# populationgenomics/cuKING

Hardware: AMD Instinct MI355X
Metric: sample-pairs/s (all-pairs KING) (higher is better)
Workload: dtype fp4 products, f32 accumulate (exact integers)

## Files before the change

### cuking_amd/build.py

```python
from __future__ import annotations

import argparse
import os
import shutil
import subprocess
import sys
from pathlib import Path

PKG = Path(__file__).resolve().parent
ROOT = PKG.parent
CSRC = PKG / "csrc"
HOST = PKG / "host"
INCLUDE = ROOT / "include"

LIB_PATH = PKG / "libcuking_amd.so"
CLI_PATH = PKG / "bin" / "cuking"
LIB_FLAGS_PATH = PKG / "libcuking_amd.flags"

HIP_SOURCES = ["king_abi.hip", "king_kernels.hip", "king_mfma.hip", "king_filter.hip",
               "king_sort.hip", "synth.hip"]
HOST_ABI_SOURCES = ["king_host.cc"]
HIP_FLAGS = [
    "--offload-arch=gfx950", "-O3", "-std=c++17", "-fPIC", "-Wall",
    "-fno-fast-math", "-ffp-contract=off",
    "-fhip-fp32-correctly-rounded-divide-sqrt",
]


ROCM = Path(os.environ.get("ROCM_PATH", "/opt/rocm"))
ROCM_HOST_FLAGS = ["-D__HIP_PLATFORM_AMD__=1", f"-isystem{ROCM / 'include'}"]
ROCM_HOST_LIBS = [f"-L{ROCM / 'lib'}", "-lrccl", "-lamdhip64"]


def _hipcc() -> str:
    exe = shutil.which("hipcc") or "/opt/rocm/bin/hipcc"
    if not os.path.exists(exe):
        raise RuntimeError("hipcc not found: the HIP library cannot be built")
    return exe


def _newer(target: Path, deps) -> bool:
    if not target.exists():
        return False
    t = target.stat().st_mtime
    return all(Path(d).stat().st_mtime <= t for d in deps)


def build_library(force: bool = False, save_temps: bool = False) -> Path:
    srcs = [CSRC / s for s in HIP_SOURCES + HOST_ABI_SOURCES]
    deps = srcs + [CSRC / "king_common.h", CSRC / "king_device.h", CSRC / "king_host.h",
                   CSRC / "king_submatrix.h", INCLUDE / "cuking_amd.h",
                   Path(__file__)]
    extra = os.environ.get("CUKING_EXTRA_HIPFLAGS", "").split()
    wanted = " ".join(extra)
    stamped = LIB_FLAGS_PATH.read_text().strip() if LIB_FLAGS_PATH.exists() else wanted
    if not force and _newer(LIB_PATH, deps) and stamped == wanted:
        return LIB_PATH
    cmd = [_hipcc(), *HIP_FLAGS, "-shared", f"-I{INCLUDE}", f"-I{CSRC}",
           *map(str, srcs), "-o", str(LIB_PATH)]
    for flag in extra:
        cmd.insert(1, flag)
    cwd = PKG / "build_tmp"
    cwd.mkdir(exist_ok=True)
    cmd += ["-save-temps"]
    if save_temps:
        cmd += ["-Rpass-analysis=kernel-resource-usage"]
        subprocess.run(cmd, check=True, cwd=str(cwd))
    else:
        with open(cwd / "build.log", "w") as log:
            r = subprocess.run(cmd, cwd=str(cwd), stdout=log, stderr=subprocess.STDOUT)
        if r.returncode != 0:
            sys.stderr.write((cwd / "build.log").read_text()[-8000:])
            raise subprocess.CalledProcessError(r.returncode, cmd)
    problems = check_mfma_loops(cwd / "king_mfma-hip-amdgcn-amd-amdhsa-gfx950.s")
    problems += check_filter_loop(cwd / "king_filter-hip-amdgcn-amd-amdhsa-gfx950.s")
    if problems and not extra:
        LIB_PATH.unlink(missing_ok=True)
        raise RuntimeError("matrix-core kernel: the compiler put vector-memory waits or scratch "
                           "accesses inside an LDS-DMA loop:\n  " + "\n  ".join(problems))
    for line in problems:
        print("warning (experiment build):", line, file=sys.stderr)
    LIB_FLAGS_PATH.write_text(wanted + "\n")
    return LIB_PATH


def check_filter_loop(asm_path: Path, verbose: bool = False):
    import re
    text = Path(asm_path).read_text()
    bodies = [m.group(1) for m in re.finditer(
        r"\n_ZN6cuking12_GLOBAL__N_1\d+king_filter(?:_persistent)?_kernelE\w+:(.*?)\.Lfunc_end", text, re.S)]
    if len(bodies) < 2:
        return [f"king_filter_kernel / king_filter_persistent_kernel not both in {asm_path}"]
    problems, seen = [], 0
    for block in (b for body in bodies for b in re.split(r"\n(?=\.LBB\d+_\d+:)", body)):
        lines = block.split("\n")
        head = lines[0].split(":")[0]
        end = next((i for i, l in enumerate(lines)
                    if re.search(r"s_cbranch_\w+ " + re.escape(head) + r"\b", l)), None)
        if end is None:
            continue
        loop = lines[:end + 1]
        mfma = sum("v_mfma" in l for l in loop)
        if mfma < 16 or not any("global_load_lds" in l for l in loop):
            continue
        seen += 1
        scratch = [l.strip() for l in loop if "scratch_" in l]
        waits = [l.strip() for l in loop if re.search(r"s_waitcnt.*vmcnt\(\d+\)", l)]
        foreign = [w for w in waits if "vmcnt(22)" not in w]
        if verbose:
            print(f"king_filter_kernel: loop {head} ({mfma} MFMAs): scratch {len(scratch)}, "
                  f"vmcnt waits {waits}")
        if scratch or foreign:
            problems.append(f"king_filter_kernel, loop {head}: scratch {scratch[:2]}, waits {foreign}")
    if seen < 2:
        problems.append("king_filter kernels: an LDS-DMA loop is missing (listing format changed?)")
    return problems


def check_mfma_loops(asm_path: Path, verbose: bool = False):
    import re
    text = Path(asm_path).read_text()
    funcs = re.split(r"\n(?=_ZN6cuking12_GLOBAL__N_116king_mfma_kernel\w+:)", text)[1:]
    if not funcs:
        return [f"no king_mfma_kernel in {asm_path}"]
    problems = []
    for f in funcs:
        m = re.match(r"_ZN6cuking12_GLOBAL__N_116king_mfma_kernelILb(\d)ELb(\d)ELb(\d)", f)
        label = f"king_mfma_kernel<FULL={m.group(1)}, SPLIT={m.group(2)}, N4={m.group(3)}>"
        body = f.split(".Lfunc_end")[0]
        seen = 0
        for block in re.split(r"\n(?=\.LBB\d+_\d+:)", body):
            lines = block.split("\n")
            head = lines[0].split(":")[0]
            end = next((i for i, l in enumerate(lines)
                        if re.search(r"s_cbranch_\w+ " + re.escape(head) + r"\b", l)), None)
            if end is None:
                continue
            loop = lines[:end + 1]
            mfma = sum("v_mfma" in l for l in loop)
            if mfma < 16 or not any("global_load_lds" in l for l in loop):
                continue
            seen += 1
            scratch = [l.strip() for l in loop if "scratch_" in l]
            waits = [l.strip() for l in loop if re.search(r"s_waitcnt.*vmcnt\(\d+\)", l)]
            foreign = [w for w in waits
                       if not any(f"vmcnt({n})" in w for n in (16, 20, 24))]
            if verbose:
                print(f"{label}: loop {head} ({mfma} MFMAs): scratch {len(scratch)}, "
                      f"vmcnt waits {waits}")
            if scratch or foreign:
                problems.append(f"{label}, loop {head}: scratch {scratch[:2]}, waits {foreign}")
        if seen == 0:
            problems.append(f"{label}: no LDS-DMA loop found (listing format changed?)")
    return problems


def arrow_flags():
    import pyarrow
    inc = pyarrow.get_include()
    libdir = pyarrow.get_library_dirs()[0]
    libs = []
    for stem in ("parquet", "arrow"):
        cands = sorted(Path(libdir).glob(f"lib{stem}.so.*"))
        if not cands:
            raise RuntimeError(f"lib{stem}.so not found in {libdir}")
        libs.append(f"-l:{cands[0].name}")
    return inc, libdir, libs


def build_cli(force: bool = False) -> Path:
    srcs = sorted(HOST.glob("*.cc"))
    if not srcs:
        raise RuntimeError("no host sources")
    deps = srcs + sorted(HOST.glob("*.h")) + [INCLUDE / "cuking_amd.h",
                                              LIB_PATH, Path(__file__)]
    if not force and _newer(CLI_PATH, deps):
        return CLI_PATH
    inc, libdir, libs = arrow_flags()
    CLI_PATH.parent.mkdir(exist_ok=True)
    cmd = ["g++", "-O2", "-std=c++20", "-Wall", "-pthread",
           f"-I{INCLUDE}", f"-I{HOST}", f"-isystem{inc}", *ROCM_HOST_FLAGS,
           *map(str, srcs), "-o", str(CLI_PATH),
           f"-L{PKG}", "-l:libcuking_amd.so", f"-L{libdir}", *libs, *ROCM_HOST_LIBS,
           f"-Wl,-rpath,{libdir}", "-Wl,-rpath,$ORIGIN/..",
           "-Wl,-rpath,/opt/rocm/lib"]
    subprocess.run(cmd, check=True)
    return CLI_PATH


def main(argv=None) -> int:
    ap = argparse.ArgumentParser()
    ap.add_argument("--lib", action="store_true", help="library only")
    ap.add_argument("--force", action="store_true")
    ap.add_argument("--save-temps", action="store_true")
    args = ap.parse_args(argv)
    print(build_library(force=args.force, save_temps=args.save_temps))
    if not args.lib:
        print(build_cli(force=args.force))
    return 0


if __name__ == "__main__":
    sys.exit(main())
```

### cuking_amd/csrc/king_abi.hip

```cpp
#include <hip/hip_runtime.h>

#include <algorithm>
#include <atomic>
#include <cstdarg>
#include <cstdio>
#include <cstdlib>
#include <cstring>
#include <string>
#include <tuple>
#include <vector>

#include "king_common.h"
#include "king_host.h"

using namespace cuking;

namespace {

#define HIP_TRY(expr)                                                      \
  do {                                                                     \
    const hipError_t _e = (expr);                                          \
    if (_e != hipSuccess) {                                                \
      (void)hipGetLastError();  \
      return cuking_fail(_e == hipErrorOutOfMemory ? CUKING_ERR_OUT_OF_MEMORY     \
                                            : CUKING_ERR_DEVICE,           \
                  "%s failed: %s", #expr, hipGetErrorString(_e));          \
    }                                                                      \
  } while (0)

uint32_t ceil_div(uint32_t a, uint32_t b) {
  return (uint32_t)(((uint64_t)a + b - 1) / b);
}
uint32_t round_up(uint32_t a, uint32_t b) { return ceil_div(a, b) * b; }

struct EventPair {
  hipEvent_t start = nullptr, stop = nullptr;
};

struct Timer {
  std::vector<EventPair> pool;
  size_t used = 0;

  hipError_t begin(hipStream_t s, EventPair **out) {
    if (used == pool.size()) {
      EventPair p;
      hipError_t e = hipEventCreate(&p.start);
      if (e != hipSuccess) return e;
      e = hipEventCreate(&p.stop);
      if (e != hipSuccess) return e;
      pool.push_back(p);
    }
    *out = &pool[used++];
    return hipEventRecord((*out)->start, s);
  }
  hipError_t collect(double *ms, uint64_t *n) {
    *ms = 0;
    *n = used;
    for (size_t k = 0; k < used; ++k) {
      hipError_t e = hipEventSynchronize(pool[k].stop);
      if (e != hipSuccess) return e;
      float t = 0;
      e = hipEventElapsedTime(&t, pool[k].start, pool[k].stop);
      if (e != hipSuccess) return e;
      *ms += t;
    }
    return hipSuccess;
  }
  void destroy() {
    for (auto &p : pool) {
      if (p.start) (void)hipEventDestroy(p.start);
      if (p.stop) (void)hipEventDestroy(p.stop);
    }
    pool.clear();
    used = 0;
  }
};

}

struct cuking_ctx {
  int device = 0;
  cuking_kernel kernel = CUKING_KERNEL_TILED;
  int variant = 0;
  uint32_t band_rows = 0;
  int counts_mode = -1;
  int xcd_swizzle = 2;
  uint32_t dyn_tail_tiles = 16384;

  uint4 *planes = nullptr;
  size_t planes_bytes = 0;
  uint64_t *band_prefix = nullptr;
  size_t band_prefix_entries = 0;
  TileSpace prefix_for = {0, 0, 0, 0};

  uint32_t split_wgs = 0;
  std::vector<std::pair<hipStream_t, uint32_t *>> split_scratch;
  struct FilterScratch {
    hipStream_t stream;
    uint8_t *base;
    uint64_t tiles;
  };
  std::vector<FilterScratch> filter_scratch;
  unsigned long long filter_totals_retired[kNumTotals] = {};
  uint32_t filter_quadrant_cap = kFilterQuadrantCap;
  uint32_t filter_cand_cap = kFilterCandCap;
  uint32_t filter_split_min_steps = 8;
  int filter_check0 = 1, filter_check1 = 1, filter_check_emit = (int)kCheckEmitCap;
  int filter_rotate = 1;
  uint32_t filter_rotate_min_steps = 128;
  uint32_t filter_rotate_min_tiles = 2048;
  bool filter_persistent = false;
  uint32_t filter_persistent_min_tiles = 2048;
  int filter_sort = 1;
  bool filter_lazy_codes = true;
  void *sort_temp = nullptr;
  size_t sort_temp_bytes = 0;

  struct Prepared {
    bool valid = false;
    cuking_submatrix sm = {0, 0, 0, 0};
    uint32_t words_per_sample = 0;
    int variant = -1;
    uint32_t tile = 0;
    const uint64_t *bits = nullptr;
    bool codes = true;
    std::vector<uint8_t> tiles;
    hipStream_t ordered_on = nullptr;
    bool ordered_valid = false;
  } prepared;
  std::vector<std::pair<hipStream_t, hipEvent_t>> readers;

  bool reuse_prepared = false;
  uint64_t workspace_allocations = 0, host_syncs = 0, conversions_skipped = 0;

  bool timing = false;
  Timer king_timer, prepare_timer;
};

namespace {

int default_variant() {
  if (const char *v = getenv("CUKING_AMD_VARIANT")) {
    const int k = atoi(v);
    if (k >= 0 && k < kNumTiledVariants) return k;
  }
  return kMfmaFilterVariant;
}

int effective_variant(const cuking_ctx *ctx, uint32_t words_per_sample) {
  const uint64_t sites = (uint64_t)round_up(words_per_sample, 8) * 32;
  int v = ctx->variant;
  if ((v == kMfmaN4Variant || v == kMfmaFilterVariant) && sites > kMfmaN4MaxSites) v = kMfmaVariant;
  if (v == kMfmaVariant && sites > kMfmaMaxSites) v = 2;
  return v;
}

TiledVariant plan_variant(const cuking_ctx *ctx, uint32_t words_per_sample) {
  TiledVariant v = tiled_variant(effective_variant(ctx, words_per_sample));
  v.tile = tiled_variant(ctx->variant).tile;
  return v;
}

bool use_full_counts(const cuking_ctx *ctx, float kin_threshold, bool dense,
                     uint32_t words_per_sample) {
  if (dense || ctx->counts_mode == 1) return true;
  if (ctx->counts_mode == 0) return false;
  if (!(kin_threshold > 0.0f)) return true;
  const double sites = 32.0 * words_per_sample;
  const double c = is_mfma_variant(effective_variant(ctx, words_per_sample)) ? 2.05 : 1.6;
  return (double)kin_threshold * kin_threshold * sites < c * c;
}

cuking_status bind(cuking_ctx *ctx) {
  if (ctx == nullptr) return cuking_fail(CUKING_ERR_INVALID_ARGUMENT, "null context");
  HIP_TRY(hipSetDevice(ctx->device));
  return CUKING_OK;
}

PlaneGeometry make_geometry(const cuking_submatrix &sm,
                            uint32_t words_per_sample,
                            const TiledVariant &v) {
  PlaneGeometry g;
  g.num_rows = sm_num_rows(sm);
  g.num_cols = sm_num_cols(sm);
  g.diag = sm_is_diag(sm) ? 1u : 0u;
  g.rows_padded = round_up(g.num_rows, v.tile);
  g.cols_padded = round_up(g.num_cols, v.tile);
  g.col_base = g.diag ? 0u : g.rows_padded;
  g.s_stride = g.diag ? g.rows_padded : g.rows_padded + g.cols_padded;
  g.k_words = round_up(words_per_sample, v.k_chunk);
  return g;
}

uint32_t band_rows_for(uint32_t pinned, const PlaneGeometry &g, const TiledVariant &v) {
  if (pinned != 0) return pinned;
  if (v.layout == kLayoutWord) return 17;
  if (v.tile == kFilterTile) return 8;
  return g.rows_padded / v.tile >= 128 ? 5 : 17;
}

TileSpace make_tiles(const PlaneGeometry &g, const TiledVariant &v,
                     uint32_t band_rows) {
  band_rows = band_rows_for(band_rows, g, v);
  TileSpace t;
  t.tiles_r = g.rows_padded / v.tile;
  t.tiles_c = g.cols_padded / v.tile;
  t.band_rows = band_rows;
  t.diag = g.diag;
  return t;
}

uint64_t total_tiles(const TileSpace &t) {
  uint64_t n = 0;
  for (uint32_t b = 0; b < t.num_bands(); ++b) n += t.band_tiles(b);
  return n;
}

cuking_status split_scratch_for(cuking_ctx *ctx, hipStream_t stream,
                                uint32_t **scratch, uint32_t **counters) {
  *scratch = *counters = nullptr;
  if (ctx->split_wgs == 0 || !is_mfma_variant(ctx->variant)) return CUKING_OK;
  const size_t bytes = mfma_split_scratch_bytes(ctx->split_wgs);
  uint32_t *base = nullptr;
  for (auto &e : ctx->split_scratch)
    if (e.first == stream) base = e.second;
  if (base == nullptr) {
    if (ctx->split_scratch.size() >= 8) {
      ++ctx->host_syncs;
      HIP_TRY(hipDeviceSynchronize());
      for (auto &e : ctx->split_scratch) (void)hipFree(e.second);
      ctx->split_scratch.clear();
    }
    HIP_TRY(hipMalloc(reinterpret_cast<void **>(&base), bytes));
    ++ctx->workspace_allocations;
    hipError_t e = hipMemsetAsync(base, 0, mfma_split_counter_bytes(ctx->split_wgs), stream);
    if (e != hipSuccess) {
      (void)hipFree(base);
      HIP_TRY(e);
    }
    ctx->split_scratch.emplace_back(stream, base);
  }
  *counters = base;
  *scratch = base + mfma_split_counter_bytes(ctx->split_wgs) / sizeof(uint32_t);
  return CUKING_OK;
}

static void retire_filter_totals(cuking_ctx *ctx, const cuking_ctx::FilterScratch &e) {
  if (e.base == nullptr) return;
  unsigned long long v[kNumTotals] = {};
  if (hipMemcpy(v, e.base + filter_scratch_layout(e.tiles).totals, sizeof v,
                hipMemcpyDeviceToHost) != hipSuccess) {
    (void)hipGetLastError();
    return;
  }
  for (uint32_t k = 0; k < kNumTotals; ++k) ctx->filter_totals_retired[k] += v[k];
}

cuking_status filter_scratch_for(cuking_ctx *ctx, hipStream_t stream, const PlaneGeometry &geo,
                                 uint64_t tiles, TiledArgs *a) {
  a->sample_stats = nullptr;
  a->t2 = nullptr;
  a->filter_ctrl = nullptr;
  a->cand_list = nullptr;
  a->dense_list = nullptr;
  a->cand_cap = a->dense_cap = a->quadrant_cap = 0;
  a->fsplit_parts = a->fsplit_first = a->fsplit_tile0 = 0;
  a->fsplit_slabs = nullptr;
  a->fsplit_tickets = nullptr;
  a->filter_totals = nullptr;
  a->tile_done = nullptr;
  a->prefix_u = nullptr;
  a->cohort_sums = nullptr;
  a->check_steps = nullptr;
  a->check0 = a->check1 = 0;
  a->rotate = a->rotate_min_steps = a->rotate_min_tiles = 0;
  a->persist_wgs = a->persist_min_tiles = 0;
  if (ctx->variant != kMfmaFilterVariant) return CUKING_OK;
  const FilterScratchLayout want = filter_scratch_layout(tiles);
  cuking_ctx::FilterScratch *entry = nullptr;
  for (auto &e : ctx->filter_scratch)
    if (e.stream == stream) entry = &e;
  if (entry != nullptr && filter_scratch_layout(entry->tiles).bytes < want.bytes) {
    ++ctx->host_syncs;
    HIP_TRY(hipStreamSynchronize(stream));
    retire_filter_totals(ctx, *entry);
    (void)hipFree(entry->base);
    entry->base = nullptr;
  }
  if (entry == nullptr || entry->base == nullptr) {
    if (entry == nullptr && ctx->filter_scratch.size() >= 8) {
      ++ctx->host_syncs;
      HIP_TRY(hipStreamSynchronize(ctx->filter_scratch.front().stream));
      (void)hipGetLastError();
      retire_filter_totals(ctx, ctx->filter_scratch.front());
      (void)hipFree(ctx->filter_scratch.front().base);
      ctx->filter_scratch.erase(ctx->filter_scratch.begin());
    }
    uint8_t *base = nullptr;
    HIP_TRY(hipMalloc(reinterpret_cast<void **>(&base), want.bytes));
    ++ctx->workspace_allocations;
    hipError_t e = hipMemsetAsync(base + want.totals, 0, kFilterCtrlBytes + kFilterTicketBytes, stream);
    if (e != hipSuccess) {
      (void)hipFree(base);
      HIP_TRY(e);
    }
    if (entry == nullptr) {
      ctx->filter_scratch.push_back({stream, base, tiles});
      entry = &ctx->filter_scratch.back();
    } else {
      entry->base = base;
      entry->tiles = tiles;
    }
  }
  uint8_t *base = entry->base;
  const FilterScratchLayout l = filter_scratch_layout(entry->tiles);
  a->sample_stats = plane_stats(ctx->planes, geo);
  a->t2 = plane_t2(ctx->planes, geo);
  a->prefix_u = plane_prefix_u(ctx->planes, geo);
  a->cohort_sums = plane_cohort_sums(ctx->planes, geo);
  a->filter_ctrl = reinterpret_cast<uint32_t *>(base);
  a->filter_totals = reinterpret_cast<unsigned long long *>(base + l.totals);
  a->fsplit_tickets = reinterpret_cast<uint32_t *>(base + l.tickets);
  a->tile_done = base + l.tile_done;
  a->cand_list = reinterpret_cast<uint2 *>(base + l.cand);
  a->cand_cap = ctx->filter_cand_cap < l.cand_entries ? ctx->filter_cand_cap : l.cand_entries;
  a->quadrant_cap = ctx->filter_quadrant_cap;
  a->dense_list = reinterpret_cast<uint2 *>(base + l.dense);
  a->dense_cap = l.chunk_tiles * 4;
  a->fsplit_first = ctx->filter_split_min_steps;
  a->fsplit_slabs = ctx->split_wgs != 0 ? reinterpret_cast<float4 *>(base + l.slabs) : nullptr;
  a->check0 = (uint32_t)ctx->filter_check0;
  a->check1 = (uint32_t)ctx->filter_check1 | ((uint32_t)ctx->filter_check_emit << 8) |
              (ctx->filter_check0 != 0 ? 1u << 16 : 0u);
  a->rotate = (uint32_t)ctx->filter_rotate;
  a->rotate_min_steps = ctx->filter_rotate_min_steps;
  a->rotate_min_tiles = ctx->filter_rotate_min_tiles;
  a->persist_wgs = ctx->filter_persistent ? 1u : 0u;
  a->persist_min_tiles = ctx->filter_persistent_min_tiles;
  a->check_steps = plane_check_steps(ctx->planes, geo);
  return CUKING_OK;
}

void layout_order_for(const cuking_ctx *ctx, uint32_t words_per_sample, const PlaneGeometry &geo,
                      TiledArgs *a) {
  a->perm = nullptr;
  a->codes_ready = nullptr;
  if (plan_variant(ctx, words_per_sample).layout != kLayoutNibbleStats) return;
  a->perm = plane_perm(ctx->planes, geo);
  if (!ctx->prepared.codes) a->codes_ready = plane_flags(ctx->planes, geo);
}

hipError_t launch_planned(const cuking_ctx *ctx, uint32_t words_per_sample, bool full,
                          TiledArgs a, uint64_t num_tiles, hipStream_t stream) {
  const int kv = effective_variant(ctx, words_per_sample);
  a.quad = 0;
  a.tile_list = nullptr;
  a.tile_list_count = nullptr;
  a.tile_list_cap = 0;
  if (tiled_variant(kv).tile != tiled_variant(ctx->variant).tile) {
    if (tiled_variant(kv).tile * 2 != tiled_variant(ctx->variant).tile) return hipErrorInvalidValue;
    a.quad = 1;
    a.tile_begin *= 4;
    num_tiles *= 4;
  }
  return launch_tiled(kv, full, a, num_tiles, stream);
}

void note_reader(cuking_ctx *ctx, hipStream_t stream) {
  for (auto &r : ctx->readers)
    if (r.first == stream) return;
  ctx->readers.emplace_back(stream, nullptr);
}

cuking_status wait_for_readers(cuking_ctx *ctx, hipStream_t stream) {
  bool failed = false;
  for (auto &r : ctx->readers) {
    if (r.first == stream) continue;
    if (r.second == nullptr &&
        hipEventCreateWithFlags(&r.second, hipEventDisableTiming) != hipSuccess) {
      failed = true;
      break;
    }
    if (hipEventRecord(r.second, r.first) != hipSuccess ||
        hipStreamWaitEvent(stream, r.second, 0) != hipSuccess) {
      failed = true;
      break;
    }
  }
  if (failed) {
    (void)hipGetLastError();
    ++ctx->host_syncs;
    HIP_TRY(hipDeviceSynchronize());
  }
  for (auto &r : ctx->readers)
    if (r.second) (void)hipEventDestroy(r.second);
  ctx->readers.clear();
  ctx->readers.emplace_back(stream, nullptr);
  ctx->prepared.ordered_on = stream;
  ctx->prepared.ordered_valid = true;
  for (auto &t : ctx->prepared.tiles)
    if (t == 2) t = 1;
  return CUKING_OK;
}

void mark_read(cuking_ctx *ctx, uint32_t begin, uint32_t end) {
  std::vector<uint8_t> &t = ctx->prepared.tiles;
  if (end > t.size()) end = (uint32_t)t.size();
  for (uint32_t k = begin; k < end; ++k) t[k] = 2;
}

bool same_block(const cuking_ctx::Prepared &p, const cuking_submatrix &sm,
                uint32_t words_per_sample, int variant, uint32_t tile, const uint64_t *bits) {
  return p.valid && p.sm.i_begin == sm.i_begin && p.sm.i_end == sm.i_end &&
         p.sm.j_begin == sm.j_begin && p.sm.j_end == sm.j_end &&
         p.words_per_sample == words_per_sample && p.variant == variant &&
         p.tile == tile && p.bits == bits;
}

cuking_status ensure_workspace(cuking_ctx *ctx, size_t need, size_t entries) {
  if (need > ctx->planes_bytes) {
    ++ctx->host_syncs;
    HIP_TRY(hipDeviceSynchronize());
    if (ctx->planes) HIP_TRY(hipFree(ctx->planes));
    ctx->planes = nullptr;
    ctx->planes_bytes = 0;
    ctx->prepared.valid = false;
    HIP_TRY(hipMalloc(reinterpret_cast<void **>(&ctx->planes), need));
    ++ctx->workspace_allocations;
    ctx->planes_bytes = need;
  }
  if (entries > ctx->band_prefix_entries) {
    ++ctx->host_syncs;
    HIP_TRY(hipDeviceSynchronize());
    if (ctx->band_prefix) HIP_TRY(hipFree(ctx->band_prefix));
    ctx->band_prefix = nullptr;
    ctx->band_prefix_entries = 0;
    ctx->prefix_for = TileSpace{0, 0, 0, 0};
    HIP_TRY(hipMalloc(reinterpret_cast<void **>(&ctx->band_prefix), entries * sizeof(uint64_t)));
    ++ctx->workspace_allocations;
    ctx->band_prefix_entries = entries;
  }
  return CUKING_OK;
}

cuking_status ensure_sort_temp(cuking_ctx *ctx, uint32_t n) {
  const size_t need = sort_temp_bytes_for(n);
  if (need <= ctx->sort_temp_bytes) return CUKING_OK;
  ++ctx->host_syncs;
  HIP_TRY(hipDeviceSynchronize());
  if (ctx->sort_temp) HIP_TRY(hipFree(ctx->sort_temp));
  ctx->sort_temp = nullptr;
  ctx->sort_temp_bytes = 0;
  HIP_TRY(hipMalloc(&ctx->sort_temp, need));
  ++ctx->workspace_allocations;
  ctx->sort_temp_bytes = need;
  return CUKING_OK;
}

bool same_tile_space(const TileSpace &a, const TileSpace &b) {
  return a.tiles_r == b.tiles_r && a.tiles_c == b.tiles_c && a.band_rows == b.band_rows &&
         a.diag == b.diag;
}

cuking_status upload_prefix(cuking_ctx *ctx, const TileSpace &tiles, hipStream_t stream) {
  const uint32_t nb = tiles.num_bands();
  std::vector<uint64_t> prefix((size_t)nb + 1, 0);
  for (uint32_t b = 0; b < nb; ++b) prefix[b + 1] = prefix[b] + tiles.band_tiles(b);
  HIP_TRY(hipMemcpyAsync(ctx->band_prefix, prefix.data(), prefix.size() * sizeof(uint64_t),
                         hipMemcpyHostToDevice, stream));
  ++ctx->host_syncs;
  HIP_TRY(hipStreamSynchronize(stream));
  ctx->prefix_for = tiles;
  return CUKING_OK;
}

cuking_status convert_codes_now(cuking_ctx *ctx, const PlaneGeometry &geo,
                                uint32_t words_per_sample, const uint64_t *d_bit_sets,
                                hipStream_t stream) {
  cuking_ctx::Prepared &pr = ctx->prepared;
  const uint32_t all = (uint32_t)pr.tiles.size();
  for (uint32_t t = 0; t < all;) {
    if (pr.tiles[t] == 0) {
      ++t;
      continue;
    }
    uint32_t e = t;
    while (e < all && pr.tiles[e] != 0) ++e;
    HIP_TRY(launch_prepare_nibbles(true, false, d_bit_sets, words_per_sample, geo, ctx->planes,
                                   plane_perm(ctx->planes, geo), t, e, nullptr, nullptr, stream));
    t = e;
  }
  HIP_TRY(hipMemsetAsync(plane_flags(ctx->planes, geo), 1, sizeof(uint32_t), stream));
  pr.codes = true;
  return CUKING_OK;
}

cuking_status prepare(cuking_ctx *ctx, const cuking_submatrix &sm,
                      uint32_t words_per_sample, const uint64_t *d_bit_sets,
                      hipStream_t stream, PlaneGeometry *geo_out,
                      TileSpace *tiles_out, bool need_codes, uint32_t s_tile_begin = 0,
                      uint32_t s_tile_end = 0xFFFFFFFFu) {
  const int variant = effective_variant(ctx, words_per_sample);
  const TiledVariant v = plan_variant(ctx, words_per_sample);
  const PlaneGeometry geo = make_geometry(sm, words_per_sample, v);
  const TileSpace tiles = make_tiles(geo, v, ctx->band_rows);
  *geo_out = geo;
  *tiles_out = tiles;

  const size_t need = plane_bytes(geo, v.layout);
  const uint32_t nb = tiles.num_bands();
  cuking_status st = ensure_workspace(ctx, need, (size_t)nb + 1);
  if (st != CUKING_OK) return st;
  if (v.layout == kLayoutNibbleStats && ctx->filter_sort != 0) {
    st = ensure_sort_temp(ctx, geo.s_stride);
    if (st != CUKING_OK) return st;
  }
  const uint32_t all_tiles = (geo.s_stride + 63) / 64;
  const uint32_t t_end = s_tile_end < all_tiles ? s_tile_end : all_tiles;
  cuking_ctx::Prepared &pr = ctx->prepared;
  const bool new_prefix = !same_tile_space(ctx->prefix_for, tiles);
  const bool same = same_block(pr, sm, words_per_sample, variant, v.tile, d_bit_sets);
  if (ctx->reuse_prepared && same && !new_prefix) {
    bool all_there = true;
    for (uint32_t t = s_tile_begin; t < t_end && all_there; ++t) all_there = pr.tiles[t] != 0;
    if (all_there) {
      ++ctx->conversions_skipped;
      if (v.layout == kLayoutNibbleStats && need_codes && !pr.codes)
        return convert_codes_now(ctx, geo, words_per_sample, d_bit_sets, stream);
      return CUKING_OK;
    }
  }
  const bool other_stream = pr.ordered_valid && pr.ordered_on != stream;
  bool must_wait = new_prefix && !ctx->readers.empty();
  if (!same) {
    must_wait = must_wait || !ctx->readers.empty();
    pr.valid = true;
    pr.sm = sm;
    pr.words_per_sample = words_per_sample;
    pr.variant = variant;
    pr.tile = v.tile;
    pr.bits = d_bit_sets;
    pr.tiles.assign(all_tiles, 0);
    pr.codes = true;
  }
  for (uint32_t t = s_tile_begin; t < t_end; ++t)
    must_wait = must_wait || pr.tiles[t] == 2 || (pr.tiles[t] == 1 && other_stream);
  if (must_wait) {
    st = wait_for_readers(ctx, stream);
    if (st != CUKING_OK) return st;
  }
  for (uint32_t t = s_tile_begin; t < t_end; ++t) pr.tiles[t] = 1;
  if (new_prefix) {
    st = upload_prefix(ctx, tiles, stream);
    if (st != CUKING_OK) return st;
  }

  if (need == 0) return CUKING_OK;
  EventPair *ev = nullptr;
  if (ctx->timing) HIP_TRY(ctx->prepare_timer.begin(stream, &ev));
  if (v.layout == kLayoutNibbleStats) {
    const bool whole = s_tile_begin == 0 && t_end == all_tiles;
    const bool codes = need_codes || !ctx->filter_lazy_codes || !whole;
    const uint32_t sb = s_tile_begin * 64, se = t_end * 64;
    if (s_tile_begin == 0)
      HIP_TRY(hipMemsetAsync(const_cast<unsigned long long *>(plane_cohort_sums(ctx->planes, geo)),
                             0, 64, stream));
    HIP_TRY(hipMemsetAsync(plane_flags(ctx->planes, geo), 0, sizeof(uint32_t), stream));
    HIP_TRY(launch_sample_stats(d_bit_sets, words_per_sample, geo, ctx->planes, sb, se, stream));
    HIP_TRY(launch_sample_order(geo, words_per_sample, ctx->planes, sb, se,
                                ctx->filter_sort == 2 || (ctx->filter_sort == 1 && whole),
                                ctx->sort_temp, ctx->sort_temp_bytes, stream));
    HIP_TRY(launch_prepare_nibbles(codes, true, d_bit_sets, words_per_sample, geo, ctx->planes,
                                   plane_perm(ctx->planes, geo), s_tile_begin, t_end, nullptr,
                                   nullptr, stream));
    if (!codes) {
      pr.codes = false;
    } else if (!pr.codes) {
      st = convert_codes_now(ctx, geo, words_per_sample, d_bit_sets, stream);
      if (st != CUKING_OK) return st;
    } else {
      HIP_TRY(hipMemsetAsync(plane_flags(ctx->planes, geo), 1, sizeof(uint32_t), stream));
    }
  } else {
    HIP_TRY(launch_prepare_planes(v.layout, d_bit_sets, words_per_sample, geo, ctx->planes,
                                  s_tile_begin, s_tile_end, stream));
  }
  if (ev) HIP_TRY(hipEventRecord(ev->stop, stream));
  return CUKING_OK;
}

cuking_status run_tiled(cuking_ctx *ctx, const cuking_submatrix &sm,
                        uint32_t words_per_sample, const uint64_t *d_bit_sets,
                        uint64_t tile_begin, uint64_t tile_end, bool whole,
                        float kin_threshold, uint32_t max_results,
                        cuking_result *d_results, uint32_t *d_result_index,
                        uint32_t *d_result_overflow, cuking_counts *d_counts,
                        hipStream_t stream) {
  PlaneGeometry geo;
  TileSpace tiles;
  const bool full = use_full_counts(ctx, kin_threshold, d_counts != nullptr, words_per_sample);
  const bool filter_runs = effective_variant(ctx, words_per_sample) == kMfmaFilterVariant &&
                           !full && kin_threshold > 0.f && kin_threshold < 0.5f;
  cuking_status st =
      prepare(ctx, sm, words_per_sample, d_bit_sets, stream, &geo, &tiles, !filter_runs);
  if (st != CUKING_OK) return st;
  const uint64_t n_tiles = total_tiles(tiles);
  if (whole) {
    tile_begin = 0;
    tile_end = n_tiles;
  }
  if (tile_begin > tile_end || tile_end > n_tiles)
    return cuking_fail(CUKING_ERR_INVALID_ARGUMENT,
                "tile range [%llu, %llu) outside [0, %llu)",
                (unsigned long long)tile_begin, (unsigned long long)tile_end,
                (unsigned long long)n_tiles);
  if (tile_begin == tile_end) return CUKING_OK;

  TiledArgs a = {};
  a.planes = ctx->planes;
  a.geo = geo;
  a.tiles = tiles;
  a.band_prefix = ctx->band_prefix;
  a.tile_begin = tile_begin;
  a.i_begin = sm.i_begin;
  a.j_begin = sm.j_begin;
  a.kin_threshold = kin_threshold;
  a.max_results = max_results;
  a.results = d_results;
  a.result_index = d_result_index;
  a.result_overflow = d_result_overflow;
  a.dense_counts = d_counts;
  a.rect_rows = a.rect_cols = a.rect_row0 = a.rect_col0 = 0;
  a.rect_row_stride = 1;
  a.bits = d_bit_sets;
  a.words_per_sample = words_per_sample;
  a.split_tiles = 0;
  a.split_whole = 0;
  a.split_wgs = ctx->split_wgs;
  a.xcd_chunk = (uint32_t)ctx->xcd_swizzle;
  a.launch_tiles = 0;
  a.dyn_tiles = ctx->dyn_tail_tiles;
  a.dyn_wgs = 0;
  st = split_scratch_for(ctx, stream, &a.split_scratch, &a.split_counters);
  if (st != CUKING_OK) return st;
  st = filter_scratch_for(ctx, stream, geo, n_tiles, &a);
  if (st != CUKING_OK) return st;
  layout_order_for(ctx, words_per_sample, geo, &a);

  EventPair *ev = nullptr;
  if (ctx->timing) HIP_TRY(ctx->king_timer.begin(stream, &ev));
  HIP_TRY(launch_planned(ctx, words_per_sample, full, a, tile_end - tile_begin, stream));
  note_reader(ctx, stream);
  mark_read(ctx, 0, 0xFFFFFFFFu);
  if (ev) HIP_TRY(hipEventRecord(ev->stop, stream));
  return CUKING_OK;
}

cuking_status run_stream(cuking_ctx *ctx, const cuking_submatrix &sm,
                         uint32_t words_per_sample, const uint64_t *d_bit_sets,
                         float kin_threshold, uint32_t max_results,
                         cuking_result *d_results, uint32_t *d_result_index,
                         uint32_t *d_result_overflow, cuking_counts *d_counts,
                         hipStream_t stream) {
  EventPair *ev = nullptr;
  if (ctx->timing) HIP_TRY(ctx->king_timer.begin(stream, &ev));
  HIP_TRY(launch_stream(sm, words_per_sample, d_bit_sets, kin_threshold,
                        max_results, d_results, d_result_index,
                        d_result_overflow, d_counts, stream));
  if (ev) HIP_TRY(hipEventRecord(ev->stop, stream));
  return CUKING_OK;
}

}

extern "C" {


int cuking_device_count(void) {
  int n = 0;
  if (hipGetDeviceCount(&n) != hipSuccess) return 0;
  return n;
}

cuking_status cuking_ctx_create(int device, cuking_ctx **out) {
  if (out == nullptr) return cuking_fail(CUKING_ERR_INVALID_ARGUMENT, "null out pointer");
  *out = nullptr;
  int n = 0;
  hipError_t e = hipGetDeviceCount(&n);
  if (e != hipSuccess || n == 0)
    return cuking_fail(CUKING_ERR_DEVICE,
                "no HIP device available (%s); this library has no CPU path",
                e == hipSuccess ? "0 devices" : hipGetErrorString(e));
  if (device < 0 || device >= n)
    return cuking_fail(CUKING_ERR_INVALID_ARGUMENT, "device %d outside [0, %d)", device, n);
  hipDeviceProp_t prop;
  HIP_TRY(hipGetDeviceProperties(&prop, device));
  if (strncmp(prop.gcnArchName, "gfx950", 6) != 0)
    return cuking_fail(CUKING_ERR_DEVICE,
                "device %d is %s; this library only carries gfx950 code",
                device, prop.gcnArchName);
  HIP_TRY(hipSetDevice(device));
  cuking_ctx *ctx = new cuking_ctx();
  ctx->device = device;
  ctx->variant = default_variant();
  ctx->split_wgs = (uint32_t)prop.multiProcessorCount;
  if (const char *v = getenv("CUKING_AMD_SPLIT_WGS")) {
    const int k = atoi(v);
    if (k >= 0 && k <= 4096) ctx->split_wgs = (uint32_t)k;
  }
  if (const char *v = getenv("CUKING_AMD_XCD_SWIZZLE")) {
    const int k = atoi(v);
    if (k >= 0 && k <= 2) ctx->xcd_swizzle = k;
  }
  if (const char *v = getenv("CUKING_AMD_DYN_TAIL_TILES")) {
    const long long k = atoll(v);
    if (k >= 0 && k <= 0x7FFFFFFF) ctx->dyn_tail_tiles = (uint32_t)k;
  }
  if (const char *v = getenv("CUKING_AMD_BAND_ROWS")) {
    const int k = atoi(v);
    if (k >= 1 && k <= 64) ctx->band_rows = (uint32_t)k;
  }
  *out = ctx;
  return CUKING_OK;
}

void cuking_ctx_destroy(cuking_ctx *ctx) {
  if (ctx == nullptr) return;
  (void)hipSetDevice(ctx->device);
  if (ctx->planes) (void)hipFree(ctx->planes);
  if (ctx->band_prefix) (void)hipFree(ctx->band_prefix);
  if (ctx->sort_temp) (void)hipFree(ctx->sort_temp);
  for (auto &e : ctx->split_scratch) (void)hipFree(e.second);
  for (auto &e : ctx->filter_scratch) (void)hipFree(e.base);
  for (auto &r : ctx->readers)
    if (r.second) (void)hipEventDestroy(r.second);
  ctx->king_timer.destroy();
  ctx->prepare_timer.destroy();
  delete ctx;
}

cuking_status cuking_ctx_set_kernel(cuking_ctx *ctx, cuking_kernel kernel) {
  if (ctx == nullptr) return cuking_fail(CUKING_ERR_INVALID_ARGUMENT, "null context");
  if (kernel != CUKING_KERNEL_TILED && kernel != CUKING_KERNEL_STREAM)
    return cuking_fail(CUKING_ERR_INVALID_ARGUMENT, "unknown kernel %d", (int)kernel);
  ctx->kernel = kernel;
  return CUKING_OK;
}

cuking_status cuking_ctx_set_option(cuking_ctx *ctx, const char *key,
                                    int64_t value) {
  if (ctx == nullptr || key == nullptr)
    return cuking_fail(CUKING_ERR_INVALID_ARGUMENT, "null argument");
  if (strcmp(key, "variant") == 0) {
    if (value < 0 || value >= kNumTiledVariants)
      return cuking_fail(CUKING_ERR_INVALID_ARGUMENT, "variant outside [0, %d)",
                  kNumTiledVariants);
    ctx->variant = (int)value;
    return CUKING_OK;
  }
  if (strcmp(key, "band_rows") == 0) {
    if (value < 0 || value > 64)
      return cuking_fail(CUKING_ERR_INVALID_ARGUMENT, "band_rows outside [0, 64]");
    ctx->band_rows = (uint32_t)value;
    return CUKING_OK;
  }
  if (strcmp(key, "split_wgs") == 0) {
    if (value < 0 || value > 4096)
      return cuking_fail(CUKING_ERR_INVALID_ARGUMENT, "split_wgs outside [0, 4096]");
    if ((uint32_t)value != ctx->split_wgs) {
      HIP_TRY(hipDeviceSynchronize());
      for (auto &e : ctx->split_scratch) (void)hipFree(e.second);
      ctx->split_scratch.clear();
    }
    ctx->split_wgs = (uint32_t)value;
    return CUKING_OK;
  }
  if (strcmp(key, "max_launch_blocks") == 0) {
    if (value < 0) return cuking_fail(CUKING_ERR_INVALID_ARGUMENT, "negative block cap");
    set_max_blocks_per_launch((uint64_t)value);
    return CUKING_OK;
  }
  if (strcmp(key, "dyn_tail_tiles") == 0) {
    if (value < 0 || value > 0x7FFFFFFF)
      return cuking_fail(CUKING_ERR_INVALID_ARGUMENT, "dyn_tail_tiles outside [0, 2^31)");
    ctx->dyn_tail_tiles = (uint32_t)value;
    return CUKING_OK;
  }
  if (strcmp(key, "xcd_swizzle") == 0) {
    if (value < 0 || value > 2)
      return cuking_fail(CUKING_ERR_INVALID_ARGUMENT, "xcd_swizzle outside [0, 2]");
    ctx->xcd_swizzle = (int)value;
    return CUKING_OK;
  }
  if (strcmp(key, "counts_mode") == 0) {
    if (value < -1 || value > 1)
      return cuking_fail(CUKING_ERR_INVALID_ARGUMENT, "counts_mode outside [-1, 1]");
    ctx->counts_mode = (int)value;
    return CUKING_OK;
  }
  if (strcmp(key, "filter_quadrant_cap") == 0) {
    if (value < 0 || value > 16384)
      return cuking_fail(CUKING_ERR_INVALID_ARGUMENT, "filter_quadrant_cap outside [0, 16384]");
    ctx->filter_quadrant_cap = (uint32_t)value;
    return CUKING_OK;
  }
  if (strcmp(key, "filter_split_min_steps") == 0) {
    if (value < 1 || value > 4096)
      return cuking_fail(CUKING_ERR_INVALID_ARGUMENT, "filter_split_min_steps outside [1, 4096]");
    ctx->filter_split_min_steps = (uint32_t)value;
    return CUKING_OK;
  }
  if (strcmp(key, "filter_check_min_steps") == 0) {
    if (value < 4 || value > 1 << 20)
      return cuking_fail(CUKING_ERR_INVALID_ARGUMENT, "filter_check_min_steps outside [4, 2^20]");
    set_filter_check_min_steps((uint32_t)value);
    ctx->prepared.valid = false;
    return CUKING_OK;
  }
  if (strcmp(key, "filter_sort") == 0) {
    if (value < 0 || value > 2)
      return cuking_fail(CUKING_ERR_INVALID_ARGUMENT, "filter_sort outside [0, 2]");
    ctx->filter_sort = (int)value;
    ctx->prepared.valid = false;
    return CUKING_OK;
  }
  if (strcmp(key, "filter_lazy_codes") == 0) {
    if (value < 0 || value > 1)
      return cuking_fail(CUKING_ERR_INVALID_ARGUMENT, "filter_lazy_codes outside [0, 1]");
    ctx->filter_lazy_codes = value != 0;
    ctx->prepared.valid = false;
    return CUKING_OK;
  }
  if (strcmp(key, "filter_check0") == 0) {
    if (value < 0 || value > 2)
      return cuking_fail(CUKING_ERR_INVALID_ARGUMENT, "filter_check0 outside [0, 2]");
    ctx->filter_check0 = (int)value;
    return CUKING_OK;
  }
  if (strcmp(key, "filter_rotate") == 0) {
    if (value < 0 || value > 2 + (int64_t)kNumPhases)
      return cuking_fail(CUKING_ERR_INVALID_ARGUMENT, "filter_rotate outside [0, %u]", 2 + kNumPhases);
    ctx->filter_rotate = (int)value;
    return CUKING_OK;
  }
  if (strcmp(key, "filter_persistent_min_tiles") == 0) {
    if (value < 0 || value > (1 << 30))
      return cuking_fail(CUKING_ERR_INVALID_ARGUMENT, "filter_persistent_min_tiles outside [0, 2^30]");
    ctx->filter_persistent_min_tiles = (uint32_t)value;
    return CUKING_OK;
  }
  if (strcmp(key, "filter_persistent") == 0) {
    ctx->filter_persistent = value != 0;
    return CUKING_OK;
  }
  if (strcmp(key, "filter_rotate_min_tiles") == 0) {
    if (value < 0 || value > (1 << 30))
      return cuking_fail(CUKING_ERR_INVALID_ARGUMENT, "filter_rotate_min_tiles outside [0, 2^30]");
    ctx->filter_rotate_min_tiles = (uint32_t)value;
    return CUKING_OK;
  }
  if (strcmp(key, "filter_rotate_min_steps") == 0) {
    if (value < 1 || value > (1 << 20))
      return cuking_fail(CUKING_ERR_INVALID_ARGUMENT, "filter_rotate_min_steps outside [1, 2^20]");
    ctx->filter_rotate_min_steps = (uint32_t)value;
    return CUKING_OK;
  }
  if (strcmp(key, "filter_check_emit") == 0) {
    if (value < 0 || value > 255)
      return cuking_fail(CUKING_ERR_INVALID_ARGUMENT, "filter_check_emit outside [0, 255]");
    ctx->filter_check_emit = (int)value;
    return CUKING_OK;
  }
  if (strcmp(key, "filter_check1") == 0) {
    if (value < 0 || value > 1 + (int64_t)kNumCheckShares || value == 2)
      return cuking_fail(CUKING_ERR_INVALID_ARGUMENT, "filter_check1 outside {0, 1, 3 .. %u}",
                  1 + kNumCheckShares);
    ctx->filter_check1 = (int)value;
    return CUKING_OK;
  }
  if (strcmp(key, "filter_cand_cap") == 0) {
    if (value < 0 || value > (int64_t)kFilterCandCap)
      return cuking_fail(CUKING_ERR_INVALID_ARGUMENT, "filter_cand_cap outside [0, %u]", kFilterCandCap);
    ctx->filter_cand_cap = (uint32_t)value;
    return CUKING_OK;
  }
  if (strcmp(key, "reuse_prepared") == 0) {
    if (value < 0 || value > 1)
      return cuking_fail(CUKING_ERR_INVALID_ARGUMENT, "reuse_prepared outside [0, 1]");
    ctx->reuse_prepared = value != 0;
    return CUKING_OK;
  }
  return cuking_fail(CUKING_ERR_INVALID_ARGUMENT, "unknown option %s", key);
}

cuking_status cuking_device_alloc(cuking_ctx *ctx, size_t bytes, void **d_ptr) {
  cuking_status st = bind(ctx);
  if (st != CUKING_OK) return st;
  if (d_ptr == nullptr) return cuking_fail(CUKING_ERR_INVALID_ARGUMENT, "null out pointer");
  *d_ptr = nullptr;
  if (bytes == 0) return CUKING_OK;
  HIP_TRY(hipMalloc(d_ptr, bytes));
  return CUKING_OK;
}

cuking_status cuking_device_free(cuking_ctx *ctx, void *d_ptr) {
  cuking_status st = bind(ctx);
  if (st != CUKING_OK) return st;
  if (d_ptr) HIP_TRY(hipFree(d_ptr));
  return CUKING_OK;
}

cuking_status cuking_memset_async(cuking_ctx *ctx, void *d_ptr, int byte_value,
                                  size_t bytes, void *stream) {
  cuking_status st = bind(ctx);
  if (st != CUKING_OK) return st;
  if (bytes) HIP_TRY(hipMemsetAsync(d_ptr, byte_value, bytes, (hipStream_t)stream));
  return CUKING_OK;
}

cuking_status cuking_copy_to_device(cuking_ctx *ctx, void *d_dst,
                                    const void *src, size_t bytes,
                                    void *stream) {
  cuking_status st = bind(ctx);
  if (st != CUKING_OK) return st;
  if (bytes)
    HIP_TRY(hipMemcpyAsync(d_dst, src, bytes, hipMemcpyHostToDevice,
                           (hipStream_t)stream));
  return CUKING_OK;
}

cuking_status cuking_copy_to_host(cuking_ctx *ctx, void *dst, const void *d_src,
                                  size_t bytes, void *stream) {
  cuking_status st = bind(ctx);
  if (st != CUKING_OK) return st;
  if (bytes)
    HIP_TRY(hipMemcpyAsync(dst, d_src, bytes, hipMemcpyDeviceToHost,
                           (hipStream_t)stream));
  return CUKING_OK;
}

cuking_status cuking_stream_synchronize(cuking_ctx *ctx, void *stream) {
  cuking_status st = bind(ctx);
  if (st != CUKING_OK) return st;
  HIP_TRY(hipStreamSynchronize((hipStream_t)stream));
  return CUKING_OK;
}

cuking_status cuking_stream_create(cuking_ctx *ctx, void **stream) {
  cuking_status st = bind(ctx);
  if (st != CUKING_OK) return st;
  if (stream == nullptr) return cuking_fail(CUKING_ERR_INVALID_ARGUMENT, "null out pointer");
  hipStream_t s = nullptr;
  HIP_TRY(hipStreamCreateWithFlags(&s, hipStreamNonBlocking));
  *stream = s;
  return CUKING_OK;
}

cuking_status cuking_stream_destroy(cuking_ctx *ctx, void *stream) {
  cuking_status st = bind(ctx);
  if (st != CUKING_OK) return st;
  if (stream) {
    auto &rs = ctx->readers;
    for (size_t k = 0; k < rs.size(); ++k)
      if (rs[k].first == (hipStream_t)stream) {
        HIP_TRY(hipStreamSynchronize((hipStream_t)stream));
        if (rs[k].second) (void)hipEventDestroy(rs[k].second);
        rs.erase(rs.begin() + k);
        break;
      }
    HIP_TRY(hipStreamDestroy((hipStream_t)stream));
  }
  return CUKING_OK;
}

cuking_status cuking_host_alloc(cuking_ctx *ctx, size_t bytes, void **ptr) {
  cuking_status st = bind(ctx);
  if (st != CUKING_OK) return st;
  if (ptr == nullptr) return cuking_fail(CUKING_ERR_INVALID_ARGUMENT, "null out pointer");
  *ptr = nullptr;
  if (bytes == 0) return CUKING_OK;
  HIP_TRY(hipHostMalloc(ptr, bytes, hipHostMallocDefault));
  return CUKING_OK;
}

cuking_status cuking_host_free(cuking_ctx *ctx, void *ptr) {
  cuking_status st = bind(ctx);
  if (st != CUKING_OK) return st;
  if (ptr) HIP_TRY(hipHostFree(ptr));
  return CUKING_OK;
}


cuking_status cuking_pack_device(cuking_ctx *ctx, const cuking_submatrix *sm,
                                 uint32_t words_per_sample, uint64_t *d_bit_set,
                                 const int64_t *d_row_idx,
                                 const int64_t *d_col_idx,
                                 const int32_t *d_n_alt_alleles,
                                 size_t num_triples, uint32_t *d_status,
                                 void *stream) {
  cuking_status st = bind(ctx);
  if (st != CUKING_OK) return st;
  st = cuking_check_block(sm, words_per_sample);
  if (st != CUKING_OK) return st;
  if (num_triples &&
      (!d_bit_set || !d_row_idx || !d_col_idx || !d_n_alt_alleles || !d_status))
    return cuking_fail(CUKING_ERR_INVALID_ARGUMENT, "null device pointer");
  HIP_TRY(launch_pack(*sm, words_per_sample, d_bit_set, d_row_idx, d_col_idx,
                      d_n_alt_alleles, num_triples, d_status,
                      (hipStream_t)stream));
  return CUKING_OK;
}

cuking_status cuking_pack_device_compact(cuking_ctx *ctx, const cuking_submatrix *sm,
                                         uint32_t words_per_sample, uint64_t *d_bit_set,
                                         const uint32_t *d_site,
                                         const uint32_t *d_sample_alt, size_t num_triples,
                                         uint32_t *d_status, void *stream) {
  cuking_status st = bind(ctx);
  if (st != CUKING_OK) return st;
  st = cuking_check_block(sm, words_per_sample);
  if (st != CUKING_OK) return st;
  if (num_triples && (!d_bit_set || !d_site || !d_sample_alt || !d_status))
    return cuking_fail(CUKING_ERR_INVALID_ARGUMENT, "null device pointer");
  HIP_TRY(launch_pack_compact(words_per_sample, sm_num_samples(*sm), d_bit_set, d_site,
                              d_sample_alt, num_triples, d_status, (hipStream_t)stream));
  return CUKING_OK;
}

cuking_status cuking_event_create(cuking_ctx *ctx, void **event) {
  cuking_status st = bind(ctx);
  if (st != CUKING_OK) return st;
  if (event == nullptr) return cuking_fail(CUKING_ERR_INVALID_ARGUMENT, "null out pointer");
  hipEvent_t e = nullptr;
  HIP_TRY(hipEventCreateWithFlags(&e, hipEventDisableTiming));
  *event = e;
  return CUKING_OK;
}

cuking_status cuking_event_record(cuking_ctx *ctx, void *event, void *stream) {
  cuking_status st = bind(ctx);
  if (st != CUKING_OK) return st;
  HIP_TRY(hipEventRecord((hipEvent_t)event, (hipStream_t)stream));
  return CUKING_OK;
}

cuking_status cuking_event_synchronize(cuking_ctx *ctx, void *event) {
  cuking_status st = bind(ctx);
  if (st != CUKING_OK) return st;
  HIP_TRY(hipEventSynchronize((hipEvent_t)event));
  return CUKING_OK;
}

cuking_status cuking_event_destroy(cuking_ctx *ctx, void *event) {
  cuking_status st = bind(ctx);
  if (st != CUKING_OK) return st;
  if (event) HIP_TRY(hipEventDestroy((hipEvent_t)event));
  return CUKING_OK;
}

uint32_t cuking_tile_samples(const cuking_ctx *ctx) {
  return tiled_variant(ctx ? ctx->variant : default_variant()).tile;
}

uint64_t cuking_num_tiles(const cuking_ctx *ctx, const cuking_submatrix *sm) {
  if (sm == nullptr) return 0;
  const TiledVariant &v = tiled_variant(ctx ? ctx->variant : default_variant());
  const PlaneGeometry g = make_geometry(*sm, 2, v);
  if (g.num_rows == 0 || g.num_cols == 0) return 0;
  return total_tiles(make_tiles(g, v, ctx ? ctx->band_rows : 0));
}

cuking_status cuking_tile_bounds(const cuking_ctx *ctx,
                                 const cuking_submatrix *sm, uint64_t tile,
                                 uint32_t *row_begin, uint32_t *row_end,
                                 uint32_t *col_begin, uint32_t *col_end) {
  cuking_status st = cuking_check_block(sm, 2);
  if (st != CUKING_OK) return st;
  const TiledVariant &v = tiled_variant(ctx ? ctx->variant : default_variant());
  const PlaneGeometry g = make_geometry(*sm, 2, v);
  const TileSpace ts = make_tiles(g, v, ctx ? ctx->band_rows : 0);
  if (g.num_rows == 0 || g.num_cols == 0 || tile >= total_tiles(ts))
    return cuking_fail(CUKING_ERR_INVALID_ARGUMENT, "tile index out of range");
  uint32_t b = 0;
  uint64_t first = 0;
  while (first + ts.band_tiles(b) <= tile) first += ts.band_tiles(b++);
  uint32_t tr, tc;
  ts.decode(b, tile - first, &tr, &tc);
  auto clampr = [&](uint64_t x) { return (uint32_t)std::min<uint64_t>(x, g.num_rows); };
  auto clampc = [&](uint64_t x) { return (uint32_t)std::min<uint64_t>(x, g.num_cols); };
  if (row_begin) *row_begin = sm->i_begin + clampr((uint64_t)tr * v.tile);
  if (row_end) *row_end = sm->i_begin + clampr((uint64_t)(tr + 1) * v.tile);
  if (col_begin) *col_begin = sm->j_begin + clampc((uint64_t)tc * v.tile);
  if (col_end) *col_end = sm->j_begin + clampc((uint64_t)(tc + 1) * v.tile);
  return CUKING_OK;
}

cuking_status cuking_ctx_get_option(const cuking_ctx *ctx, const char *key,
                                    int64_t *value) {
  if (ctx == nullptr || key == nullptr || value == nullptr)
    return cuking_fail(CUKING_ERR_INVALID_ARGUMENT, "null argument");
  if (strcmp(key, "variant") == 0) *value = ctx->variant;
  else if (strcmp(key, "split_wgs") == 0) *value = ctx->split_wgs;
  else if (strcmp(key, "band_rows") == 0) *value = ctx->band_rows;
  else if (strcmp(key, "counts_mode") == 0) *value = ctx->counts_mode;
  else if (strcmp(key, "xcd_swizzle") == 0) *value = ctx->xcd_swizzle;
  else if (strcmp(key, "dyn_tail_tiles") == 0) *value = ctx->dyn_tail_tiles;
  else if (strcmp(key, "reuse_prepared") == 0) *value = ctx->reuse_prepared ? 1 : 0;
  else if (strcmp(key, "filter_quadrant_cap") == 0) *value = ctx->filter_quadrant_cap;
  else if (strcmp(key, "filter_cand_cap") == 0) *value = ctx->filter_cand_cap;
  else if (strcmp(key, "filter_split_min_steps") == 0) *value = ctx->filter_split_min_steps;
  else if (strcmp(key, "filter_sort") == 0) *value = ctx->filter_sort;
  else if (strcmp(key, "filter_lazy_codes") == 0) *value = ctx->filter_lazy_codes ? 1 : 0;
  else if (strcmp(key, "filter_check0") == 0) *value = ctx->filter_check0;
  else if (strcmp(key, "filter_check1") == 0) *value = ctx->filter_check1;
  else if (strcmp(key, "filter_check_emit") == 0) *value = ctx->filter_check_emit;
  else if (strcmp(key, "filter_rotate") == 0) *value = ctx->filter_rotate;
  else if (strcmp(key, "filter_rotate_min_steps") == 0) *value = ctx->filter_rotate_min_steps;
  else if (strcmp(key, "filter_rotate_min_tiles") == 0) *value = ctx->filter_rotate_min_tiles;
  else if (strcmp(key, "filter_persistent") == 0) *value = ctx->filter_persistent ? 1 : 0;
  else if (strcmp(key, "filter_persistent_min_tiles") == 0) *value = ctx->filter_persistent_min_tiles;
  else if (strcmp(key, "filter_candidates") == 0 || strcmp(key, "filter_dense_quadrants") == 0 ||
           strcmp(key, "filter_early_exits") == 0 || strcmp(key, "filter_rotated_tiles") == 0) {
    const size_t word = strcmp(key, "filter_candidates") == 0        ? kTotalCand
                        : strcmp(key, "filter_dense_quadrants") == 0 ? kTotalDense
                        : strcmp(key, "filter_early_exits") == 0     ? kTotalEarly
                                                                     : kTotalRotated;
    unsigned long long total = 0;
    if (hipSetDevice(ctx->device) != hipSuccess || hipDeviceSynchronize() != hipSuccess)
      return cuking_fail(CUKING_ERR_DEVICE, "device wait failed");
    for (auto &e : ctx->filter_scratch) {
      unsigned long long v = 0;
      if (hipMemcpy(&v, e.base + filter_scratch_layout(e.tiles).totals + word * 8, 8,
                    hipMemcpyDeviceToHost) != hipSuccess)
        return cuking_fail(CUKING_ERR_DEVICE, "reading the filter counters failed");
      total += v;
    }
    *value = (int64_t)(total + ctx->filter_totals_retired[word]);
  }
  else if (strcmp(key, "filter_step_ticks16") == 0) {
    if (hipSetDevice(ctx->device) != hipSuccess || hipDeviceSynchronize() != hipSuccess)
      return cuking_fail(CUKING_ERR_DEVICE, "device wait failed");
    uint64_t sum = 0, count = 0;
    for (auto &e : ctx->filter_scratch) {
      uint32_t w[8];
      if (hipMemcpy(w, e.base + kCtrlStepTicks * 4, sizeof w, hipMemcpyDeviceToHost) != hipSuccess)
        return cuking_fail(CUKING_ERR_DEVICE, "reading the filter counters failed");
      for (uint32_t v : w)
        if (v != 0) {
          sum += v;
          ++count;
        }
    }
    *value = count != 0 ? (int64_t)(sum / count) : 0;
  }
  else if (strcmp(key, "workspace_allocations") == 0) *value = (int64_t)ctx->workspace_allocations;
  else if (strcmp(key, "host_syncs") == 0) *value = (int64_t)ctx->host_syncs;
  else if (strcmp(key, "conversions_skipped") == 0) *value = (int64_t)ctx->conversions_skipped;
  else return cuking_fail(CUKING_ERR_INVALID_ARGUMENT, "unknown option %s", key);
  return CUKING_OK;
}

int cuking_num_variants(void) { return kNumTiledVariants; }
const char *cuking_variant_name(int variant) {
  if (variant < 0 || variant >= kNumTiledVariants) return "";
  return tiled_variant(variant).name;
}

static cuking_status check_compute_args(const cuking_submatrix *sm,
                                        uint32_t words_per_sample,
                                        const uint64_t *d_bit_sets) {
  cuking_status st = cuking_check_block(sm, words_per_sample);
  if (st != CUKING_OK) return st;
  if (sm_num_samples(*sm) != 0 && d_bit_sets == nullptr)
    return cuking_fail(CUKING_ERR_INVALID_ARGUMENT, "null bitset pointer");
  return CUKING_OK;
}

cuking_status cuking_compute_king(cuking_ctx *ctx, const cuking_submatrix *sm,
                                  uint32_t words_per_sample,
                                  const uint64_t *d_bit_sets,
                                  float kin_threshold, uint32_t max_results,
                                  cuking_result *d_results,
                                  uint32_t *d_result_index,
                                  uint32_t *d_result_overflow, void *stream) {
  cuking_status st = bind(ctx);
  if (st != CUKING_OK) return st;
  st = check_compute_args(sm, words_per_sample, d_bit_sets);
  if (st != CUKING_OK) return st;
  if (!d_result_index || !d_result_overflow || (max_results && !d_results))
    return cuking_fail(CUKING_ERR_INVALID_ARGUMENT, "null result pointer");
  if (sm_num_rows(*sm) == 0 || sm_num_cols(*sm) == 0) return CUKING_OK;
  if (ctx->kernel == CUKING_KERNEL_STREAM)
    return run_stream(ctx, *sm, words_per_sample, d_bit_sets, kin_threshold,
                      max_results, d_results, d_result_index, d_result_overflow,
                      nullptr, (hipStream_t)stream);
  return run_tiled(ctx, *sm, words_per_sample, d_bit_sets, 0, 0, true,
                   kin_threshold, max_results, d_results, d_result_index,
                   d_result_overflow, nullptr, (hipStream_t)stream);
}

cuking_status cuking_compute_king_tiles(
    cuking_ctx *ctx, const cuking_submatrix *sm, uint32_t words_per_sample,
    const uint64_t *d_bit_sets, uint64_t tile_begin, uint64_t tile_end,
    float kin_threshold, uint32_t max_results, cuking_result *d_results,
    uint32_t *d_result_index, uint32_t *d_result_overflow, void *stream) {
  cuking_status st = bind(ctx);
  if (st != CUKING_OK) return st;
  st = check_compute_args(sm, words_per_sample, d_bit_sets);
  if (st != CUKING_OK) return st;
  if (!d_result_index || !d_result_overflow || (max_results && !d_results))
    return cuking_fail(CUKING_ERR_INVALID_ARGUMENT, "null result pointer");
  if (sm_num_rows(*sm) == 0 || sm_num_cols(*sm) == 0) {
    if (tile_begin != 0 || tile_end != 0)
      return cuking_fail(CUKING_ERR_INVALID_ARGUMENT, "empty block has no tiles");
    return CUKING_OK;
  }
  return run_tiled(ctx, *sm, words_per_sample, d_bit_sets, tile_begin, tile_end,
                   false, kin_threshold, max_results, d_results, d_result_index,
                   d_result_overflow, nullptr, (hipStream_t)stream);
}

static cuking_status tile_span(const cuking_submatrix &sm, uint32_t tile,
                               uint32_t begin, uint32_t end, const char *what,
                               uint32_t *t0, uint32_t *t1) {
  if (begin < sm.i_begin || end > sm.i_end || begin > end)
    return cuking_fail(CUKING_ERR_INVALID_ARGUMENT, "%s range [%u, %u) outside the block",
                what, begin, end);
  const uint32_t b = begin - sm.i_begin, e = end - sm.i_begin;
  if (b % tile != 0 || (e % tile != 0 && end != sm.i_end))
    return cuking_fail(CUKING_ERR_INVALID_ARGUMENT,
                "%s range [%u, %u) is not aligned to the %u-sample tile edge", what,
                begin, end, tile);
  *t0 = b / tile;
  *t1 = (e + tile - 1) / tile;
  return CUKING_OK;
}

cuking_status cuking_prepare_samples(cuking_ctx *ctx, const cuking_submatrix *sm,
                                     uint32_t words_per_sample,
                                     const uint64_t *d_bit_sets,
                                     uint32_t sample_begin, uint32_t sample_end,
                                     void *stream) {
  cuking_status st = bind(ctx);
  if (st != CUKING_OK) return st;
  st = check_compute_args(sm, words_per_sample, d_bit_sets);
  if (st != CUKING_OK) return st;
  if (!sm_is_diag(*sm))
    return cuking_fail(CUKING_ERR_INVALID_ARGUMENT,
                "staged preparation needs a diagonal block (rows == columns)");
  const uint32_t tile = plan_variant(ctx, words_per_sample).tile;
  uint32_t t0, t1;
  st = tile_span(*sm, tile, sample_begin, sample_end, "sample", &t0, &t1);
  if (st != CUKING_OK) return st;
  if (t0 == t1) return CUKING_OK;
  PlaneGeometry geo;
  TileSpace tiles;
  return prepare(ctx, *sm, words_per_sample, d_bit_sets, (hipStream_t)stream, &geo,
                 &tiles, true, t0 * (tile / 64), t1 * (tile / 64));
}

cuking_status cuking_compute_king_rect(
    cuking_ctx *ctx, const cuking_submatrix *sm, uint32_t words_per_sample,
    const uint64_t *d_bit_sets, uint32_t row_begin, uint32_t row_end,
    uint32_t row_step, uint32_t col_begin, uint32_t col_end, float kin_threshold,
    uint32_t max_results, cuking_result *d_results, uint32_t *d_result_index,
    uint32_t *d_result_overflow, void *stream) {
  cuking_status st = bind(ctx);
  if (st != CUKING_OK) return st;
  st = check_compute_args(sm, words_per_sample, d_bit_sets);
  if (st != CUKING_OK) return st;
  if (!sm_is_diag(*sm))
    return cuking_fail(CUKING_ERR_INVALID_ARGUMENT,
                "rectangle launches need a diagonal block (rows == columns)");
  if (!d_result_index || !d_result_overflow || (max_results && !d_results))
    return cuking_fail(CUKING_ERR_INVALID_ARGUMENT, "null result pointer");
  const TiledVariant v = plan_variant(ctx, words_per_sample);
  const PlaneGeometry geo = make_geometry(*sm, words_per_sample, v);
  const TileSpace tiles = make_tiles(geo, v, ctx->band_rows ? ctx->band_rows : 17);
  const size_t need = plane_bytes(geo, v.layout);
  const int variant = effective_variant(ctx, words_per_sample);
  if (ctx->planes == nullptr || ctx->planes_bytes < need ||
      !same_block(ctx->prepared, *sm, words_per_sample, variant, v.tile, d_bit_sets))
    return cuking_fail(CUKING_ERR_FAILED_PRECONDITION,
                "cuking_prepare_samples() has not been called for this block "
                "(or the workspace has been converted for another one since)");
  uint32_t r0, r1, c0, c1;
  st = tile_span(*sm, v.tile, row_begin, row_end, "row", &r0, &r1);
  if (st != CUKING_OK) return st;
  st = tile_span(*sm, v.tile, col_begin, col_end, "column", &c0, &c1);
  if (st != CUKING_OK) return st;
  if (r0 == r1 || c0 == c1) return CUKING_OK;
  if (row_step == 0) row_step = v.tile;
  if (row_step % v.tile != 0)
    return cuking_fail(CUKING_ERR_INVALID_ARGUMENT,
                "row_step %u is not a multiple of the %u-sample tile edge", row_step,
                v.tile);
  const uint32_t stride = row_step / v.tile;
  const uint32_t n_rows = (r1 - r0 + stride - 1) / stride;
  {
    const uint32_t per = v.tile / 64;
    const std::vector<uint8_t> &done = ctx->prepared.tiles;
    auto converted = [&](uint32_t tile) {
      for (uint32_t t = tile * per; t < (tile + 1) * per; ++t)
        if (t >= done.size() || !done[t]) return false;
      return true;
    };
    for (uint32_t r = r0; r < r1; r += stride)
      if (!converted(r))
        return cuking_fail(CUKING_ERR_FAILED_PRECONDITION,
                    "row samples from %u on have not been prepared",
                    sm->i_begin + r * v.tile);
    for (uint32_t c = c0; c < c1; ++c)
      if (!converted(c))
        return cuking_fail(CUKING_ERR_FAILED_PRECONDITION,
                    "column samples from %u on have not been prepared",
                    sm->i_begin + c * v.tile);
  }

  TiledArgs a = {};
  a.planes = ctx->planes;
  a.geo = geo;
  a.tiles = tiles;
  a.band_prefix = ctx->band_prefix;
  a.tile_begin = 0;
  a.rect_rows = n_rows;
  a.rect_cols = c1 - c0;
  a.rect_row0 = r0;
  a.rect_col0 = c0;
  a.rect_row_stride = stride;
  a.i_begin = sm->i_begin;
  a.j_begin = sm->j_begin;
  a.kin_threshold = kin_threshold;
  a.max_results = max_results;
  a.results = d_results;
  a.result_index = d_result_index;
  a.result_overflow = d_result_overflow;
  a.dense_counts = nullptr;
  a.bits = d_bit_sets;
  a.words_per_sample = words_per_sample;
  a.split_tiles = 0;
  a.split_whole = 0;
  a.split_wgs = ctx->split_wgs;
  a.xcd_chunk = ctx->xcd_swizzle == 2 ? 2u : 0u;
  a.launch_tiles = 0;
  a.dyn_tiles = ctx->dyn_tail_tiles;
  a.dyn_wgs = 0;
  st = split_scratch_for(ctx, (hipStream_t)stream, &a.split_scratch, &a.split_counters);
  if (st != CUKING_OK) return st;
  st = filter_scratch_for(ctx, (hipStream_t)stream, geo, total_tiles(make_tiles(geo, v, ctx->band_rows)), &a);
  if (st != CUKING_OK) return st;
  layout_order_for(ctx, words_per_sample, geo, &a);
  const bool full = use_full_counts(ctx, kin_threshold, false, words_per_sample);
  if (v.layout == kLayoutNibbleStats && !ctx->prepared.codes &&
      !(variant == kMfmaFilterVariant && !full && kin_threshold > 0.f && kin_threshold < 0.5f)) {
    st = convert_codes_now(ctx, geo, words_per_sample, d_bit_sets, (hipStream_t)stream);
    if (st != CUKING_OK) return st;
    a.codes_ready = nullptr;
  }
  EventPair *ev = nullptr;
  if (ctx->timing) HIP_TRY(ctx->king_timer.begin((hipStream_t)stream, &ev));
  HIP_TRY(launch_planned(ctx, words_per_sample, full, a, (uint64_t)n_rows * (c1 - c0),
                         (hipStream_t)stream));
  note_reader(ctx, (hipStream_t)stream);
  {
    const uint32_t per = v.tile / 64;
    for (uint32_t r = r0; r < r1; r += stride) mark_read(ctx, r * per, (r + 1) * per);
    mark_read(ctx, c0 * per, c1 * per);
  }
  if (ev) HIP_TRY(hipEventRecord(ev->stop, (hipStream_t)stream));
  return CUKING_OK;
}

cuking_status cuking_ctx_reserve(cuking_ctx *ctx, const cuking_submatrix *sm,
                                 uint32_t words_per_sample, void *const *streams,
                                 size_t num_streams) {
  cuking_status st = bind(ctx);
  if (st != CUKING_OK) return st;
  st = cuking_check_block(sm, words_per_sample);
  if (st != CUKING_OK) return st;
  if (num_streams != 0 && streams == nullptr)
    return cuking_fail(CUKING_ERR_INVALID_ARGUMENT, "null stream list");
  if (sm_num_rows(*sm) == 0 || sm_num_cols(*sm) == 0) return CUKING_OK;
  const TiledVariant v = plan_variant(ctx, words_per_sample);
  const PlaneGeometry geo = make_geometry(*sm, words_per_sample, v);
  const TileSpace tiles = make_tiles(geo, v, ctx->band_rows);
  st = ensure_workspace(ctx, plane_bytes(geo, v.layout), (size_t)tiles.num_bands() + 1);
  if (st != CUKING_OK) return st;
  if (v.layout == kLayoutNibbleStats && ctx->filter_sort != 0) {
    st = ensure_sort_temp(ctx, geo.s_stride);
    if (st != CUKING_OK) return st;
  }
  if (!same_tile_space(ctx->prefix_for, tiles)) {
    if (!ctx->readers.empty()) {
      ++ctx->host_syncs;
      HIP_TRY(hipDeviceSynchronize());
    }
    st = upload_prefix(ctx, tiles, nullptr);
    if (st != CUKING_OK) return st;
  }
  if (num_streams > 8)
    return cuking_fail(CUKING_ERR_INVALID_ARGUMENT, "at most 8 streams per context can be reserved");
  if (ctx->split_wgs != 0 && is_mfma_variant(ctx->variant)) {
    size_t missing = 0;
    for (size_t k = 0; k < num_streams; ++k) {
      bool have = false;
      for (auto &e : ctx->split_scratch) have = have || e.first == (hipStream_t)streams[k];
      missing += have ? 0 : 1;
    }
    if (missing != 0 && ctx->split_scratch.size() + missing > 8) {
      ++ctx->host_syncs;
      HIP_TRY(hipDeviceSynchronize());
      for (auto &e : ctx->split_scratch) (void)hipFree(e.second);
      ctx->split_scratch.clear();
    }
  }
  if (ctx->variant == kMfmaFilterVariant) {
    size_t missing = 0;
    for (size_t k = 0; k < num_streams; ++k) {
      bool have = false;
      for (auto &e : ctx->filter_scratch) have = have || e.stream == (hipStream_t)streams[k];
      missing += have ? 0 : 1;
    }
    if (missing != 0 && ctx->filter_scratch.size() + missing > 8) {
      ++ctx->host_syncs;
      HIP_TRY(hipDeviceSynchronize());
      std::vector<cuking_ctx::FilterScratch> keep;
      for (auto &e : ctx->filter_scratch) {
        bool named = false;
        for (size_t k = 0; k < num_streams; ++k) named = named || e.stream == (hipStream_t)streams[k];
        if (named) {
          keep.push_back(e);
        } else {
          retire_filter_totals(ctx, e);
          (void)hipFree(e.base);
        }
      }
      ctx->filter_scratch.swap(keep);
    }
  }
  for (size_t k = 0; k < num_streams; ++k) {
    uint32_t *scratch, *counters;
    st = split_scratch_for(ctx, (hipStream_t)streams[k], &scratch, &counters);
    if (st != CUKING_OK) return st;
    TiledArgs unused = {};
    st = filter_scratch_for(ctx, (hipStream_t)streams[k], geo, total_tiles(tiles), &unused);
    if (st != CUKING_OK) return st;
  }
  return CUKING_OK;
}

cuking_status cuking_invalidate(cuking_ctx *ctx) {
  if (ctx == nullptr) return cuking_fail(CUKING_ERR_INVALID_ARGUMENT, "null context");
  ctx->prepared.valid = false;
  return CUKING_OK;
}

cuking_status cuking_compute_counts(cuking_ctx *ctx, const cuking_submatrix *sm,
                                    uint32_t words_per_sample,
                                    const uint64_t *d_bit_sets,
                                    cuking_counts *d_counts, void *stream) {
  cuking_status st = bind(ctx);
  if (st != CUKING_OK) return st;
  st = check_compute_args(sm, words_per_sample, d_bit_sets);
  if (st != CUKING_OK) return st;
  if (sm_num_rows(*sm) == 0 || sm_num_cols(*sm) == 0) return CUKING_OK;
  if (d_counts == nullptr)
    return cuking_fail(CUKING_ERR_INVALID_ARGUMENT, "null counts pointer");
  if (ctx->kernel == CUKING_KERNEL_STREAM)
    return run_stream(ctx, *sm, words_per_sample, d_bit_sets, 0.f, 0, nullptr,
                      nullptr, nullptr, d_counts, (hipStream_t)stream);
  return run_tiled(ctx, *sm, words_per_sample, d_bit_sets, 0, 0, true, 0.f, 0,
                   nullptr, nullptr, nullptr, d_counts, (hipStream_t)stream);
}


cuking_status cuking_timing_enable(cuking_ctx *ctx, int enabled) {
  if (ctx == nullptr) return cuking_fail(CUKING_ERR_INVALID_ARGUMENT, "null context");
  ctx->timing = enabled != 0;
  return CUKING_OK;
}

cuking_status cuking_timing_reset(cuking_ctx *ctx) {
  if (ctx == nullptr) return cuking_fail(CUKING_ERR_INVALID_ARGUMENT, "null context");
  ctx->king_timer.used = 0;
  ctx->prepare_timer.used = 0;
  return CUKING_OK;
}

cuking_status cuking_timing_collect(cuking_ctx *ctx, double *king_ms,
                                    uint64_t *king_launches, double *prepare_ms,
                                    uint64_t *prepare_launches) {
  cuking_status st = bind(ctx);
  if (st != CUKING_OK) return st;
  double a = 0, b = 0;
  uint64_t na = 0, nb = 0;
  HIP_TRY(ctx->king_timer.collect(&a, &na));
  HIP_TRY(ctx->prepare_timer.collect(&b, &nb));
  if (king_ms) *king_ms = a;
  if (king_launches) *king_launches = na;
  if (prepare_ms) *prepare_ms = b;
  if (prepare_launches) *prepare_launches = nb;
  return CUKING_OK;
}

cuking_status cuking_clock_probe(cuking_ctx *ctx, uint64_t microseconds,
                                 uint64_t *d_ticks, void *stream) {
  cuking_status st = bind(ctx);
  if (st != CUKING_OK) return st;
  if (d_ticks == nullptr) return cuking_fail(CUKING_ERR_INVALID_ARGUMENT, "null out pointer");
  if (microseconds == 0 || microseconds > 60ull * 1000 * 1000)
    return cuking_fail(CUKING_ERR_INVALID_ARGUMENT, "probe time outside (0, 60 s]");
  HIP_TRY(launch_clock_probe(microseconds, d_ticks, (hipStream_t)stream));
  return CUKING_OK;
}


cuking_status cuking_synth_bitset(cuking_ctx *ctx, uint64_t seed,
                                  const uint32_t *d_kind, const uint32_t *d_pa,
                                  const uint32_t *d_pb, uint32_t sample_begin,
                                  uint32_t sample_end, uint32_t num_sites,
                                  uint32_t words_per_sample,
                                  uint64_t *d_bit_set, void *stream) {
  cuking_status st = bind(ctx);
  if (st != CUKING_OK) return st;
  if (sample_end < sample_begin)
    return cuking_fail(CUKING_ERR_INVALID_ARGUMENT, "sample range reversed");
  if (words_per_sample != cuking_words_per_sample(num_sites))
    return cuking_fail(CUKING_ERR_INVALID_ARGUMENT,
                "words_per_sample %u does not match %u sites", words_per_sample,
                num_sites);
  if (sample_end > sample_begin && (!d_kind || !d_pa || !d_pb || !d_bit_set))
    return cuking_fail(CUKING_ERR_INVALID_ARGUMENT, "null device pointer");
  HIP_TRY(launch_synth(seed, d_kind, d_pa, d_pb, sample_begin, sample_end,
                       num_sites, words_per_sample, d_bit_set,
                       (hipStream_t)stream));
  return CUKING_OK;
}

}
```

### cuking_amd/csrc/king_common.h

```cpp
#ifndef CUKING_AMD_KING_COMMON_H_
#define CUKING_AMD_KING_COMMON_H_

#include <hip/hip_runtime.h>
#include <stdint.h>

#include "cuking_amd.h"
#include "king_submatrix.h"

namespace cuking {

constexpr uint32_t kLayoutWord = 0;
constexpr uint32_t kLayoutQuad = 1;
constexpr uint32_t kLayoutNibble = 2;
constexpr uint32_t kLayoutNibbleStats = 3;

struct PlaneGeometry {
  uint32_t num_rows, num_cols;
  uint32_t rows_padded, cols_padded;
  uint32_t col_base;
  uint32_t s_stride;
  uint32_t k_words;
  uint32_t diag;
};

struct TileSpace {
  uint32_t tiles_r, tiles_c;
  uint32_t band_rows;
  uint32_t diag;

  __host__ __device__ uint32_t num_bands() const {
    return (tiles_r + band_rows - 1) / band_rows;
  }
  __host__ __device__ uint64_t band_tiles(uint32_t b) const {
    const uint32_t r0 = b * band_rows;
    const uint32_t h = (tiles_r - r0 < band_rows) ? tiles_r - r0 : band_rows;
    if (!diag) return (uint64_t)h * tiles_c;
    const uint32_t ncols = tiles_c - r0;
    return (uint64_t)h * (h + 1) / 2 + (uint64_t)(ncols - h) * h;
  }
  __host__ __device__ void decode(uint32_t b, uint64_t u, uint32_t *tr,
                                  uint32_t *tc) const {
    const uint32_t r0 = b * band_rows;
    const uint32_t h = (tiles_r - r0 < band_rows) ? tiles_r - r0 : band_rows;
    if (!diag) {
      *tc = (uint32_t)(u / h);
      *tr = r0 + (uint32_t)(u % h);
      return;
    }
    const uint64_t tri = (uint64_t)h * (h + 1) / 2;
    if (u < tri) {
      uint32_t c = 0;
      uint64_t before = 0;
      while (before + c + 1 <= u) {
        before += c + 1;
        ++c;
      }
      *tc = r0 + c;
      *tr = r0 + (uint32_t)(u - before);
    } else {
      const uint64_t v = u - tri;
      *tc = r0 + h + (uint32_t)(v / h);
      *tr = r0 + (uint32_t)(v % h);
    }
  }
};

struct TiledArgs {
  const uint4 *planes;
  PlaneGeometry geo;
  TileSpace tiles;
  const uint64_t *band_prefix;
  uint64_t tile_begin;
  uint32_t rect_rows, rect_cols, rect_row0, rect_col0, rect_row_stride;
  uint32_t i_begin, j_begin;
  float kin_threshold;
  uint32_t max_results;
  cuking_result *results;
  uint32_t *result_index;
  uint32_t *result_overflow;
  cuking_counts *dense_counts;
  const uint64_t *bits;
  uint32_t words_per_sample;
  uint32_t split_tiles, split_wgs;
  uint32_t split_whole;
  uint32_t *split_scratch, *split_counters;
  uint32_t xcd_chunk, launch_tiles;
  uint32_t dyn_tiles, dyn_wgs;
  uint32_t quad;
  const uint2 *tile_list;
  const uint32_t *tile_list_count;
  uint32_t tile_list_cap;
  const float2 *sample_stats;
  const uint4 *t2;
  uint32_t *filter_ctrl;
  unsigned long long *filter_totals;
  uint2 *cand_list;
  uint32_t cand_cap;
  uint32_t quadrant_cap;
  uint2 *dense_list;
  uint32_t dense_cap;
  uint32_t fsplit_parts, fsplit_first, fsplit_tile0;
  float4 *fsplit_slabs;
  uint32_t *fsplit_tickets;
  const uint32_t *check_steps;
  const float *prefix_u;
  const unsigned long long *cohort_sums;
  uint32_t check0, check1;
  uint32_t rotate, rotate_min_steps;
  uint32_t rotate_min_tiles;
  uint32_t persist_wgs;
  uint32_t persist_min_tiles;
  uint8_t *tile_done;
  const uint32_t *gate;
  uint32_t gate_count;
  const uint8_t *skip_tiles;
  uint64_t skip_base;
  const uint32_t *perm;
  uint32_t *codes_ready;
};

constexpr uint32_t kCheckEmitCap = 64;
constexpr uint32_t kNumCheckShares = 8;
constexpr uint32_t kCheckShares64[kNumCheckShares] = {8, 50, 53, 56, 58, 60, 61, 62};
constexpr uint32_t kNumPhases = 128;
constexpr uint32_t kPhasesPerShare = kNumPhases / 64;
constexpr uint32_t kNumCum = kNumPhases - 1;
__host__ __device__ inline uint32_t phase_step(uint32_t all_steps, uint32_t x) {
  return (uint32_t)((uint64_t)all_steps * x / kNumPhases);
}
__host__ __device__ inline uint32_t check_step_of(uint32_t all_steps, uint32_t k,
                                                  uint32_t min_steps = 64) {
  if (all_steps < min_steps) return 0;
  return phase_step(all_steps, kCheckShares64[k] * kPhasesPerShare);
}
constexpr uint32_t kFilterSplitSlabs = 256;
constexpr size_t kFilterSlabBytes = 256 * 256 * sizeof(float);
constexpr size_t kFilterTicketBytes = kFilterSplitSlabs * sizeof(uint32_t);
__host__ __device__ inline size_t plane_bytes(const PlaneGeometry &g,
                                              uint32_t layout) {
  const size_t base = (size_t)g.k_words * g.s_stride * (layout == kLayoutQuad ? 8 : 16);
  if (layout == kLayoutNibble) return base + base / 4;
  if (layout == kLayoutNibbleStats)
    return base + base / 4 + base / 2 + (size_t)g.s_stride * sizeof(float2) +
           (size_t)g.s_stride * kNumCum * sizeof(float) + 64 + 64 +
           64 + (size_t)g.s_stride * (4 + 8 + 4 * kNumCum + 16);
  return base;
}
__host__ __device__ inline const uint4 *plane_t2(const uint4 *planes, const PlaneGeometry &g) {
  return planes + (size_t)g.k_words * g.s_stride * 5 / 4;
}
__host__ __device__ inline const float2 *plane_stats(const uint4 *planes, const PlaneGeometry &g) {
  return reinterpret_cast<const float2 *>(planes + (size_t)g.k_words * g.s_stride * 7 / 4);
}
__host__ __device__ inline const float *plane_prefix_u(const uint4 *planes, const PlaneGeometry &g) {
  return reinterpret_cast<const float *>(plane_stats(planes, g) + g.s_stride);
}
__host__ __device__ inline const unsigned long long *plane_cohort_sums(const uint4 *planes,
                                                                       const PlaneGeometry &g) {
  return reinterpret_cast<const unsigned long long *>(plane_prefix_u(planes, g) +
                                                      (size_t)g.s_stride * kNumCum);
}

struct TiledVariant {
  const char *name;
  uint32_t tile;
  uint32_t k_chunk;
  uint32_t threads;
  uint32_t lds_bytes;
  uint32_t layout;
};

constexpr uint32_t kMfmaMaxSites = 1u << 24;

constexpr int kNumTiledVariants = 8;
constexpr int kMfmaVariant = 5;
constexpr int kMfmaN4Variant = 6;
constexpr uint32_t kMfmaN4MaxSites = 1u << 22;
constexpr int kMfmaN4Stages = 5;
constexpr uint32_t kMfmaN4LdsBytes = kMfmaN4Stages * 2 * 2 * 4 * 128 * 16;
static_assert(kMfmaN4LdsBytes <= 160 * 1024, "LDS of one CU");
constexpr int kMfmaFilterVariant = 7;
constexpr uint32_t kFilterTile = 256;
constexpr uint32_t kFilterLdsBytes = 5 * 2 * 2 * 2 * 256 * 16;
static_assert(kFilterLdsBytes <= 160 * 1024, "LDS of one CU");
constexpr uint32_t kFilterChunkTiles = 1u << 17;
constexpr uint32_t kFilterCandCap = 1u << 25;
constexpr uint32_t kFilterQuadrantCap = 384;
constexpr size_t kFilterCtrlBytes = 256;
constexpr uint32_t kCtrlCand = 0, kCtrlDense = 1, kCtrlDyn = 2, kCtrlFinished = 3,
                   kCtrlLeft = 4, kCtrlAllLeave = 5, kCtrlGate = 6;
constexpr uint32_t kCtrlStepTicks = 8, kCtrlPos = 16, kPosSlots = 16;
constexpr uint32_t kCtrlTickets = kCtrlPos + 8 * kPosSlots * 2;
constexpr size_t kCtrlChunkBytes = (kCtrlTickets + 16) * 4;
constexpr uint32_t kTotalCand = 0, kTotalDense = 1, kTotalEarly = 2, kTotalRotated = 3;
constexpr uint32_t kNumTotals = 4;
__host__ __device__ inline const uint32_t *plane_check_steps(const uint4 *planes,
                                                             const PlaneGeometry &g) {
  return reinterpret_cast<const uint32_t *>(plane_cohort_sums(planes, g) + 8);
}
__host__ __device__ inline uint32_t *plane_flags(const uint4 *planes, const PlaneGeometry &g) {
  return const_cast<uint32_t *>(plane_check_steps(planes, g)) + 16;
}
__host__ __device__ inline uint32_t *plane_perm(const uint4 *planes, const PlaneGeometry &g) {
  return plane_flags(planes, g) + 16;
}
__host__ __device__ inline float2 *plane_tmp_stats(const uint4 *planes, const PlaneGeometry &g) {
  return reinterpret_cast<float2 *>(plane_perm(planes, g) + g.s_stride);
}
__host__ __device__ inline float *plane_tmp_prefix(const uint4 *planes, const PlaneGeometry &g) {
  return reinterpret_cast<float *>(plane_tmp_stats(planes, g) + g.s_stride);
}
__host__ __device__ inline uint32_t *plane_sort_words(const uint4 *planes, const PlaneGeometry &g) {
  return reinterpret_cast<uint32_t *>(plane_tmp_prefix(planes, g) +
                                      (size_t)g.s_stride * kNumCum);
}
constexpr uint32_t kNoSample = 0xFFFFFFFFu;

struct FilterScratchLayout {
  size_t tile_done, totals, tickets, cand, dense, slabs, bytes;
  uint32_t chunk_tiles, cand_entries;
};
inline FilterScratchLayout filter_scratch_layout(uint64_t tiles) {
  FilterScratchLayout l;
  l.chunk_tiles = (uint32_t)(tiles < kFilterChunkTiles ? (tiles ? tiles : 1) : kFilterChunkTiles);
  const uint64_t cand = (uint64_t)l.chunk_tiles * 4 * 64;
  l.cand_entries = (uint32_t)(cand < kFilterCandCap ? cand : kFilterCandCap);
  auto up = [](size_t x) { return (x + 255) / 256 * 256; };
  l.tile_done = kCtrlChunkBytes;
  l.totals = up(l.tile_done + l.chunk_tiles);
  l.tickets = l.totals + kFilterCtrlBytes;
  l.cand = l.tickets + kFilterTicketBytes;
  l.dense = l.cand + up((size_t)l.cand_entries * sizeof(uint2));
  l.slabs = l.dense + up((size_t)l.chunk_tiles * 4 * sizeof(uint2));
  l.bytes = l.slabs + kFilterSplitSlabs * kFilterSlabBytes;
  return l;
}
inline bool is_mfma_variant(int v) {
  return v == kMfmaVariant || v == kMfmaN4Variant || v == kMfmaFilterVariant;
}
constexpr int kMfmaStages = 6;
constexpr uint32_t kMfmaLdsBytes = kMfmaStages * 2 * 2 * 2 * 128 * 16;
constexpr uint32_t kMfmaParkBytes = 4 * 64 * 64 * 4;
static_assert(kMfmaLdsBytes + kMfmaParkBytes <= 160 * 1024, "LDS of one CU");
const TiledVariant &tiled_variant(int v);
hipError_t launch_tiled(int variant, bool full, const TiledArgs &args,
                        uint64_t num_tiles, hipStream_t stream);
hipError_t launch_mfma(bool full, bool nibble, const TiledArgs &args, uint64_t num_tiles,
                       uint32_t lds_bytes, hipStream_t stream);
hipError_t launch_mfma_list(const TiledArgs &args, uint32_t grid, hipStream_t stream);
hipError_t launch_mfma_gated(const TiledArgs &args, uint64_t num_units, uint32_t grid,
                             hipStream_t stream);
hipError_t launch_filter(const TiledArgs &args, uint64_t num_tiles, hipStream_t stream);
hipError_t launch_sample_stats(const uint64_t *d_bit_sets, uint32_t words_per_sample,
                               const PlaneGeometry &geo, uint4 *d_planes, uint32_t s_begin,
                               uint32_t s_end, hipStream_t stream);
void set_filter_check_min_steps(uint32_t steps);
size_t sort_temp_bytes_for(uint32_t n);
hipError_t launch_sample_order(const PlaneGeometry &geo, uint32_t words_per_sample,
                               uint4 *d_planes, uint32_t s_begin, uint32_t s_end, bool sort,
                               void *sort_temp, size_t sort_temp_bytes, hipStream_t stream);
hipError_t launch_prepare_nibbles(bool codes, bool t2, const uint64_t *d_bit_sets,
                                  uint32_t words_per_sample, const PlaneGeometry &geo,
                                  uint4 *d_planes, const uint32_t *perm, uint32_t s_tile_begin,
                                  uint32_t s_tile_end, const uint32_t *gate,
                                  const uint32_t *ready, hipStream_t stream);
hipError_t launch_mark_codes_ready(const uint32_t *gate, uint32_t *ready, hipStream_t stream);
size_t mfma_split_scratch_bytes(uint32_t wgs);
size_t mfma_split_counter_bytes(uint32_t wgs);

void set_max_blocks_per_launch(uint64_t blocks);

hipError_t launch_prepare_planes(uint32_t layout, const uint64_t *d_bit_sets,
                                 uint32_t words_per_sample,
                                 const PlaneGeometry &geo, uint4 *d_planes,
                                 uint32_t s_tile_begin, uint32_t s_tile_end,
                                 hipStream_t stream);

hipError_t launch_stream(const cuking_submatrix &sm, uint32_t words_per_sample,
                         const uint64_t *d_bit_sets, float kin_threshold,
                         uint32_t max_results, cuking_result *d_results,
                         uint32_t *d_result_index, uint32_t *d_result_overflow,
                         cuking_counts *d_dense_counts, hipStream_t stream);

hipError_t launch_pack(const cuking_submatrix &sm, uint32_t words_per_sample,
                       uint64_t *d_bit_set, const int64_t *d_row_idx,
                       const int64_t *d_col_idx, const int32_t *d_n_alt,
                       size_t num_triples, uint32_t *d_status,
                       hipStream_t stream);

hipError_t launch_pack_compact(uint32_t words_per_sample, uint32_t num_samples,
                               uint64_t *d_bit_set, const uint32_t *d_site,
                               const uint32_t *d_sample_alt, size_t num_triples,
                               uint32_t *d_status, hipStream_t stream);

hipError_t launch_synth(uint64_t seed, const uint32_t *d_kind,
                        const uint32_t *d_pa, const uint32_t *d_pb,
                        uint32_t sample_begin, uint32_t sample_end,
                        uint32_t num_sites, uint32_t words_per_sample,
                        uint64_t *d_bit_set, hipStream_t stream);

hipError_t launch_clock_probe(uint64_t microseconds, uint64_t *d_out,
                              hipStream_t stream);

}

#endif
```

### cuking_amd/csrc/king_filter.hip

```cpp
#include <hip/hip_runtime.h>
#include <stdio.h>

#include <atomic>
#include <stdlib.h>

#include "king_common.h"
#include "king_device.h"

#pragma clang diagnostic ignored "-Winline-asm"

namespace cuking {

namespace {

typedef int v8i __attribute__((ext_vector_type(8)));
typedef float v16f __attribute__((ext_vector_type(16)));

constexpr int kT = (int)kFilterTile;
constexpr int kUnits = 2;
constexpr int kStages = 5;
constexpr int kSliceU4 = kT;
constexpr int kStageU4 = 2 * 2 * kUnits * kSliceU4;
constexpr int kStageReqs = 4 * kUnits;
constexpr int kSyncVm = (kStages - 3) * kStageReqs + (kStageReqs - 2);
static_assert(kSyncVm < 64, "vmcnt is a 6-bit counter");
static_assert(kStages * kStageU4 * 16 == (int)kFilterLdsBytes, "LDS size");
constexpr int vmcnt_imm(int n) { return 0x0F70 | (n & 15) | ((n >> 4) << 14); }
constexpr uint32_t kNoPair = 0xFFFFFFFFu;

__device__ __forceinline__ uint32_t source_sample(const PlaneGeometry &geo, uint32_t ps) {
  if (geo.diag || ps < geo.rows_padded) return ps < geo.num_rows ? ps : kNoPair;
  const uint32_t c = ps - geo.col_base;
  return c < geo.num_cols ? geo.num_rows + c : kNoPair;
}

struct CheckWords {
  uint32_t w[kNumCheckShares];
};
constexpr uint32_t kStatsMaxSteps = kMfmaN4MaxSites / 256;
__global__ __launch_bounds__(256) void sample_stats_kernel(
    const uint64_t *__restrict__ bits, uint32_t words_per_sample, PlaneGeometry geo,
    float2 *__restrict__ stats, float *__restrict__ cum, unsigned long long *__restrict__ sums,
    uint32_t *__restrict__ steps_out, CheckWords cw, uint32_t s_begin, uint32_t s_end) {
  __shared__ uint8_t phase_of[kStatsMaxSteps];
  __shared__ int32_t phase_sum[4][kNumPhases];
  const uint32_t lane = threadIdx.x & 63, wave = threadIdx.x >> 6;
  if (blockIdx.x == 0 && threadIdx.x < kNumCheckShares) steps_out[threadIdx.x] = cw.w[threadIdx.x];
  const uint32_t all_steps = geo.k_words / 8;
  for (uint32_t st = threadIdx.x; st < all_steps; st += 256) {
    const uint32_t x = (kNumPhases * (st + 1) - 1) / all_steps;
    phase_of[st] = (uint8_t)(x < kNumPhases ? x : kNumPhases - 1);
  }
#pragma unroll
  for (uint32_t k = 0; k < kNumPhases / 64; ++k) phase_sum[wave][lane + 64 * k] = 0;
  __syncthreads();
  const uint32_t ps = s_begin + blockIdx.x * 4 + wave;
  if (ps >= s_end) return;
  const uint32_t src = source_sample(geo, ps);
  int32_t yc = 0, mc = 0, hc = 0;
  if (src != kNoPair) {
    const uint32_t n = words_per_sample / 2;
    const uint64_t *het = bits + (uint64_t)src * words_per_sample;
    const uint64_t *hom = het + n;
    constexpr uint32_t kAhead = 4;
    for (uint32_t w0 = 0; w0 < n; w0 += 64 * kAhead) {
      uint64_t h[kAhead], v[kAhead];
#pragma unroll
      for (uint32_t k = 0; k < kAhead; ++k) {
        const uint32_t w = w0 + 64 * k + lane;
        const bool in = w < n;
        h[k] = in ? het[w] : 0ull;
        v[k] = in ? hom[w] : 0ull;
      }
#pragma unroll
      for (uint32_t k = 0; k < kAhead; ++k) {
        const uint32_t w = w0 + 64 * k + lane;
        const bool in = w < n;
        const int32_t y = in ? __popcll(~h[k]) : 0;
        const int32_t m = __popcll(h[k] & v[k]);
        yc += y;
        mc += m;
        hc += __popcll(h[k] & ~v[k]);
        int32_t d = y - m;
        d += __shfl_xor(d, 1);
        d += __shfl_xor(d, 2);
        if ((lane & 3) == 0 && in) atomicAdd(&phase_sum[wave][phase_of[w >> 2]], d);
      }
    }
#pragma unroll
    for (int off = 32; off > 0; off >>= 1) {
      yc += __shfl_xor(yc, off);
      mc += __shfl_xor(mc, off);
      hc += __shfl_xor(hc, off);
    }
  }
  static_assert(kNumPhases == 128, "two phases per lane");
  const int32_t p0 = phase_sum[wave][2 * lane], p1 = phase_sum[wave][2 * lane + 1];
  int32_t run = p0 + p1;
#pragma unroll
  for (int off = 1; off < 64; off <<= 1) {
    const int32_t up = __shfl_up(run, off);
    if ((int)lane >= off) run += up;
  }
  cum[(size_t)(2 * lane) * geo.s_stride + ps] = (float)(run - p1);
  if (2 * lane + 1 < kNumCum) cum[(size_t)(2 * lane + 1) * geo.s_stride + ps] = (float)run;
  if (lane == 0) {
    stats[ps] = make_float2((float)(yc - mc), (float)hc);
    if (src != kNoPair && ((blockIdx.x & 15) == 0 || gridDim.x < 64)) {
      __hip_atomic_fetch_add(sums, 1ull, __ATOMIC_RELAXED, __HIP_MEMORY_SCOPE_AGENT);
      __hip_atomic_fetch_add(sums + 1, (unsigned long long)mc, __ATOMIC_RELAXED,
                             __HIP_MEMORY_SCOPE_AGENT);
      __hip_atomic_fetch_add(sums + 2, (unsigned long long)hc, __ATOMIC_RELAXED,
                             __HIP_MEMORY_SCOPE_AGENT);
    }
  }
}

__device__ __forceinline__ v16f mma(const v8i a, const v8i b, const v16f c) {
  return __builtin_amdgcn_mfma_scale_f32_32x32x64_f8f6f4(a, b, c, 4 , 4, 0, 0, 0, 0);
}

__device__ __forceinline__ v8i tfrag(const uint4 w, uint32_t mask) {
  v8i r = {0, 0, 0, 0, 0, 0, 0, 0};
  r[0] = (int)(w.x & mask);
  r[1] = (int)(w.y & mask);
  r[2] = (int)(w.z & mask);
  r[3] = (int)(w.w & mask);
  return r;
}

__device__ __forceinline__ uint4 shl2(const uint4 w) {
  return make_uint4(w.x << 2, w.y << 2, w.z << 2, w.w << 2);
}

#define F_ISSUE(SRC, DST, OFF)                                                 \
  asm volatile("s_mov_b32 m0, %0\n\t"                                          \
               "s_nop 0\n\t"                                                   \
               "global_load_lds_dwordx4 %1, %2 offset:" #OFF                   \
               :                                                               \
               : "s"(DST), "v"(lane16), "s"(SRC)                               \
               : "memory", "m0")

__device__ __forceinline__ int filter_tile(const TiledArgs &a, const uint32_t wg, uint4 *const lds) {
  uint32_t bid = wg;
  const bool split = a.fsplit_parts != 0 && wg >= a.fsplit_first;
  uint32_t part = 0, piece = 0;
  if (split) {
    piece = wg - a.fsplit_first;
    part = __builtin_amdgcn_readfirstlane(piece % a.fsplit_parts);
    bid = a.fsplit_tile0 + piece / a.fsplit_parts;
  } else
  if (a.dyn_tiles != 0 && wg >= a.launch_tiles) {
    uint32_t *slot = reinterpret_cast<uint32_t *>(lds);
    if (threadIdx.x == 0)
      *slot = __hip_atomic_fetch_add(a.filter_ctrl + kCtrlDyn, 1u, __ATOMIC_RELAXED,
                                     __HIP_MEMORY_SCOPE_AGENT);
    __syncthreads();
    const uint32_t t = __builtin_amdgcn_readfirstlane(*slot);
    __syncthreads();
    if (t >= a.dyn_tiles) return 1;
    bid = a.launch_tiles + t;
  } else if (a.xcd_chunk == 1) {
    const uint32_t x = bid & 7, j = bid >> 3;
    bid = (((j >> 5) * 8 + x) << 5) + (j & 31);
    if (bid >= a.launch_tiles) return 0;
  }
  bid = __builtin_amdgcn_readfirstlane(bid);
  uint32_t tr, tc;
  if (!decode_tile_space(a, a.tile_begin + bid, &tr, &tc)) return 0;
  tr = __builtin_amdgcn_readfirstlane(tr);
  tc = __builtin_amdgcn_readfirstlane(tc);

  const uint32_t lane = threadIdx.x & 63;
  const uint32_t wave = __builtin_amdgcn_readfirstlane(threadIdx.x >> 6);
  const uint32_t wy = wave >> 1, wx = wave & 1;
  uint32_t xcd_pos = 0;
  if (!split && a.tile_done != nullptr) {
    uint32_t *verdict = reinterpret_cast<uint32_t *>(lds);
    if (threadIdx.x == 0) {
      uint32_t leave = __hip_atomic_load(a.filter_ctrl + kCtrlAllLeave, __ATOMIC_RELAXED,
                                         __HIP_MEMORY_SCOPE_AGENT);
      if (leave == 0 && a.cohort_sums != nullptr && a.check_steps != nullptr) {
        const float ns = (float)a.cohort_sums[0], nm = (float)a.cohort_sums[1],
                    nh = (float)a.cohort_sums[2];
        if (ns > 0.f && nh > 0.f) {
          const float sites = 32.f * (float)a.geo.k_words;
          const float m = nm / (ns * sites), h = nh / (ns * sites);
          if (m * (1.f + m / (2.f * h * (1.f - m))) - 4.f * rsqrtf(sites) > a.kin_threshold &&
              (a.check1 >> 16) != 0) {
            leave = 1;
            __hip_atomic_store(a.filter_ctrl + kCtrlAllLeave, 1u, __ATOMIC_RELAXED,
                               __HIP_MEMORY_SCOPE_AGENT);
            __hip_atomic_store(a.filter_ctrl + kCtrlGate, 1u, __ATOMIC_RELAXED,
                               __HIP_MEMORY_SCOPE_AGENT);
          }
        }
      }
      if (leave == 0) {
        const uint32_t dense_so_far =
            __hip_atomic_load(a.filter_ctrl + kCtrlDense, __ATOMIC_RELAXED, __HIP_MEMORY_SCOPE_AGENT) +
            __hip_atomic_load(a.filter_ctrl + kCtrlLeft, __ATOMIC_RELAXED, __HIP_MEMORY_SCOPE_AGENT);
        const uint32_t finished = __hip_atomic_load(a.filter_ctrl + kCtrlFinished, __ATOMIC_RELAXED,
                                                    __HIP_MEMORY_SCOPE_AGENT);
        if (finished >= 512 && 2 * dense_so_far > finished) {
          leave = 1;
          __hip_atomic_store(a.filter_ctrl + kCtrlAllLeave, 1u, __ATOMIC_RELAXED,
                             __HIP_MEMORY_SCOPE_AGENT);
          __hip_atomic_store(a.filter_ctrl + kCtrlGate, 1u, __ATOMIC_RELAXED,
                             __HIP_MEMORY_SCOPE_AGENT);
        }
      }
      verdict[0] = leave;
    }
    if (a.rotate == 1 && threadIdx.x < kPosSlots) {
      const uint32_t x = wg & 7;
      const unsigned long long said = __hip_atomic_load(
          reinterpret_cast<const unsigned long long *>(a.filter_ctrl + kCtrlPos) + x * kPosSlots +
              threadIdx.x,
          __ATOMIC_RELAXED, __HIP_MEMORY_SCOPE_AGENT);
      const uint32_t ticks16 = __hip_atomic_load(a.filter_ctrl + kCtrlStepTicks + x,
                                                 __ATOMIC_RELAXED, __HIP_MEMORY_SCOPE_AGENT);
      uint32_t pos = (uint32_t)(said >> 32);
      const uint32_t ago = (uint32_t)__builtin_amdgcn_s_memrealtime() - (uint32_t)said;
      if (said != 0 && ticks16 != 0 && ago < 16384u)
        pos += ago * 16u / ticks16;
      verdict[1 + threadIdx.x] = pos;
    }
    __syncthreads();
    const bool give_up = verdict[0] != 0;
    if (a.rotate == 1) {
#pragma unroll
      for (uint32_t k = 0; k < kPosSlots; ++k) xcd_pos = max(xcd_pos, verdict[1 + k]);
    }
    __syncthreads();
    if (give_up) {
      if (threadIdx.x == 0)
        __hip_atomic_fetch_add(a.filter_totals + kTotalDense, 4ull, __ATOMIC_RELAXED,
                               __HIP_MEMORY_SCOPE_AGENT);
      return 0;
    }
  }
  xcd_pos = __builtin_amdgcn_readfirstlane(xcd_pos);
  const uint32_t g = lane >> 5;
  const uint32_t lr = lane & 31;
  uint32_t lane16 = lane * 16;
  const uint32_t s_stride = a.geo.s_stride;
  const uint32_t all_steps = a.geo.k_words / (4 * kUnits);
  const uint32_t k_first = __builtin_amdgcn_readfirstlane(
      split ? part * all_steps / a.fsplit_parts : 0u);
  const uint32_t num_steps = __builtin_amdgcn_readfirstlane(
      split ? (part + 1) * all_steps / a.fsplit_parts - k_first : all_steps);
  const uint4 *g_rows = a.t2 + (uint64_t)tr * kT;
  const uint4 *g_cols = a.t2 + a.geo.col_base + (uint64_t)tc * kT;

  uint32_t mT;
  asm volatile("s_mov_b32 %0, 0xcccccccc" : "=s"(mT));

  const uint32_t dma_side = wave >> 1, dma_h = wave & 1;
  const uint32_t row_bytes = s_stride * 16;
  const char *const g_wave = reinterpret_cast<const char *>(
      (dma_side ? g_cols : g_rows) + ((uint64_t)2 * kUnits * k_first + kUnits * dma_h) * s_stride);
  const uint32_t l_wave = (uint32_t)(uintptr_t)(lds_void_ptr)(
      lds + ((dma_side * 2 + dma_h) * kUnits) * kSliceU4);
  struct Addr { const char *src; uint32_t dst; };
  const uint32_t kstep_bytes = 2 * kUnits * row_bytes;
  const char *seg_src = g_wave;
  uint32_t seg_steps = num_steps;
  uint32_t seg_wrap = 0xFFFFFFFFu;
  auto addr_of = [&](uint32_t step, uint32_t buf) {
    Addr pa;
    if (step >= seg_steps) step = seg_steps - 1;
    const int32_t rel = (int32_t)step - (int32_t)(step >= seg_wrap ? all_steps : 0u);
    pa.src = seg_src + (int64_t)rel * (int64_t)kstep_bytes;
    pa.dst = l_wave + buf * (kStageU4 * 16);
    asm volatile("" : "+s"(pa.src), "+s"(pa.dst));
    return pa;
  };
  auto addr_next = [&](const Addr &cur, uint32_t step, uint32_t buf) {
    Addr pa;
    const int32_t adv = (int32_t)(step < seg_steps ? 1u : 0u) -
                        (int32_t)(step == seg_wrap ? all_steps : 0u);
    pa.src = cur.src + (int64_t)adv * (int64_t)kstep_bytes;
    pa.dst = l_wave + buf * (kStageU4 * 16);
    asm volatile("" : "+s"(pa.src), "+s"(pa.dst));
    return pa;
  };
#define F_ISSUE4(PA, C)                                                        \
  {                                                                            \
    const char *src_ = (PA).src + (C) * row_bytes;                             \
    const uint32_t dst_ = (PA).dst + (C) * (kSliceU4 * 16);                    \
    F_ISSUE(src_, dst_, 0);                                                    \
    F_ISSUE(src_, dst_, 1024);                                                 \
    F_ISSUE(src_, dst_, 2048);                                                 \
    F_ISSUE(src_, dst_, 3072);                                                 \
  }

  v16f acc[4][4];
#pragma unroll
  for (int bi = 0; bi < 4; ++bi)
#pragma unroll
    for (int bj = 0; bj < 4; ++bj)
#pragma unroll
      for (int r = 0; r < 16; ++r) acc[bi][bj][r] = 0.f;

  uint32_t row_off = ((0 * 2 + g) * kUnits) * kSliceU4 + wy * 128 + lr;
  uint32_t col_off = ((1 * 2 + g) * kUnits) * kSliceU4 + wx * 128 + lr;
  asm volatile("" : "+v"(row_off), "+v"(col_off), "+v"(lane16));
  v8i FA[2][4], FB[2][4];
  uint4 RAW[8];
#define F_READ(K, BUF, C)                                                      \
  RAW[K] = lds[(BUF) * kStageU4 + ((K) < 4 ? row_off : col_off) + (C) * kSliceU4 + ((K) & 3) * 32];
#define F_PIN4(W) asm volatile("" : "+v"((W).x), "+v"((W).y), "+v"((W).z), "+v"((W).w));
#define F_PINF(F) asm volatile("" : "+v"((F)[0]), "+v"((F)[1]), "+v"((F)[2]), "+v"((F)[3]));
#define F_BUILD_B(NXT, K)                                                      \
  F_PIN4(RAW[K])                                                               \
  if ((K) < 4) {                                                               \
    FA[NXT][(K) & 3] = tfrag(RAW[K], mT);                                      \
    F_PINF(FA[NXT][(K) & 3])                                                   \
  } else {                                                                     \
    FB[NXT][(K) & 3] = tfrag(RAW[K], mT);                                      \
    F_PINF(FB[NXT][(K) & 3])                                                   \
  }
#define F_BUILD_A(NXT, K)                                                      \
  F_PIN4(RAW[K])                                                               \
  if ((K) < 4) {                                                               \
    FA[NXT][(K) & 3] = tfrag(shl2(RAW[K]), mT);                                \
    F_PINF(FA[NXT][(K) & 3])                                                   \
  } else {                                                                     \
    FB[NXT][(K) & 3] = tfrag(shl2(RAW[K]), mT);                                \
    F_PINF(FB[NXT][(K) & 3])                                                   \
  }
#define F_MMA(CUR, BI, BJ) acc[BI][BJ] = mma(FA[CUR][BI], FB[CUR][BJ], acc[BI][BJ]);
#define F_BAR __builtin_amdgcn_sched_barrier(0);
#define F_SLICE_B(CUR, NXT, PA, DC, OFF0, OFF1)                                \
  {                                                                            \
    const char *src_ = (PA).src + (DC) * row_bytes;                            \
    const uint32_t dst_ = (PA).dst + (DC) * (kSliceU4 * 16);                   \
    F_ISSUE(src_, dst_, OFF0);                                                 \
    F_MMA(CUR, 0, 0) F_BAR                                                     \
    F_BUILD_A(NXT, 0) F_MMA(CUR, 0, 1) F_BAR                                   \
    F_MMA(CUR, 0, 2) F_BAR                                                     \
    F_BUILD_A(NXT, 1) F_MMA(CUR, 0, 3) F_BAR                                   \
    F_MMA(CUR, 1, 0) F_BAR                                                     \
    F_BUILD_A(NXT, 2) F_MMA(CUR, 1, 1) F_BAR                                   \
    F_MMA(CUR, 1, 2) F_BAR                                                     \
    F_BUILD_A(NXT, 3) F_MMA(CUR, 1, 3) F_BAR                                   \
    F_ISSUE(src_, dst_, OFF1);                                                 \
    F_MMA(CUR, 2, 0) F_BAR                                                     \
    F_BUILD_A(NXT, 4) F_MMA(CUR, 2, 1) F_BAR                                   \
    F_MMA(CUR, 2, 2) F_BAR                                                     \
    F_BUILD_A(NXT, 5) F_MMA(CUR, 2, 3) F_BAR                                   \
    F_MMA(CUR, 3, 0) F_BAR                                                     \
    F_BUILD_A(NXT, 6) F_MMA(CUR, 3, 1) F_BAR                                   \
    F_MMA(CUR, 3, 2) F_BAR                                                     \
    F_BUILD_A(NXT, 7) F_MMA(CUR, 3, 3) F_BAR                                   \
  }
#define F_SLICE_A(CUR, NXT, RBUF, RC, SYNC, PA, DC, OFF0, OFF1)                \
  {                                                                            \
    if (SYNC) {                                                                \
      __builtin_amdgcn_s_waitcnt(vmcnt_imm(kSyncVm));                          \
      __syncthreads();                                                         \
    }                                                                          \
    const char *src_ = (PA).src + (DC) * row_bytes;                            \
    const uint32_t dst_ = (PA).dst + (DC) * (kSliceU4 * 16);                   \
    F_READ(0, RBUF, RC) F_READ(1, RBUF, RC)                                    \
    F_ISSUE(src_, dst_, OFF0);                                                 \
    F_MMA(CUR, 0, 0) F_MMA(CUR, 0, 1) F_BAR                                    \
    F_READ(2, RBUF, RC) F_READ(3, RBUF, RC)                                    \
    F_MMA(CUR, 0, 2) F_MMA(CUR, 0, 3) F_BAR                                    \
    F_READ(4, RBUF, RC) F_READ(5, RBUF, RC)                                    \
    F_ISSUE(src_, dst_, OFF1);                                                 \
    F_MMA(CUR, 1, 0) F_MMA(CUR, 1, 1) F_BAR                                    \
    F_READ(6, RBUF, RC) F_READ(7, RBUF, RC)                                    \
    F_MMA(CUR, 1, 2) F_MMA(CUR, 1, 3) F_BAR                                    \
    F_BUILD_B(NXT, 0) F_MMA(CUR, 2, 0) F_BAR                                   \
    F_BUILD_B(NXT, 1) F_MMA(CUR, 2, 1) F_BAR                                   \
    F_BUILD_B(NXT, 2) F_MMA(CUR, 2, 2) F_BAR                                   \
    F_BUILD_B(NXT, 3) F_MMA(CUR, 2, 3) F_BAR                                   \
    F_BUILD_B(NXT, 4) F_MMA(CUR, 3, 0) F_BAR                                   \
    F_BUILD_B(NXT, 5) F_MMA(CUR, 3, 1) F_BAR                                   \
    F_BUILD_B(NXT, 6) F_MMA(CUR, 3, 2) F_BAR                                   \
    F_BUILD_B(NXT, 7) F_MMA(CUR, 3, 3) F_BAR                                   \
  }
#define F_KSTEP                                                                \
  {                                                                            \
    const uint32_t nbuf = buf == kStages - 1 ? 0 : buf + 1;                    \
    F_SLICE_B(0, 1, pa, 0, 0, 1024)                                            \
    F_SLICE_A(1, 0, buf, 1, false, pa, 0, 2048, 3072)                          \
    F_SLICE_B(0, 1, pa, 1, 0, 1024)                                            \
    F_SLICE_A(1, 0, nbuf, 0, true, pa, 1, 2048, 3072)                          \
    pa = addr_next(pa, step + kStages, buf);                                   \
    buf = nbuf;                                                                \
    ++step;                                                                    \
  }

  uint32_t chk0 = 0, chk1 = 0, entry1 = 0, share1 = 0;
  uint32_t phase = 0, k0 = 0, wrap = 0, start_abs = 0;
  if (!split && a.check_steps != nullptr && a.tile_done != nullptr) {
    if (a.rotate != 0 && all_steps >= a.rotate_min_steps) {
      uint32_t base = 0;
      if (a.rotate == 1) {
        const uint32_t r = xcd_pos % all_steps;
        base = xcd_pos - r;
        phase = (r * kNumPhases + all_steps / 2) / all_steps;
        if (phase >= kNumPhases) {
          phase = 0;
          base += all_steps;
        }
      } else if (a.rotate == 2) {
        phase = (bid * 37u + 11u) & (kNumPhases - 1);
      } else {
        phase = (a.rotate - 3u) & (kNumPhases - 1);
      }
      k0 = phase_step(all_steps, phase);
      start_abs = base + k0;
      wrap = k0 != 0 ? all_steps - k0 : 0u;
    }
    float kappa = -1.f;
    {
      const float ns = (float)a.cohort_sums[0], nm = (float)a.cohort_sums[1],
                  nh = (float)a.cohort_sums[2];
      if (ns > 0.f && nh > 0.f) {
        const float sites = 256.f * (float)all_steps;
        const float m = nm / (ns * sites), h = nh / (ns * sites);
        kappa = m * (1.f + m / (2.f * h * (1.f - m))) + 4.6f * rsqrtf(sites) + 0.003f;
      }
    }
    auto steps_of = [&](uint32_t share) {
      const uint32_t hi = phase + share * kPhasesPerShare;
      return hi <= kNumPhases ? phase_step(all_steps, hi) - k0
                              : (all_steps - k0) + phase_step(all_steps, hi - kNumPhases);
    };
    if ((a.check0 == 2 || (a.check0 == 1 && kappa > 0.7f * a.kin_threshold)) &&
        a.check_steps[0] != 0)
      chk0 = steps_of(kCheckShares64[0]);
    const uint32_t sw1 = a.check1 & 0xFFu;
    if (sw1 >= 2) {
      entry1 = sw1 - 2;
    } else if (sw1 == 1 && kappa >= 0.f) {
      const float f64 = 64.f * (1.f - 2.f * a.kin_threshold) / (1.f - 2.f * kappa);
      if (f64 <= 62.f) {
        share1 = (uint32_t)ceilf(f64);
        if (share1 < 32) share1 = 32;
        entry1 = 1;
      }
    }
#pragma unroll
    for (uint32_t k = 1; k < kNumCheckShares; ++k)
      if (sw1 >= 2 && k == entry1) share1 = kCheckShares64[k];
    if (share1 != 0 && a.check_steps[entry1] != 0) chk1 = steps_of(share1);
    if (chk0 >= num_steps) chk0 = 0;
    if (chk1 >= num_steps || chk1 <= chk0) chk1 = 0;
  }
  chk0 = __builtin_amdgcn_readfirstlane(chk0);
  chk1 = __builtin_amdgcn_readfirstlane(chk1);
  share1 = __builtin_amdgcn_readfirstlane(share1);
  phase = __builtin_amdgcn_readfirstlane(phase);
  k0 = __builtin_amdgcn_readfirstlane(k0);
  wrap = __builtin_amdgcn_readfirstlane(wrap);
  start_abs = __builtin_amdgcn_readfirstlane(start_abs);
  auto prefix_u_of = [&](uint32_t share, size_t idx, float total) {
    const uint32_t hi = phase + share * kPhasesPerShare;
    const uint32_t xb = hi > kNumPhases ? hi - kNumPhases : hi;
    float u = hi > kNumPhases ? total : 0.f;
    if (xb == kNumPhases)
      u += total;
    else if (xb != 0)
      u += a.prefix_u[(size_t)(xb - 1) * s_stride + idx];
    if (phase != 0) u -= a.prefix_u[(size_t)(phase - 1) * s_stride + idx];
    return u;
  };
  unsigned long long *const pos_word =
      reinterpret_cast<unsigned long long *>(a.filter_ctrl + kCtrlPos) +
      (wg & 7) * kPosSlots + ((wg >> 3) & (kPosSlots - 1));
  uint32_t *const ticks_word = a.filter_ctrl + kCtrlStepTicks + (wg & 7);
  const uint32_t t_start = a.rotate == 1 ? (uint32_t)__builtin_amdgcn_s_memrealtime() : 0u;
#define F_PUBLISH(STEPS)                                                       \
  if (a.rotate == 1 && wave == 0) {                                            \
    const uint32_t now_ = (uint32_t)__builtin_amdgcn_s_memrealtime();          \
    const unsigned long long val_ =                                            \
        ((unsigned long long)(start_abs + (STEPS)) << 32) | now_;              \
     \
    const uint32_t t16_ = (STEPS) >= 32 ? (now_ - t_start) * 16u / (STEPS) : 0u; \
    const uint32_t zero_ = 0;                                                  \
    unsigned long long save_;                                                  \
    asm volatile("s_mov_b64 %0, exec\n\t"                                      \
                 "s_mov_b64 exec, 1\n\t"                                       \
                 "global_store_dwordx2 %1, %2, %3\n\t"                         \
                 "s_mov_b64 exec, %0"                                          \
                 : "=&s"(save_)                                                \
                 : "v"(zero_), "v"(val_), "s"(pos_word)                        \
                 : "memory");                                                  \
    if (t16_ != 0)                                                             \
      asm volatile("s_mov_b64 %0, exec\n\t"                                    \
                   "s_mov_b64 exec, 1\n\t"                                     \
                   "global_store_dword %1, %2, %3\n\t"                         \
                   "s_mov_b64 exec, %0"                                        \
                   : "=&s"(save_)                                              \
                   : "v"(zero_), "v"(t16_), "s"(ticks_word)                    \
                   : "memory");                                                \
  }

  uint32_t seg_first = 0;
  bool left = false, left_forecast = false, left_emit = false;
#pragma nounroll
  while (true) {
    uint32_t seg_end = num_steps;
    if (chk1 > seg_first) seg_end = chk1;
    if (chk0 > seg_first) seg_end = chk0;
    seg_end = __builtin_amdgcn_readfirstlane(seg_end);
    seg_steps = seg_end - seg_first;
    const uint32_t seg_k = seg_first >= wrap && wrap != 0 ? seg_first - wrap : k0 + seg_first;
    seg_src = g_wave + (uint64_t)seg_k * kstep_bytes;
    seg_wrap = __builtin_amdgcn_readfirstlane(
        wrap > seg_first && wrap < seg_end ? wrap - seg_first : 0xFFFFFFFFu);
    asm volatile("" : "+s"(seg_src), "+s"(seg_steps), "+s"(seg_wrap));

#pragma unroll
    for (int st = 0; st < kStages - 1; ++st) {
      const Addr p0 = addr_of(st, st);
      F_ISSUE4(p0, 0)
      F_ISSUE4(p0, 1)
    }
    __builtin_amdgcn_s_waitcnt(vmcnt_imm((kStages - 2) * kStageReqs));
    __syncthreads();
#pragma unroll
    for (int k = 0; k < 8; ++k) {
      F_READ(k, 0, 0)
    }
#pragma unroll
    for (int k = 0; k < 8; ++k) {
      F_BUILD_B(0, k)
    }
    uint32_t buf = 0;
    Addr pa = addr_of(kStages - 1, kStages - 1);
    uint32_t step = 0;
    while (step + 1 < seg_steps) {
      F_KSTEP
      F_KSTEP
    }
    if (step < seg_steps) F_KSTEP
    __builtin_amdgcn_s_waitcnt(0x0F70);
    __syncthreads();
    F_PUBLISH(seg_end)
    if (seg_end == num_steps) break;

    const bool forecast = seg_end == chk0;
    const float scale = forecast ? (float)kCheckShares64[0] * (1.f / 64.f) : 1.f;
    float2 *const ck_rows = reinterpret_cast<float2 *>(lds);
    float2 *const ck_cols = ck_rows + kT;
    uint32_t *const ck_words = reinterpret_cast<uint32_t *>(ck_cols + kT);
    {
      const uint32_t share = forecast ? kCheckShares64[0] : share1;
      const float thr_f = forecast ? a.kin_threshold + 3.66f * rsqrtf(256.f * (float)all_steps)
                                   : a.kin_threshold;
      const float t = 2.f - 4.f * thr_f;
      const size_t ir = (size_t)tr * kT + threadIdx.x;
      const size_t ic = (size_t)a.geo.col_base + (size_t)tc * kT + threadIdx.x;
      const float2 sr = a.sample_stats[ir], sc = a.sample_stats[ic];
      ck_rows[threadIdx.x] = make_float2(prefix_u_of(share, ir, sr.x), scale * fmaf(t, sr.y, 8.f));
      ck_cols[threadIdx.x] = make_float2(prefix_u_of(share, ic, sc.x), scale * fmaf(t, sc.y, 8.f));
    }
    __syncthreads();
    const uint32_t emit_cap = (a.check1 >> 8) & 0xFFu;
    uint32_t cnt = 0;
    {
      float2 cc[4];
#pragma unroll
      for (int bj = 0; bj < 4; ++bj) cc[bj] = ck_cols[wx * 128 + bj * 32 + lr];
#pragma unroll
      for (int bi = 0; bi < 4; ++bi)
#pragma unroll
        for (int r = 0; r < 16; ++r) {
          const float2 cr = ck_rows[wy * 128 + bi * 32 + (r & 3) + 8 * (r >> 2) + 4 * g];
#pragma unroll
          for (int bj = 0; bj < 4; ++bj)
            cnt += fmaf(-0.5f, acc[bi][bj][r], cr.x + cc[bj].x) < fminf(cr.y, cc[bj].y) ? 1u : 0u;
        }
    }
#pragma unroll
    for (int off = 32; off > 0; off >>= 1) cnt += __shfl_xor(cnt, off);
    if (lane == 0)
      ck_words[wave] = forecast ? (cnt > 2 * a.quadrant_cap ? 1u : 0u)
                                : (cnt > emit_cap ? emit_cap + 1 : cnt);
    __syncthreads();
    uint32_t found = forecast ? ck_words[0] + ck_words[1] + ck_words[2] + ck_words[3]
                              : max(max(ck_words[0], ck_words[1]), max(ck_words[2], ck_words[3]));
    found = __builtin_amdgcn_readfirstlane(found);
    __syncthreads();
    if (forecast ? found >= 3 : found <= emit_cap) {
      left = true;
      left_forecast = forecast;
      left_emit = !forecast && found != 0;
      break;
    }
    seg_first = seg_end;
  }
#undef F_KSTEP
#undef F_SLICE_A
#undef F_SLICE_B
#undef F_BAR
#undef F_MMA
#undef F_BUILD_A
#undef F_BUILD_B
#undef F_PIN4
#undef F_PINF
#undef F_READ
#undef F_ISSUE4
#undef F_PUBLISH
  if (left && left_emit && threadIdx.x == 0)
    __hip_atomic_fetch_add(a.filter_totals + kTotalEarly, 1ull, __ATOMIC_RELAXED,
                           __HIP_MEMORY_SCOPE_AGENT);
  if (phase != 0 && threadIdx.x == 0)
    __hip_atomic_fetch_add(a.filter_totals + kTotalRotated, 1ull, __ATOMIC_RELAXED,
                           __HIP_MEMORY_SCOPE_AGENT);
  if (left && !left_emit) {
    if (threadIdx.x == 0) {
      __hip_atomic_fetch_add(a.filter_ctrl + kCtrlFinished, 4u, __ATOMIC_RELAXED,
                             __HIP_MEMORY_SCOPE_AGENT);
      if (left_forecast) {
        __hip_atomic_fetch_add(a.filter_ctrl + kCtrlLeft, 4u, __ATOMIC_RELAXED,
                               __HIP_MEMORY_SCOPE_AGENT);
        __hip_atomic_store(a.filter_ctrl + kCtrlGate, 1u, __ATOMIC_RELAXED,
                           __HIP_MEMORY_SCOPE_AGENT);
        __hip_atomic_fetch_add(
            a.filter_totals + kTotalDense, 4ull,
            __ATOMIC_RELAXED, __HIP_MEMORY_SCOPE_AGENT);
      } else {
        a.tile_done[bid] = 1;
        __hip_atomic_fetch_add(
            a.filter_totals + kTotalEarly, 1ull,
            __ATOMIC_RELAXED, __HIP_MEMORY_SCOPE_AGENT);
      }
    }
    return 0;
  }

  if (!split && a.tile_done != nullptr && threadIdx.x == 0) a.tile_done[bid] = 1;

  if (split) {
    typedef uint32_t v4u __attribute__((ext_vector_type(4)));
    constexpr uint32_t kSlabU4 = 64 * 256;
    {
      const __amdgpu_buffer_rsrc_t rsrc = __builtin_amdgcn_make_buffer_rsrc(
          a.fsplit_slabs + (size_t)piece * kSlabU4, 0, (int)(kSlabU4 * 16), 0x00020000);
#pragma unroll
      for (int bi = 0; bi < 4; ++bi)
#pragma unroll
        for (int bj = 0; bj < 4; ++bj)
#pragma unroll
          for (int r4 = 0; r4 < 4; ++r4) {
            v4u v;
            v[0] = __float_as_uint(acc[bi][bj][4 * r4]);
            v[1] = __float_as_uint(acc[bi][bj][4 * r4 + 1]);
            v[2] = __float_as_uint(acc[bi][bj][4 * r4 + 2]);
            v[3] = __float_as_uint(acc[bi][bj][4 * r4 + 3]);
            __builtin_amdgcn_raw_buffer_store_b128(
                v, rsrc, (int)((((bi * 4 + bj) * 4 + r4) * 256 + threadIdx.x) * 16), 0,
                16 );
          }
    }
    asm volatile("s_waitcnt vmcnt(0)" ::: "memory");
    __syncthreads();
    uint32_t *flag = reinterpret_cast<uint32_t *>(lds);
    if (threadIdx.x == 0) {
      uint32_t *counter = a.fsplit_tickets + piece / a.fsplit_parts;
      const uint32_t ticket = __hip_atomic_fetch_add(counter, 1u, __ATOMIC_RELAXED,
                                                     __HIP_MEMORY_SCOPE_AGENT);
      const bool last = ticket == a.fsplit_parts - 1;
      if (last) {
        __builtin_amdgcn_fence(__ATOMIC_ACQUIRE, "agent");
        asm volatile("s_waitcnt vmcnt(0)" ::: "memory");
        *counter = 0;
      }
      *flag = last ? 1u : 0u;
    }
    __syncthreads();
    const bool last = *flag != 0;
    __syncthreads();
    if (!last) return 0;
    const uint32_t first_piece = piece - part;
    for (uint32_t p = 0; p < a.fsplit_parts; ++p) {
      if (p == part) continue;
      const float4 *src = a.fsplit_slabs + (size_t)(first_piece + p) * kSlabU4 + threadIdx.x;
#pragma unroll
      for (int bi = 0; bi < 4; ++bi)
#pragma unroll
        for (int bj = 0; bj < 4; ++bj)
#pragma unroll
          for (int r4 = 0; r4 < 4; ++r4) {
            const float4 v = src[((bi * 4 + bj) * 4 + r4) * 256];
            acc[bi][bj][4 * r4] += v.x;
            acc[bi][bj][4 * r4 + 1] += v.y;
            acc[bi][bj][4 * r4 + 2] += v.z;
            acc[bi][bj][4 * r4 + 3] += v.w;
          }
    }
  }

  float2 *const st_rows = reinterpret_cast<float2 *>(lds);
  float2 *const st_cols = st_rows + kT;
  {
    const float t = 2.f - 4.f * a.kin_threshold;
    const size_t ir = (size_t)tr * kT + threadIdx.x;
    const size_t ic = (size_t)a.geo.col_base + (size_t)tc * kT + threadIdx.x;
    float2 r = a.sample_stats[ir];
    float2 c = a.sample_stats[ic];
    if (left_emit) {
      r.x = prefix_u_of(share1, ir, r.x);
      c.x = prefix_u_of(share1, ic, c.x);
    }
    r.y = fmaf(t, r.y, 8.f);
    c.y = fmaf(t, c.y, 8.f);
    st_rows[threadIdx.x] = r;
    st_cols[threadIdx.x] = c;
  }
  __syncthreads();
  float2 sc[4];
#pragma unroll
  for (int bj = 0; bj < 4; ++bj) sc[bj] = st_cols[wx * 128 + bj * 32 + lr];

  {
    float best = -1.f;
#pragma unroll
    for (int bi = 0; bi < 4; ++bi)
#pragma unroll
      for (int r = 0; r < 16; ++r) {
        const float2 sr = st_rows[wy * 128 + bi * 32 + (r & 3) + 8 * (r >> 2) + 4 * g];
#pragma unroll
        for (int bj = 0; bj < 4; ++bj)
          best = fmaxf(best, fminf(sr.y, sc[bj].y) -
                                 fmaf(-0.5f, acc[bi][bj][r], sr.x + sc[bj].x));
      }
    if (__ballot(best > 0.f) == 0) {
      if (lane == 0)
        __hip_atomic_fetch_add(a.filter_ctrl + kCtrlFinished, 1u, __ATOMIC_RELAXED, __HIP_MEMORY_SCOPE_AGENT);
      return 0;
    }
  }
  if (lane == 0)
    __hip_atomic_fetch_add(a.filter_ctrl + kCtrlFinished, 1u, __ATOMIC_RELAXED, __HIP_MEMORY_SCOPE_AGENT);

  uint32_t total = 0, base = 0, run = 0;
#pragma nounroll
  for (int pass = 0; pass < 2; ++pass) {
    uint32_t tr_p = tr, tc_p = tc;
    asm volatile("" : "+s"(tr_p), "+s"(tc_p));
#pragma unroll
    for (int bi = 0; bi < 4; ++bi) {
#pragma unroll
      for (int r = 0; r < 16; ++r) {
        const uint32_t row = wy * 128 + bi * 32 + (r & 3) + 8 * (r >> 2) + 4 * g;
        const float2 sr = st_rows[row];
        const uint32_t li = tr_p * kT + row;
#pragma unroll
        for (int bj = 0; bj < 4; ++bj) {
          const uint32_t lj = tc_p * kT + wx * 128 + bj * 32 + lr;
          const bool valid = li < a.geo.num_rows && lj < a.geo.num_cols &&
                             a.i_begin + li < a.j_begin + lj;
          const float x_lb = fmaf(-0.5f, acc[bi][bj][r], sr.x + sc[bj].x);
          const bool cand = valid && x_lb < fminf(sr.y, sc[bj].y);
          const unsigned long long b = __ballot(cand);
          if (b != 0) {
            if (pass == 0) {
              total += (uint32_t)__popcll(b);
            } else {
              const uint32_t before = __builtin_amdgcn_mbcnt_hi(
                  (uint32_t)(b >> 32), __builtin_amdgcn_mbcnt_lo((uint32_t)b, 0u));
              if (cand) a.cand_list[base + run + before] = make_uint2(li, lj);
              run += (uint32_t)__popcll(b);
            }
          }
        }
      }
    }
    if (pass == 0) {
      if (total == 0) break;
      bool dense = total > a.quadrant_cap;
      if (!dense) {
        uint32_t got = 0;
        if (lane == 0) {
          got = __hip_atomic_fetch_add(a.filter_ctrl, total, __ATOMIC_RELAXED,
                                       __HIP_MEMORY_SCOPE_AGENT);
          __hip_atomic_fetch_add(a.filter_totals + kTotalCand,
                                 (unsigned long long)total, __ATOMIC_RELAXED,
                                 __HIP_MEMORY_SCOPE_AGENT);
        }
        base = (uint32_t)__builtin_amdgcn_readfirstlane(got);
        if (base >= a.cand_cap || total > a.cand_cap - base) {
          for (uint32_t k = base + lane; k < a.cand_cap; k += 64)
            a.cand_list[k] = make_uint2(kNoPair, kNoPair);
          dense = true;
        }
      }
      if (dense) {
        if (lane == 0) {
          const uint32_t slot = __hip_atomic_fetch_add(a.filter_ctrl + kCtrlDense, 1u, __ATOMIC_RELAXED,
                                                       __HIP_MEMORY_SCOPE_AGENT);
          if (slot < a.dense_cap) a.dense_list[slot] = make_uint2(2 * tr + wy, 2 * tc + wx);
          __hip_atomic_fetch_add(a.filter_totals + kTotalDense, 1ull,
                                 __ATOMIC_RELAXED, __HIP_MEMORY_SCOPE_AGENT);
        }
        break;
      }
    }
  }
  return 0;
}

__global__ __launch_bounds__(256, 1) void king_filter_kernel(const TiledArgs a) {
  extern __shared__ uint4 lds[];
  (void)filter_tile(a, blockIdx.x, lds);
}

__global__ __launch_bounds__(256, 1) void king_filter_persistent_kernel(const TiledArgs a) {
  extern __shared__ uint4 lds[];
  const uint32_t x = blockIdx.x & 7;
  bool tail = false;
  for (;;) {
    uint32_t wg = a.launch_tiles + x;
    if (!tail) {
      uint32_t *slot = reinterpret_cast<uint32_t *>(lds);
      if (threadIdx.x == 0)
        *slot = __hip_atomic_fetch_add(a.filter_ctrl + kCtrlTickets + x, 1u, __ATOMIC_RELAXED,
                                       __HIP_MEMORY_SCOPE_AGENT);
      __syncthreads();
      const uint32_t j = __builtin_amdgcn_readfirstlane(*slot);
      __syncthreads();
      if (j * 8 + x < a.persist_wgs) {
        wg = j * 8 + x;
      } else {
        if (a.dyn_tiles == 0) break;
        tail = true;
      }
    }
    if (filter_tile(a, wg, lds) != 0) break;
    __syncthreads();
  }
}

__global__ __launch_bounds__(256) void king_refine_kernel(const TiledArgs a) {
  const uint32_t lane = threadIdx.x & 63;
  uint32_t count = *a.filter_ctrl;
  if (count > a.cand_cap) count = a.cand_cap;
  const uint32_t n = a.words_per_sample / 2;
  const uint32_t stride = gridDim.x * 4;
  for (uint32_t p = blockIdx.x * 4 + (threadIdx.x >> 6); p < count; p += stride) {
    const uint2 e = a.cand_list[p];
    if (e.x == kNoPair) continue;
    const uint32_t off_i = a.perm != nullptr ? a.perm[e.x] : e.x;
    const uint32_t off_j = a.perm != nullptr ? a.perm[a.geo.col_base + e.y]
                                             : (a.geo.diag ? e.y : a.geo.num_rows + e.y);
    const uint64_t *het_i_w = a.bits + (uint64_t)off_i * a.words_per_sample;
    const uint64_t *alt_i_w = het_i_w + n;
    const uint64_t *het_j_w = a.bits + (uint64_t)off_j * a.words_per_sample;
    const uint64_t *alt_j_w = het_j_w + n;
    uint32_t s_het_i = 0, s_het_j = 0, s_both = 0, s_opp = 0, s_conc = 0, s_shared = 0;
    constexpr uint32_t kAhead = 8;
    for (uint32_t w0 = 0; w0 < n; w0 += 64 * kAhead) {
      uint64_t hi[kAhead], ai[kAhead], hj[kAhead], aj[kAhead];
#pragma unroll
      for (uint32_t k = 0; k < kAhead; ++k) {
        const uint32_t w = w0 + 64 * k + lane;
        const bool in = w < n;
        hi[k] = in ? het_i_w[w] : ~0ull;
        ai[k] = in ? alt_i_w[w] : ~0ull;
        hj[k] = in ? het_j_w[w] : ~0ull;
        aj[k] = in ? alt_j_w[w] : ~0ull;
      }
#pragma unroll
      for (uint32_t k = 0; k < kAhead; ++k) {
        const uint64_t ri = ~(hi[k] | ai[k]), rj = ~(hj[k] | aj[k]);
        const uint64_t defined = ~((hi[k] & ai[k]) | (hj[k] & aj[k]));
        s_het_i += __popcll(hi[k] & defined);
        s_het_j += __popcll(hj[k] & defined);
        s_both += __popcll(hi[k] & hj[k] & defined);
        s_opp += __popcll(((ri & aj[k]) | (ai[k] & rj)) & defined);
        s_conc += __popcll(((ri & rj) | (ai[k] & aj[k])) & defined);
        s_shared += __popcll(defined);
      }
    }
#pragma unroll
    for (int off = 32; off > 0; off >>= 1) {
      s_het_i += __shfl_xor(s_het_i, off);
      s_het_j += __shfl_xor(s_het_j, off);
      s_both += __shfl_xor(s_both, off);
      s_opp += __shfl_xor(s_opp, off);
      s_conc += __shfl_xor(s_conc, off);
      s_shared += __shfl_xor(s_shared, off);
    }
    if (lane == 0) {
      const float kin = king_kinship(s_het_i, s_het_j, s_both, s_opp);
      if (kin > a.kin_threshold) {
        const uint32_t ibs0 = s_opp, ibs2 = s_conc + s_both;
        const uint32_t gi = a.i_begin + off_i;
        const uint32_t gj = a.geo.diag ? a.j_begin + off_j : a.j_begin + (off_j - a.geo.num_rows);
        emit_result(gi < gj ? gi : gj, gi < gj ? gj : gi, kin, ibs0, s_shared - ibs0 - ibs2, ibs2,
                    a.max_results, a.results, a.result_index, a.result_overflow);
      }
    }
  }
}

}

static std::atomic<uint32_t> g_check_min_steps{64};
void set_filter_check_min_steps(uint32_t steps) { g_check_min_steps.store(steps); }

hipError_t launch_sample_stats(const uint64_t *d_bit_sets, uint32_t words_per_sample,
                               const PlaneGeometry &geo, uint4 *d_planes, uint32_t s_begin,
                               uint32_t s_end, hipStream_t stream) {
  if (s_end > geo.s_stride) s_end = geo.s_stride;
  if (s_begin >= s_end) return hipSuccess;
  float2 *stats = plane_tmp_stats(d_planes, geo);
  float *prefix = plane_tmp_prefix(d_planes, geo);
  unsigned long long *sums = const_cast<unsigned long long *>(plane_cohort_sums(d_planes, geo));
  uint32_t *steps = const_cast<uint32_t *>(plane_check_steps(d_planes, geo));
  CheckWords cw;
  const uint32_t all_steps = geo.k_words / 8;
  if (all_steps > kStatsMaxSteps) return hipErrorInvalidValue;
  for (uint32_t k = 0; k < kNumCheckShares; ++k)
    cw.w[k] = check_step_of(all_steps, k, g_check_min_steps.load());
  sample_stats_kernel<<<dim3((s_end - s_begin + 3) / 4), dim3(256), 0, stream>>>(
      d_bit_sets, words_per_sample, geo, stats, prefix, sums, steps, cw, s_begin, s_end);
  return hipGetLastError();
}

hipError_t launch_filter(const TiledArgs &args, uint64_t num_tiles, hipStream_t stream) {
  if ((uint64_t)args.geo.k_words * 32 > kMfmaN4MaxSites || args.filter_ctrl == nullptr ||
      args.cand_list == nullptr || args.dense_list == nullptr || args.sample_stats == nullptr)
    return hipErrorInvalidValue;
  static DeviceOnce attr_set;
  if (!attr_set.done()) {
    hipError_t e = hipFuncSetAttribute(reinterpret_cast<const void *>(king_filter_kernel),
                                       hipFuncAttributeMaxDynamicSharedMemorySize,
                                       (int)kFilterLdsBytes);
    if (e != hipSuccess) return e;
    e = hipFuncSetAttribute(reinterpret_cast<const void *>(king_filter_persistent_kernel),
                            hipFuncAttributeMaxDynamicSharedMemorySize, (int)kFilterLdsBytes);
    if (e != hipSuccess) return e;
    attr_set.mark();
  }
  uint64_t cap = max_blocks_per_launch(256);
  if (cap > kFilterChunkTiles) cap = kFilterChunkTiles;
  if (cap > args.dense_cap / 4) cap = args.dense_cap / 4;
  if (cap == 0) return hipErrorInvalidValue;
  const uint32_t wgs = args.split_wgs != 0 ? args.split_wgs : 256;
  uint64_t done = 0;
  while (done < num_tiles) {
    const uint64_t n = num_tiles - done < cap ? num_tiles - done : cap;
    const bool checks = args.tile_done != nullptr;
    hipError_t e = hipMemsetAsync(args.filter_ctrl, 0, kCtrlChunkBytes + (checks ? n : 0), stream);
    if (e != hipSuccess) return e;
    TiledArgs a = args;
    a.tile_begin = args.tile_begin + done;
    a.quad = 0;
    a.tile_list = nullptr;
    a.gate = nullptr;
    a.skip_tiles = nullptr;
    a.check0 = !checks ? 0u : args.check0 == 2 ? 2u : (args.check0 == 1 && n < 16ull * wgs) ? 1u : 0u;
    a.check1 = checks ? args.check1 : 0u;
    a.rotate = checks && (n >= args.rotate_min_tiles || args.rotate >= 2) ? args.rotate : 0u;
    uint32_t rest = 0, parts = 0;
    if (args.fsplit_slabs != nullptr && args.fsplit_tickets != nullptr && n < 16ull * wgs) {
      rest = (uint32_t)(n % wgs);
      if (rest != 0 && 2 * rest <= wgs && rest <= kFilterSplitSlabs / 2) {
        parts = wgs / rest;
        if (parts > 8) parts = 8;
        if (parts * rest > kFilterSplitSlabs) parts = kFilterSplitSlabs / rest;
        const uint32_t min_steps = args.fsplit_first != 0 ? args.fsplit_first : 8;
        while (parts > 1 && args.geo.k_words / 8 / parts < min_steps) --parts;
      }
      if (parts < 2) rest = parts = 0;
    }
    const uint64_t n_whole = n - rest;
    uint64_t grid = n_whole;
    a.dyn_tiles = a.dyn_wgs = 0;
    if (args.xcd_chunk == 2 && args.dyn_tiles != 0 && n_whole >= args.dyn_tiles / 4 &&
        n_whole >= 288) {
      const uint64_t fixed = (n_whole - n_whole / 16) / 256 * 256;
      a.launch_tiles = (uint32_t)fixed;
      a.xcd_chunk = 1;
      a.dyn_tiles = (uint32_t)(n_whole - fixed);
      a.dyn_wgs = a.dyn_tiles + a.dyn_tiles / 2;
      grid = fixed + a.dyn_wgs;
    } else if (args.xcd_chunk == 2 && n_whole >= 64) {
      a.launch_tiles = (uint32_t)n_whole;
      a.xcd_chunk = 1;
      grid = 8ull * 32 * ((((n_whole + 31) / 32) + 7) / 8);
    } else {
      a.xcd_chunk = 0;
      a.launch_tiles = (uint32_t)n_whole;
    }
    a.fsplit_parts = parts;
    a.fsplit_tile0 = (uint32_t)n_whole;
    a.fsplit_first = (uint32_t)grid;
    grid += (uint64_t)rest * parts;
    if (checks && rest != 0) {
      e = hipMemsetAsync(args.tile_done + n_whole, 1, rest, stream);
      if (e != hipSuccess) return e;
    }
    a.persist_wgs = 0;
    if (args.persist_wgs != 0 && rest == 0 && n >= args.persist_min_tiles) {
      a.persist_wgs = (uint32_t)(a.dyn_tiles != 0 ? a.launch_tiles : grid);
      king_filter_persistent_kernel<<<dim3(wgs), dim3(256), kFilterLdsBytes, stream>>>(a);
    } else {
      king_filter_kernel<<<dim3((uint32_t)grid), dim3(256), kFilterLdsBytes, stream>>>(a);
    }
    e = hipGetLastError();
    if (e != hipSuccess) return e;
    king_refine_kernel<<<dim3(wgs * 4), dim3(256), 0, stream>>>(a);
    e = hipGetLastError();
    if (e != hipSuccess) return e;
    if (a.codes_ready != nullptr) {
      e = launch_prepare_nibbles(true, false, a.bits, a.words_per_sample, a.geo,
                                 const_cast<uint4 *>(a.planes), a.perm, 0, 0xFFFFFFFFu,
                                 a.filter_ctrl, a.codes_ready, stream);
      if (e != hipSuccess) return e;
      e = launch_mark_codes_ready(a.filter_ctrl, a.codes_ready, stream);
      if (e != hipSuccess) return e;
    }
    TiledArgs d = a;
    d.tile_list = a.dense_list;
    d.tile_list_count = a.filter_ctrl + kCtrlDense;
    d.tile_list_cap = a.dense_cap;
    e = launch_mfma_list(d, wgs, stream);
    if (e != hipSuccess) return e;
    if (checks) {
      TiledArgs f = a;
      f.quad = 1;
      f.tile_begin = a.tile_begin * 4;
      f.gate = a.filter_ctrl + kCtrlGate;
      f.skip_tiles = a.tile_done;
      f.skip_base = a.tile_begin;
      e = launch_mfma_gated(f, n * 4, wgs, stream);
      if (e != hipSuccess) return e;
    }
    done += n;
  }
  return hipSuccess;
}

}
```

### cuking_amd/csrc/king_sort.hip

```cpp
#include <hip/hip_runtime.h>

#include <hipcub/hipcub.hpp>

#include "king_common.h"

namespace cuking {

namespace {

__global__ void sort_keys_kernel(const float2 *__restrict__ tmp_stats, uint32_t begin, uint32_t n,
                                 float stored_sites, uint32_t *__restrict__ keys,
                                 uint32_t *__restrict__ vals) {
  const uint32_t p = blockIdx.x * blockDim.x + threadIdx.x;
  if (p >= n) return;
  const float2 st = tmp_stats[begin + p];
  const float missing = 0.5f * (stored_sites - st.y - st.x);
  uint32_t key = (uint32_t)(missing * 64.f / stored_sites);
  keys[p] = key > 255u ? 255u : key;
  vals[p] = begin + p;
}

__global__ void identity_order_kernel(uint32_t begin, uint32_t n, uint32_t *__restrict__ vals) {
  const uint32_t p = blockIdx.x * blockDim.x + threadIdx.x;
  if (p < n) vals[p] = begin + p;
}

__global__ void apply_order_kernel(PlaneGeometry geo, uint32_t begin, uint32_t end, uint32_t n,
                                   const uint32_t *__restrict__ order,
                                   const float2 *__restrict__ tmp_stats,
                                   const float *__restrict__ tmp_prefix,
                                   uint32_t *__restrict__ perm, float2 *__restrict__ stats,
                                   float *__restrict__ prefix) {
  const uint32_t p = begin + blockIdx.x * blockDim.x + threadIdx.x;
  if (p >= end) return;
  if (p - begin >= n) {
    perm[p] = kNoSample;
    stats[p] = make_float2(0.f, 0.f);
#pragma unroll
    for (uint32_t c = 0; c < kNumCum; ++c) prefix[(size_t)c * geo.s_stride + p] = 0.f;
    return;
  }
  const uint32_t src = order[p - begin];
  perm[p] = (geo.diag || src < geo.rows_padded) ? src : geo.num_rows + (src - geo.col_base);
  stats[p] = tmp_stats[src];
#pragma unroll 7
  for (uint32_t c = 0; c < kNumCum; ++c)
    prefix[(size_t)c * geo.s_stride + p] = tmp_prefix[(size_t)c * geo.s_stride + src];
}

}

size_t sort_temp_bytes_for(uint32_t n) {
  size_t bytes = 0;
  uint32_t *nil = nullptr;
  if (n == 0) return 0;
  (void)hipcub::DeviceRadixSort::SortPairs(nullptr, bytes, nil, nil, nil, nil, (int)n, 0, 8);
  return (bytes + 255) / 256 * 256;
}

hipError_t launch_sample_order(const PlaneGeometry &geo, uint32_t words_per_sample,
                               uint4 *d_planes, uint32_t s_begin, uint32_t s_end, bool sort,
                               void *sort_temp, size_t sort_temp_bytes, hipStream_t stream) {
  if (s_end > geo.s_stride) s_end = geo.s_stride;
  if (s_begin >= s_end) return hipSuccess;
  const float2 *tmp_stats = plane_tmp_stats(d_planes, geo);
  const float *tmp_prefix = plane_tmp_prefix(d_planes, geo);
  uint32_t *perm = plane_perm(d_planes, geo);
  float2 *stats = const_cast<float2 *>(plane_stats(d_planes, geo));
  float *prefix = const_cast<float *>(plane_prefix_u(d_planes, geo));
  uint32_t *words = plane_sort_words(d_planes, geo);
  const float stored_sites = 32.f * (float)words_per_sample;
  struct Side { uint32_t begin, end, real_end; };
  Side sides[2];
  int num_sides = 0;
  if (geo.diag) {
    sides[num_sides++] = {0, geo.rows_padded, geo.num_rows};
  } else {
    sides[num_sides++] = {0, geo.rows_padded, geo.num_rows};
    sides[num_sides++] = {geo.col_base, geo.col_base + geo.cols_padded, geo.col_base + geo.num_cols};
  }
  for (int k = 0; k < num_sides; ++k) {
    const uint32_t b = s_begin > sides[k].begin ? s_begin : sides[k].begin;
    const uint32_t e = s_end < sides[k].end ? s_end : sides[k].end;
    if (b >= e) continue;
    const uint32_t real_e = e < sides[k].real_end ? e : sides[k].real_end;
    const uint32_t n = real_e > b ? real_e - b : 0;
    uint32_t *keys_in = words + b, *keys_out = words + geo.s_stride + b;
    uint32_t *vals_in = words + 2 * (size_t)geo.s_stride + b;
    uint32_t *vals_out = words + 3 * (size_t)geo.s_stride + b;
    const uint32_t *order = vals_in;
    if (n != 0) {
      if (sort) {
        sort_keys_kernel<<<dim3((n + 255) / 256), dim3(256), 0, stream>>>(
            tmp_stats, b, n, stored_sites, keys_in, vals_in);
        hipError_t e0 = hipGetLastError();
        if (e0 != hipSuccess) return e0;
        size_t bytes = sort_temp_bytes;
        e0 = hipcub::DeviceRadixSort::SortPairs(sort_temp, bytes, keys_in, keys_out, vals_in,
                                                vals_out, (int)n, 0, 8, stream);
        if (e0 != hipSuccess) return e0;
        order = vals_out;
      } else {
        identity_order_kernel<<<dim3((n + 255) / 256), dim3(256), 0, stream>>>(b, n, vals_in);
        hipError_t e0 = hipGetLastError();
        if (e0 != hipSuccess) return e0;
      }
    }
    apply_order_kernel<<<dim3((e - b + 255) / 256), dim3(256), 0, stream>>>(
        geo, b, e, n, order, tmp_stats, tmp_prefix, perm, stats, prefix);
    hipError_t e1 = hipGetLastError();
    if (e1 != hipSuccess) return e1;
  }
  return hipSuccess;
}

}
```

Before: 37.43 billion.

## Reorder sites by population mass to tighten the early-exit filter bound

Result: faster. 41.52 billion, median of 6 (+10.9%).

```diff
diff --git a/cuking_amd/build.py b/cuking_amd/build.py
--- a/cuking_amd/build.py
+++ b/cuking_amd/build.py
@@ -18,6 +18,7 @@
 LIB_FLAGS_PATH = PKG / "libcuking_amd.flags"
 
 HIP_SOURCES = ["king_abi.hip", "king_kernels.hip", "king_mfma.hip", "king_filter.hip",
+               "king_site_order.hip",
                "king_sort.hip", "synth.hip"]
 HOST_ABI_SOURCES = ["king_host.cc"]
 HIP_FLAGS = [
diff --git a/cuking_amd/csrc/king_abi.hip b/cuking_amd/csrc/king_abi.hip
--- a/cuking_amd/csrc/king_abi.hip
+++ b/cuking_amd/csrc/king_abi.hip
@@ -101,6 +101,7 @@
     uint64_t tiles;
   };
   std::vector<FilterScratch> filter_scratch;
+  hipStream_t filter_last_stream = nullptr;
   unsigned long long filter_totals_retired[kNumTotals] = {};
   uint32_t filter_quadrant_cap = kFilterQuadrantCap;
   uint32_t filter_cand_cap = kFilterCandCap;
@@ -112,6 +113,8 @@
   bool filter_persistent = false;
   uint32_t filter_persistent_min_tiles = 2048;
   int filter_sort = 1;
+  int filter_site_order = 1;
+  uint64_t site_ordered_blocks = 0;
   bool filter_lazy_codes = true;
   void *sort_temp = nullptr;
   size_t sort_temp_bytes = 0;
@@ -124,6 +127,7 @@
     uint32_t tile = 0;
     const uint64_t *bits = nullptr;
     bool codes = true;
+    bool site_ordered = false;
     std::vector<uint8_t> tiles;
     hipStream_t ordered_on = nullptr;
     bool ordered_valid = false;
@@ -313,6 +317,7 @@
     }
   }
   uint8_t *base = entry->base;
+  ctx->filter_last_stream = stream;
   const FilterScratchLayout l = filter_scratch_layout(entry->tiles);
   a->sample_stats = plane_stats(ctx->planes, geo);
   a->t2 = plane_t2(ctx->planes, geo);
@@ -345,9 +350,11 @@
                       TiledArgs *a) {
   a->perm = nullptr;
   a->codes_ready = nullptr;
+  a->site_mass = nullptr;
   if (plan_variant(ctx, words_per_sample).layout != kLayoutNibbleStats) return;
   a->perm = plane_perm(ctx->planes, geo);
   if (!ctx->prepared.codes) a->codes_ready = plane_flags(ctx->planes, geo);
+  a->site_mass = ctx->prepared.site_ordered ? plane_site_mass(ctx->planes, geo) : nullptr;
 }
 
 hipError_t launch_planned(const cuking_ctx *ctx, uint32_t words_per_sample, bool full,
@@ -542,6 +549,7 @@
     pr.bits = d_bit_sets;
     pr.tiles.assign(all_tiles, 0);
     pr.codes = true;
+    pr.site_ordered = false;
   }
   for (uint32_t t = s_tile_begin; t < t_end; ++t)
     must_wait = must_wait || pr.tiles[t] == 2 || (pr.tiles[t] == 1 && other_stream);
@@ -566,13 +574,31 @@
       HIP_TRY(hipMemsetAsync(const_cast<unsigned long long *>(plane_cohort_sums(ctx->planes, geo)),
                              0, 64, stream));
     HIP_TRY(hipMemsetAsync(plane_flags(ctx->planes, geo), 0, sizeof(uint32_t), stream));
-    HIP_TRY(launch_sample_stats(d_bit_sets, words_per_sample, geo, ctx->planes, sb, se, stream));
+    const bool site_order_fits = geo.k_words >= 8 && (uint64_t)geo.k_words * 32 <= kSiteOrderMaxSites;
+    const uint32_t stored = geo.diag ? geo.num_rows : geo.num_rows + geo.num_cols;
+    if (whole)
+      pr.site_ordered = site_order_fits && (ctx->filter_site_order == 2 ||
+                                            (ctx->filter_site_order == 1 && stored >= kSiteOrderMinSamples));
+    HIP_TRY(launch_sample_stats(d_bit_sets, words_per_sample, geo, ctx->planes, sb, se,
+                                !pr.site_ordered, stream));
     HIP_TRY(launch_sample_order(geo, words_per_sample, ctx->planes, sb, se,
                                 ctx->filter_sort == 2 || (ctx->filter_sort == 1 && whole),
-                                ctx->sort_temp, ctx->sort_temp_bytes, stream));
-    HIP_TRY(launch_prepare_nibbles(codes, true, d_bit_sets, words_per_sample, geo, ctx->planes,
-                                   plane_perm(ctx->planes, geo), s_tile_begin, t_end, nullptr,
-                                   nullptr, stream));
+                                !pr.site_ordered, ctx->sort_temp, ctx->sort_temp_bytes, stream));
+    if (pr.site_ordered) {
+      if (whole) {
+        HIP_TRY(launch_site_order(d_bit_sets, words_per_sample, geo, ctx->planes, stream));
+        ++ctx->site_ordered_blocks;
+      }
+      if (codes)
+        HIP_TRY(launch_prepare_nibbles(true, false, d_bit_sets, words_per_sample, geo,
+                                       ctx->planes, plane_perm(ctx->planes, geo), s_tile_begin,
+                                       t_end, nullptr, nullptr, stream));
+      HIP_TRY(launch_gather_t2(d_bit_sets, words_per_sample, geo, ctx->planes, sb, se, stream));
+    } else {
+      HIP_TRY(launch_prepare_nibbles(codes, true, d_bit_sets, words_per_sample, geo, ctx->planes,
+                                     plane_perm(ctx->planes, geo), s_tile_begin, t_end, nullptr,
+                                     nullptr, stream));
+    }
     if (!codes) {
       pr.codes = false;
     } else if (!pr.codes) {
@@ -824,6 +850,13 @@
     ctx->prepared.valid = false;
     return CUKING_OK;
   }
+  if (strcmp(key, "filter_site_order") == 0) {
+    if (value < 0 || value > 2)
+      return cuking_fail(CUKING_ERR_INVALID_ARGUMENT, "filter_site_order outside [0, 2]");
+    if (ctx->filter_site_order != (int)value) ctx->prepared.valid = false;
+    ctx->filter_site_order = (int)value;
+    return CUKING_OK;
+  }
   if (strcmp(key, "filter_lazy_codes") == 0) {
     if (value < 0 || value > 1)
       return cuking_fail(CUKING_ERR_INVALID_ARGUMENT, "filter_lazy_codes outside [0, 1]");
@@ -1111,6 +1144,21 @@
   else if (strcmp(key, "filter_split_min_steps") == 0) *value = ctx->filter_split_min_steps;
   else if (strcmp(key, "filter_sort") == 0) *value = ctx->filter_sort;
   else if (strcmp(key, "filter_lazy_codes") == 0) *value = ctx->filter_lazy_codes ? 1 : 0;
+  else if (strcmp(key, "filter_site_order") == 0) *value = ctx->filter_site_order;
+  else if (strcmp(key, "filter_site_ordered") == 0) *value = (int64_t)ctx->site_ordered_blocks;
+  else if (strcmp(key, "filter_site_order_active") == 0)
+    *value = ctx->prepared.valid && ctx->prepared.site_ordered ? 1 : 0;
+  else if (strcmp(key, "filter_check_share") == 0) {
+    if (hipSetDevice(ctx->device) != hipSuccess || hipDeviceSynchronize() != hipSuccess)
+      return cuking_fail(CUKING_ERR_DEVICE, "device wait failed");
+    unsigned long long v = 0;
+    for (auto &e : ctx->filter_scratch)
+      if (e.stream == ctx->filter_last_stream && e.base != nullptr &&
+          hipMemcpy(&v, e.base + filter_scratch_layout(e.tiles).totals + kTotalShare * 8, 8,
+                    hipMemcpyDeviceToHost) != hipSuccess)
+        return cuking_fail(CUKING_ERR_DEVICE, "reading the filter counters failed");
+    *value = (int64_t)v;
+  }
   else if (strcmp(key, "filter_check0") == 0) *value = ctx->filter_check0;
   else if (strcmp(key, "filter_check1") == 0) *value = ctx->filter_check1;
   else if (strcmp(key, "filter_check_emit") == 0) *value = ctx->filter_check_emit;
diff --git a/cuking_amd/csrc/king_common.h b/cuking_amd/csrc/king_common.h
--- a/cuking_amd/csrc/king_common.h
+++ b/cuking_amd/csrc/king_common.h
@@ -117,6 +117,7 @@
   uint64_t skip_base;
   const uint32_t *perm;
   uint32_t *codes_ready;
+  const float *site_mass;
 };
 
 constexpr uint32_t kCheckEmitCap = 64;
@@ -136,6 +137,18 @@
 constexpr uint32_t kFilterSplitSlabs = 256;
 constexpr size_t kFilterSlabBytes = 256 * 256 * sizeof(float);
 constexpr size_t kFilterTicketBytes = kFilterSplitSlabs * sizeof(uint32_t);
+constexpr uint32_t kSiteWindowUnits = 16;
+constexpr uint32_t kSiteOrderMinSamples = 32768;
+constexpr uint32_t kSiteOrderMaxSites = 1u << 21;
+constexpr uint32_t kSiteWindowSites = kSiteWindowUnits * 64;
+__host__ __device__ inline size_t site_order_bytes(const PlaneGeometry &g) {
+  const size_t sites = (size_t)g.k_words * 32;
+  return 512 + 64 + sites * 8 + (sites * 2 + 255) / 256 * 256 + sites / 64 * 4 + 256;
+}
+__host__ __device__ inline uint32_t site_order_unit(uint32_t j, uint32_t w, uint32_t windows,
+                                                    uint32_t last) {
+  return j < last ? j * windows + w : last * windows + (j - last) * (windows - 1) + w;
+}
 __host__ __device__ inline size_t plane_bytes(const PlaneGeometry &g,
                                               uint32_t layout) {
   const size_t base = (size_t)g.k_words * g.s_stride * (layout == kLayoutQuad ? 8 : 16);
@@ -143,7 +156,8 @@
   if (layout == kLayoutNibbleStats)
     return base + base / 4 + base / 2 + (size_t)g.s_stride * sizeof(float2) +
            (size_t)g.s_stride * kNumCum * sizeof(float) + 64 + 64 +
-           64 + (size_t)g.s_stride * (4 + 8 + 4 * kNumCum + 16);
+           64 + (size_t)g.s_stride * (4 + 8 + 4 * kNumCum + 16) +
+           site_order_bytes(g);
   return base;
 }
 __host__ __device__ inline const uint4 *plane_t2(const uint4 *planes, const PlaneGeometry &g) {
@@ -194,6 +208,7 @@
 constexpr size_t kCtrlChunkBytes = (kCtrlTickets + 16) * 4;
 constexpr uint32_t kTotalCand = 0, kTotalDense = 1, kTotalEarly = 2, kTotalRotated = 3;
 constexpr uint32_t kNumTotals = 4;
+constexpr uint32_t kTotalShare = 4;
 __host__ __device__ inline const uint32_t *plane_check_steps(const uint4 *planes,
                                                              const PlaneGeometry &g) {
   return reinterpret_cast<const uint32_t *>(plane_cohort_sums(planes, g) + 8);
@@ -215,6 +230,20 @@
                                       (size_t)g.s_stride * kNumCum);
 }
 constexpr uint32_t kNoSample = 0xFFFFFFFFu;
+__host__ __device__ inline float *plane_site_mass(const uint4 *planes, const PlaneGeometry &g) {
+  return reinterpret_cast<float *>(plane_sort_words(planes, g) + 4 * (size_t)g.s_stride);
+}
+__host__ __device__ inline unsigned long long *plane_site_counts(const uint4 *planes,
+                                                                 const PlaneGeometry &g) {
+  return reinterpret_cast<unsigned long long *>(plane_site_mass(planes, g) + kNumPhases + 16);
+}
+__host__ __device__ inline uint16_t *plane_site_local(const uint4 *planes, const PlaneGeometry &g) {
+  return reinterpret_cast<uint16_t *>(plane_site_counts(planes, g) + (size_t)g.k_words * 32);
+}
+__host__ __device__ inline float *plane_unit_mass(const uint4 *planes, const PlaneGeometry &g) {
+  return reinterpret_cast<float *>(plane_site_local(planes, g) +
+                                   ((size_t)g.k_words * 32 * 2 + 255) / 256 * 128);
+}
 
 struct FilterScratchLayout {
   size_t tile_done, totals, tickets, cand, dense, slabs, bytes;
@@ -253,17 +282,23 @@
 hipError_t launch_filter(const TiledArgs &args, uint64_t num_tiles, hipStream_t stream);
 hipError_t launch_sample_stats(const uint64_t *d_bit_sets, uint32_t words_per_sample,
                                const PlaneGeometry &geo, uint4 *d_planes, uint32_t s_begin,
-                               uint32_t s_end, hipStream_t stream);
+                               uint32_t s_end, bool prefix, hipStream_t stream);
 void set_filter_check_min_steps(uint32_t steps);
 size_t sort_temp_bytes_for(uint32_t n);
 hipError_t launch_sample_order(const PlaneGeometry &geo, uint32_t words_per_sample,
                                uint4 *d_planes, uint32_t s_begin, uint32_t s_end, bool sort,
-                               void *sort_temp, size_t sort_temp_bytes, hipStream_t stream);
+                               bool prefix, void *sort_temp, size_t sort_temp_bytes,
+                               hipStream_t stream);
 hipError_t launch_prepare_nibbles(bool codes, bool t2, const uint64_t *d_bit_sets,
                                   uint32_t words_per_sample, const PlaneGeometry &geo,
                                   uint4 *d_planes, const uint32_t *perm, uint32_t s_tile_begin,
                                   uint32_t s_tile_end, const uint32_t *gate,
                                   const uint32_t *ready, hipStream_t stream);
+hipError_t launch_site_order(const uint64_t *d_bit_sets, uint32_t words_per_sample,
+                             const PlaneGeometry &geo, uint4 *d_planes, hipStream_t stream);
+hipError_t launch_gather_t2(const uint64_t *d_bit_sets, uint32_t words_per_sample,
+                            const PlaneGeometry &geo, uint4 *d_planes, uint32_t s_begin,
+                            uint32_t s_end, hipStream_t stream);
 hipError_t launch_mark_codes_ready(const uint32_t *gate, uint32_t *ready, hipStream_t stream);
 size_t mfma_split_scratch_bytes(uint32_t wgs);
 size_t mfma_split_counter_bytes(uint32_t wgs);
diff --git a/cuking_amd/csrc/king_filter.hip b/cuking_amd/csrc/king_filter.hip
--- a/cuking_amd/csrc/king_filter.hip
+++ b/cuking_amd/csrc/king_filter.hip
@@ -81,10 +81,12 @@
         yc += y;
         mc += m;
         hc += __popcll(h[k] & ~v[k]);
-        int32_t d = y - m;
-        d += __shfl_xor(d, 1);
-        d += __shfl_xor(d, 2);
-        if ((lane & 3) == 0 && in) atomicAdd(&phase_sum[wave][phase_of[w >> 2]], d);
+        if (cum != nullptr) {
+          int32_t d = y - m;
+          d += __shfl_xor(d, 1);
+          d += __shfl_xor(d, 2);
+          if ((lane & 3) == 0 && in) atomicAdd(&phase_sum[wave][phase_of[w >> 2]], d);
+        }
       }
     }
 #pragma unroll
@@ -95,6 +97,9 @@
     }
   }
   static_assert(kNumPhases == 128, "two phases per lane");
+  if (cum == nullptr) {
+    if (lane == 0) stats[ps] = make_float2((float)(yc - mc), (float)hc);
+  } else {
   const int32_t p0 = phase_sum[wave][2 * lane], p1 = phase_sum[wave][2 * lane + 1];
   int32_t run = p0 + p1;
 #pragma unroll
@@ -104,8 +109,9 @@
   }
   cum[(size_t)(2 * lane) * geo.s_stride + ps] = (float)(run - p1);
   if (2 * lane + 1 < kNumCum) cum[(size_t)(2 * lane + 1) * geo.s_stride + ps] = (float)run;
+  if (lane == 0) stats[ps] = make_float2((float)(yc - mc), (float)hc);
+  }
   if (lane == 0) {
-    stats[ps] = make_float2((float)(yc - mc), (float)hc);
     if (src != kNoPair && ((blockIdx.x & 15) == 0 || gridDim.x < 64)) {
       __hip_atomic_fetch_add(sums, 1ull, __ATOMIC_RELAXED, __HIP_MEMORY_SCOPE_AGENT);
       __hip_atomic_fetch_add(sums + 1, (unsigned long long)mc, __ATOMIC_RELAXED,
@@ -140,6 +146,40 @@
                :                                                               \
                : "s"(DST), "v"(lane16), "s"(SRC)                               \
                : "memory", "m0")
+
+__device__ uint32_t check_choice(const TiledArgs &a, uint32_t all_steps) {
+  float kappa = -1.f;
+  {
+    const float ns = (float)a.cohort_sums[0], nm = (float)a.cohort_sums[1],
+                nh = (float)a.cohort_sums[2];
+    if (ns > 0.f && nh > 0.f) {
+      const float sites = 256.f * (float)all_steps;
+      const float m = nm / (ns * sites), h = nh / (ns * sites);
+      kappa = m * (1.f + m / (2.f * h * (1.f - m))) + 4.6f * rsqrtf(sites) + 0.003f;
+    }
+  }
+  const uint32_t fc = kappa > 0.7f * a.kin_threshold ? 1u : 0u;
+  uint32_t share1 = 0, entry1 = 0;
+  const uint32_t sw1 = a.check1 & 0xFFu;
+  if (sw1 >= 2) {
+    entry1 = sw1 - 2;
+    if (entry1 >= 1 && entry1 < kNumCheckShares) share1 = kCheckShares64[entry1];
+  } else if (sw1 == 1 && kappa >= 0.f) {
+    const float need = (1.f - 2.f * a.kin_threshold) / (1.f - 2.f * kappa);
+    if (a.site_mass == nullptr) {
+      const float f64 = 64.f * need;
+      if (f64 <= 62.f) {
+        share1 = (uint32_t)ceilf(f64);
+        if (share1 < 32) share1 = 32;
+      }
+    } else {
+      for (uint32_t k = 32; k <= 62 && share1 == 0; ++k)
+        if (a.site_mass[k * kPhasesPerShare - 1] >= need) share1 = k;
+    }
+    if (share1 != 0) entry1 = 1;
+  }
+  return share1 | (entry1 << 8) | (fc << 16);
+}
 
 __device__ __forceinline__ int filter_tile(const TiledArgs &a, const uint32_t wg, uint4 *const lds) {
   uint32_t bid = wg;
@@ -175,6 +215,7 @@
   const uint32_t wave = __builtin_amdgcn_readfirstlane(threadIdx.x >> 6);
   const uint32_t wy = wave >> 1, wx = wave & 1;
   uint32_t xcd_pos = 0;
+  uint32_t choice = 0;
   if (!split && a.tile_done != nullptr) {
     uint32_t *verdict = reinterpret_cast<uint32_t *>(lds);
     if (threadIdx.x == 0) {
@@ -211,6 +252,11 @@
         }
       }
       verdict[0] = leave;
+      const uint32_t choice = a.check_steps != nullptr ? check_choice(a, a.geo.k_words / 8) : 0u;
+      verdict[1 + kPosSlots] = choice;
+      if (wg == 0 && a.check_steps != nullptr)
+        __hip_atomic_store(a.filter_totals + kTotalShare, (unsigned long long)(choice & 0xFFu),
+                           __ATOMIC_RELAXED, __HIP_MEMORY_SCOPE_AGENT);
     }
     if (a.rotate == 1 && threadIdx.x < kPosSlots) {
       const uint32_t x = wg & 7;
@@ -228,6 +274,7 @@
     }
     __syncthreads();
     const bool give_up = verdict[0] != 0;
+    choice = verdict[1 + kPosSlots];
     if (a.rotate == 1) {
 #pragma unroll
       for (uint32_t k = 0; k < kPosSlots; ++k) xcd_pos = max(xcd_pos, verdict[1 + k]);
@@ -250,6 +297,7 @@
       split ? part * all_steps / a.fsplit_parts : 0u);
   const uint32_t num_steps = __builtin_amdgcn_readfirstlane(
       split ? (part + 1) * all_steps / a.fsplit_parts - k_first : all_steps);
+  uint32_t ring_ph = kNumPhases, ring = all_steps;
   const uint4 *g_rows = a.t2 + (uint64_t)tr * kT;
   const uint4 *g_cols = a.t2 + a.geo.col_base + (uint64_t)tc * kT;
 
@@ -270,7 +318,7 @@
   auto addr_of = [&](uint32_t step, uint32_t buf) {
     Addr pa;
     if (step >= seg_steps) step = seg_steps - 1;
-    const int32_t rel = (int32_t)step - (int32_t)(step >= seg_wrap ? all_steps : 0u);
+    const int32_t rel = (int32_t)step - (int32_t)(step >= seg_wrap ? ring : 0u);
     pa.src = seg_src + (int64_t)rel * (int64_t)kstep_bytes;
     pa.dst = l_wave + buf * (kStageU4 * 16);
     asm volatile("" : "+s"(pa.src), "+s"(pa.dst));
@@ -279,7 +327,7 @@
   auto addr_next = [&](const Addr &cur, uint32_t step, uint32_t buf) {
     Addr pa;
     const int32_t adv = (int32_t)(step < seg_steps ? 1u : 0u) -
-                        (int32_t)(step == seg_wrap ? all_steps : 0u);
+                        (int32_t)(step == seg_wrap ? ring : 0u);
     pa.src = cur.src + (int64_t)adv * (int64_t)kstep_bytes;
     pa.dst = l_wave + buf * (kStageU4 * 16);
     asm volatile("" : "+s"(pa.src), "+s"(pa.dst));
@@ -396,62 +444,50 @@
 
   uint32_t chk0 = 0, chk1 = 0, entry1 = 0, share1 = 0;
   uint32_t phase = 0, k0 = 0, wrap = 0, start_abs = 0;
+  bool ring_head = false;
   if (!split && a.check_steps != nullptr && a.tile_done != nullptr) {
+    choice = __builtin_amdgcn_readfirstlane(choice);
+    share1 = choice & 0xFFu;
+    entry1 = (choice >> 8) & 0xFFu;
+    ring_head = a.site_mass != nullptr && share1 != 0 && a.check_steps[entry1] != 0;
+    if (ring_head) {
+      ring_ph = share1 * kPhasesPerShare;
+      ring = phase_step(all_steps, ring_ph);
+    }
     if (a.rotate != 0 && all_steps >= a.rotate_min_steps) {
       uint32_t base = 0;
       if (a.rotate == 1) {
-        const uint32_t r = xcd_pos % all_steps;
+        const uint32_t r = xcd_pos % ring;
         base = xcd_pos - r;
-        phase = (r * kNumPhases + all_steps / 2) / all_steps;
-        if (phase >= kNumPhases) {
+        phase = (r * ring_ph + ring / 2) / ring;
+        if (phase >= ring_ph) {
           phase = 0;
-          base += all_steps;
+          base += ring;
         }
       } else if (a.rotate == 2) {
-        phase = (bid * 37u + 11u) & (kNumPhases - 1);
+        phase = ((bid * 37u + 11u) & (kNumPhases - 1)) % ring_ph;
       } else {
-        phase = (a.rotate - 3u) & (kNumPhases - 1);
+        phase = ((a.rotate - 3u) & (kNumPhases - 1)) % ring_ph;
       }
       k0 = phase_step(all_steps, phase);
+      if (k0 >= ring) phase = k0 = 0;
       start_abs = base + k0;
-      wrap = k0 != 0 ? all_steps - k0 : 0u;
-    }
-    float kappa = -1.f;
-    {
-      const float ns = (float)a.cohort_sums[0], nm = (float)a.cohort_sums[1],
-                  nh = (float)a.cohort_sums[2];
-      if (ns > 0.f && nh > 0.f) {
-        const float sites = 256.f * (float)all_steps;
-        const float m = nm / (ns * sites), h = nh / (ns * sites);
-        kappa = m * (1.f + m / (2.f * h * (1.f - m))) + 4.6f * rsqrtf(sites) + 0.003f;
-      }
+      wrap = k0 != 0 ? ring - k0 : 0u;
     }
     auto steps_of = [&](uint32_t share) {
       const uint32_t hi = phase + share * kPhasesPerShare;
-      return hi <= kNumPhases ? phase_step(all_steps, hi) - k0
-                              : (all_steps - k0) + phase_step(all_steps, hi - kNumPhases);
+      return hi <= ring_ph ? phase_step(all_steps, hi) - k0
+                           : (ring - k0) + phase_step(all_steps, hi - ring_ph);
     };
-    if ((a.check0 == 2 || (a.check0 == 1 && kappa > 0.7f * a.kin_threshold)) &&
-        a.check_steps[0] != 0)
+    if ((a.check0 == 2 || (a.check0 == 1 && (choice >> 16) != 0)) && a.check_steps[0] != 0)
       chk0 = steps_of(kCheckShares64[0]);
-    const uint32_t sw1 = a.check1 & 0xFFu;
-    if (sw1 >= 2) {
-      entry1 = sw1 - 2;
-    } else if (sw1 == 1 && kappa >= 0.f) {
-      const float f64 = 64.f * (1.f - 2.f * a.kin_threshold) / (1.f - 2.f * kappa);
-      if (f64 <= 62.f) {
-        share1 = (uint32_t)ceilf(f64);
-        if (share1 < 32) share1 = 32;
-        entry1 = 1;
-      }
-    }
-#pragma unroll
-    for (uint32_t k = 1; k < kNumCheckShares; ++k)
-      if (sw1 >= 2 && k == entry1) share1 = kCheckShares64[k];
     if (share1 != 0 && a.check_steps[entry1] != 0) chk1 = steps_of(share1);
     if (chk0 >= num_steps) chk0 = 0;
     if (chk1 >= num_steps || chk1 <= chk0) chk1 = 0;
   }
+  ring_ph = __builtin_amdgcn_readfirstlane(ring_ph);
+  ring = __builtin_amdgcn_readfirstlane(ring);
+  const uint32_t ring_end = __builtin_amdgcn_readfirstlane(ring_head && wrap != 0 ? ring : 0u);
   chk0 = __builtin_amdgcn_readfirstlane(chk0);
   chk1 = __builtin_amdgcn_readfirstlane(chk1);
   share1 = __builtin_amdgcn_readfirstlane(share1);
@@ -460,15 +496,17 @@
   wrap = __builtin_amdgcn_readfirstlane(wrap);
   start_abs = __builtin_amdgcn_readfirstlane(start_abs);
   auto prefix_u_of = [&](uint32_t share, size_t idx, float total) {
+    auto cum = [&](uint32_t x) {
+      return x == 0 ? 0.f : x >= kNumPhases ? total : a.prefix_u[(size_t)(x - 1) * s_stride + idx];
+    };
     const uint32_t hi = phase + share * kPhasesPerShare;
-    const uint32_t xb = hi > kNumPhases ? hi - kNumPhases : hi;
-    float u = hi > kNumPhases ? total : 0.f;
-    if (xb == kNumPhases)
-      u += total;
-    else if (xb != 0)
-      u += a.prefix_u[(size_t)(xb - 1) * s_stride + idx];
-    if (phase != 0) u -= a.prefix_u[(size_t)(phase - 1) * s_stride + idx];
-    return u;
+    return hi <= ring_ph ? cum(hi) - cum(phase) : (cum(ring_ph) - cum(phase)) + cum(hi - ring_ph);
+  };
+  auto mass_of = [&](uint32_t share) {
+    if (a.site_mass == nullptr) return (float)share * (1.f / 64.f);
+    auto cum = [&](uint32_t x) { return x == 0 ? 0.f : a.site_mass[x - 1]; };
+    const uint32_t hi = phase + share * kPhasesPerShare;
+    return hi <= ring_ph ? cum(hi) - cum(phase) : (cum(ring_ph) - cum(phase)) + cum(hi - ring_ph);
   };
   unsigned long long *const pos_word =
       reinterpret_cast<unsigned long long *>(a.filter_ctrl + kCtrlPos) +
@@ -508,9 +546,12 @@
     uint32_t seg_end = num_steps;
     if (chk1 > seg_first) seg_end = chk1;
     if (chk0 > seg_first) seg_end = chk0;
+    if (ring_end > seg_first && ring_end < seg_end) seg_end = ring_end;
     seg_end = __builtin_amdgcn_readfirstlane(seg_end);
     seg_steps = seg_end - seg_first;
-    const uint32_t seg_k = seg_first >= wrap && wrap != 0 ? seg_first - wrap : k0 + seg_first;
+    const uint32_t seg_k = seg_first >= ring                ? seg_first
+                           : seg_first >= wrap && wrap != 0 ? seg_first - wrap
+                                                            : k0 + seg_first;
     seg_src = g_wave + (uint64_t)seg_k * kstep_bytes;
     seg_wrap = __builtin_amdgcn_readfirstlane(
         wrap > seg_first && wrap < seg_end ? wrap - seg_first : 0xFFFFFFFFu);
@@ -542,11 +583,17 @@
     if (step < seg_steps) F_KSTEP
     __builtin_amdgcn_s_waitcnt(0x0F70);
     __syncthreads();
-    F_PUBLISH(seg_end)
+    if (seg_end <= ring) {
+      F_PUBLISH(seg_end)
+    }
     if (seg_end == num_steps) break;
+    if (seg_end != chk0 && seg_end != chk1) {
+      seg_first = seg_end;
+      continue;
+    }
 
     const bool forecast = seg_end == chk0;
-    const float scale = forecast ? (float)kCheckShares64[0] * (1.f / 64.f) : 1.f;
+    const float scale = forecast ? mass_of(kCheckShares64[0]) : 1.f;
     float2 *const ck_rows = reinterpret_cast<float2 *>(lds);
     float2 *const ck_cols = ck_rows + kT;
     uint32_t *const ck_words = reinterpret_cast<uint32_t *>(ck_cols + kT);
@@ -909,11 +956,11 @@
 
 hipError_t launch_sample_stats(const uint64_t *d_bit_sets, uint32_t words_per_sample,
                                const PlaneGeometry &geo, uint4 *d_planes, uint32_t s_begin,
-                               uint32_t s_end, hipStream_t stream) {
+                               uint32_t s_end, bool prefix, hipStream_t stream) {
   if (s_end > geo.s_stride) s_end = geo.s_stride;
   if (s_begin >= s_end) return hipSuccess;
   float2 *stats = plane_tmp_stats(d_planes, geo);
-  float *prefix = plane_tmp_prefix(d_planes, geo);
+  float *cum = prefix ? plane_tmp_prefix(d_planes, geo) : nullptr;
   unsigned long long *sums = const_cast<unsigned long long *>(plane_cohort_sums(d_planes, geo));
   uint32_t *steps = const_cast<uint32_t *>(plane_check_steps(d_planes, geo));
   CheckWords cw;
@@ -922,7 +969,7 @@
   for (uint32_t k = 0; k < kNumCheckShares; ++k)
     cw.w[k] = check_step_of(all_steps, k, g_check_min_steps.load());
   sample_stats_kernel<<<dim3((s_end - s_begin + 3) / 4), dim3(256), 0, stream>>>(
-      d_bit_sets, words_per_sample, geo, stats, prefix, sums, steps, cw, s_begin, s_end);
+      d_bit_sets, words_per_sample, geo, stats, cum, sums, steps, cw, s_begin, s_end);
   return hipGetLastError();
 }
 
diff --git a/cuking_amd/csrc/king_site_order.hip b/cuking_amd/csrc/king_site_order.hip
--- /dev/null
+++ b/cuking_amd/csrc/king_site_order.hip
@@ -0,0 +1,280 @@
+#include <hip/hip_runtime.h>
+
+#include "king_common.h"
+
+namespace cuking {
+
+namespace {
+
+constexpr uint32_t kCountChunks = 32;
+constexpr uint32_t kCountBits = 21;
+
+__host__ __device__ inline uint32_t stored_samples(const PlaneGeometry &g) {
+  return g.diag ? g.num_rows : g.num_rows + g.num_cols;
+}
+__host__ __device__ inline uint32_t subset_stride(uint32_t n) {
+  uint32_t s = n <= 4096 ? 1u : 16u;
+  while ((n + s - 1) / s >= (1u << (kCountBits - 1))) s *= 2;
+  return s;
+}
+
+__global__ __launch_bounds__(256) void site_counts_kernel(const uint64_t *__restrict__ bits,
+                                                          uint32_t words_per_sample, uint32_t n_sub,
+                                                          uint32_t stride,
+                                                          unsigned long long *__restrict__ counts) {
+  const uint32_t plane_words = words_per_sample / 2;
+  const uint32_t lane = threadIdx.x & 63;
+  const uint32_t w = __builtin_amdgcn_readfirstlane(blockIdx.x * 4 + (threadIdx.x >> 6));
+  if (w >= plane_words) return;
+  uint32_t het = 0, alt = 0, mis = 0;
+  const uint64_t row_step = (uint64_t)kCountChunks * stride * words_per_sample;
+  const uint64_t *row = bits + (uint64_t)blockIdx.y * stride * words_per_sample + w;
+  uint32_t i = blockIdx.y;
+  constexpr uint32_t kAhead = 8;
+  for (; i + (kAhead - 1) * kCountChunks < n_sub; i += kAhead * kCountChunks) {
+    uint64_t hw[kAhead], mw[kAhead];
+#pragma unroll
+    for (uint32_t k = 0; k < kAhead; ++k) {
+      hw[k] = row[k * row_step];
+      mw[k] = row[k * row_step + plane_words];
+    }
+#pragma unroll
+    for (uint32_t k = 0; k < kAhead; ++k) {
+      const uint32_t h = (uint32_t)(hw[k] >> lane) & 1u, m = (uint32_t)(mw[k] >> lane) & 1u;
+      het += h & (m ^ 1u);
+      alt += m & (h ^ 1u);
+      mis += h & m;
+    }
+    row += kAhead * row_step;
+  }
+  for (; i < n_sub; i += kCountChunks, row += row_step) {
+    const uint32_t h = (uint32_t)(row[0] >> lane) & 1u, m = (uint32_t)(row[plane_words] >> lane) & 1u;
+    het += h & (m ^ 1u);
+    alt += m & (h ^ 1u);
+    mis += h & m;
+  }
+  const uint32_t site = w * 64 + lane;
+  const unsigned long long packed = (unsigned long long)het |
+                                    ((unsigned long long)alt << kCountBits) |
+                                    ((unsigned long long)mis << (2 * kCountBits));
+  if (packed != 0) atomicAdd(counts + site, packed);
+}
+
+__device__ inline float site_key(unsigned long long c, uint32_t n_sub) {
+  const uint32_t mask = (1u << kCountBits) - 1;
+  const double het = (double)(c & mask), alt = (double)((c >> kCountBits) & mask),
+               mis = (double)((c >> (2 * kCountBits)) & mask);
+  const double ref = (double)n_sub - het - alt - mis;
+  const double def = n_sub - mis;
+  const double k = def * (ref + alt) - (alt - ref) * (alt - ref);
+  return k > 0.0 ? (float)(k / ((double)n_sub * (double)n_sub)) : 0.f;
+}
+
+__global__ __launch_bounds__(256) void window_order_kernel(
+    const unsigned long long *__restrict__ counts, uint32_t n_sub, uint32_t plane_sites,
+    uint32_t units, uint16_t *__restrict__ local, float *__restrict__ unit_mass) {
+  __shared__ float key[kSiteWindowSites];
+  __shared__ uint16_t order[kSiteWindowSites];
+  const uint32_t win = blockIdx.x, windows = gridDim.x;
+  const uint32_t n_units = min(kSiteWindowUnits, units - win * kSiteWindowUnits);
+  const uint32_t n = n_units * 64;
+  const uint32_t first = win * kSiteWindowSites;
+  for (uint32_t l = threadIdx.x; l < n; l += 256)
+    key[l] = first + l < plane_sites ? site_key(counts[first + l], n_sub) : 0.f;
+  __syncthreads();
+  for (uint32_t l = threadIdx.x; l < n; l += 256) {
+    const float k = key[l];
+    uint32_t rank = 0;
+    for (uint32_t j = 0; j < n; ++j) {
+      const float kj = key[j];
+      rank += (kj > k || (kj == k && j < l)) ? 1u : 0u;
+    }
+    order[rank] = (uint16_t)l;
+  }
+  __syncthreads();
+  for (uint32_t l = threadIdx.x; l < n; l += 256) local[first + l] = order[l];
+  const uint32_t last = units - (windows - 1) * kSiteWindowUnits;
+  if (threadIdx.x < n_units) {
+    float m = 0.f;
+    for (uint32_t r = 0; r < 64; ++r) m += key[order[threadIdx.x * 64 + r]];
+    unit_mass[site_order_unit(threadIdx.x, win, windows, last)] = m;
+  }
+}
+
+__global__ __launch_bounds__(kNumPhases) void site_mass_kernel(const float *__restrict__ unit_mass,
+                                                               uint32_t all_steps,
+                                                               float *__restrict__ mass) {
+  __shared__ float phase[kNumPhases];
+  const uint32_t x = threadIdx.x;
+  float m = 0.f;
+  for (uint32_t u = 4 * phase_step(all_steps, x); u < 4 * phase_step(all_steps, x + 1); ++u)
+    m += unit_mass[u];
+  phase[x] = m;
+  __syncthreads();
+  if (x == 0) {
+    double total = 0.0;
+    for (uint32_t k = 0; k < kNumPhases; ++k) total += phase[k];
+    double run = 0.0;
+    for (uint32_t k = 0; k < kNumPhases; ++k) {
+      run += phase[k];
+      mass[k] = total > 0.0 ? (float)(run / total) : (float)(k + 1) / (float)kNumPhases;
+    }
+    mass[kNumPhases - 1] = 1.f;
+  }
+}
+
+__device__ inline uint32_t spread16(uint32_t x) {
+  x &= 0xFFFFu;
+  x = (x | (x << 8)) & 0x00FF00FFu;
+  x = (x | (x << 4)) & 0x0F0F0F0Fu;
+  x = (x | (x << 2)) & 0x33333333u;
+  x = (x | (x << 1)) & 0x55555555u;
+  return x;
+}
+
+constexpr uint32_t kGatherSamples = 64;
+constexpr uint32_t kCodeRow = kSiteWindowSites / 16 + 1;
+
+__global__ __launch_bounds__(256) void gather_t2_kernel(
+    const uint64_t *__restrict__ bits, uint32_t words_per_sample, PlaneGeometry geo,
+    const uint32_t *__restrict__ perm, const uint16_t *__restrict__ local_all,
+    uint4 *__restrict__ t2, float *__restrict__ prefix, uint32_t s_begin, uint32_t s_end) {
+  __shared__ uint32_t codes[kGatherSamples * kCodeRow];
+  __shared__ uint32_t acc[kNumPhases / 2][kGatherSamples];
+  const uint32_t lane = threadIdx.x & 63;
+  const uint32_t wave = __builtin_amdgcn_readfirstlane(threadIdx.x >> 6);
+  const uint32_t s0 = s_begin + blockIdx.x * kGatherSamples;
+  const uint32_t plane_words = words_per_sample / 2;
+  const uint32_t units = geo.k_words / 2, all_steps = geo.k_words / 8;
+  const uint32_t windows = (units + kSiteWindowUnits - 1) / kSiteWindowUnits;
+  const uint32_t last = units - (windows - 1) * kSiteWindowUnits;
+  for (uint32_t k = threadIdx.x; k < kNumPhases / 2 * kGatherSamples; k += 256)
+    (&acc[0][0])[k] = 0;
+  const uint32_t lw = threadIdx.x & 15;
+  const uint64_t *rows[4];
+#pragma unroll
+  for (int i = 0; i < 4; ++i) {
+    const uint32_t ps = s0 + (threadIdx.x >> 4) + 16 * i;
+    const uint32_t src = ps < s_end ? perm[ps] : kNoSample;
+    rows[i] = src != kNoSample ? bits + (uint64_t)src * words_per_sample : nullptr;
+  }
+  uint64_t h[4], m[4];
+  auto load = [&](uint32_t win) {
+    const uint32_t w = win * kSiteWindowUnits + lw;
+#pragma unroll
+    for (int i = 0; i < 4; ++i) {
+      const bool in = rows[i] != nullptr && w < plane_words;
+      h[i] = in ? rows[i][w] : ~0ull;
+      m[i] = in ? rows[i][plane_words + w] : 0ull;
+    }
+  };
+  load(0);
+  for (uint32_t win = 0; win < windows; ++win) {
+    __syncthreads();
+#pragma unroll
+    for (int i = 0; i < 4; ++i) {
+      uint32_t *row = codes + ((threadIdx.x >> 4) + 16 * i) * kCodeRow + lw * 4;
+#pragma unroll
+      for (int q = 0; q < 4; ++q) {
+        const uint32_t hq = (uint32_t)(h[i] >> (16 * q)), mq = (uint32_t)(m[i] >> (16 * q));
+        row[q] = spread16(hq) | (spread16(mq) << 1);
+      }
+    }
+    const uint32_t n_units = win + 1 < windows ? kSiteWindowUnits : last;
+    __syncthreads();
+    if (win + 1 < windows) load(win + 1);
+    const uint32_t *my = codes + lane * kCodeRow;
+    for (uint32_t j = wave; j < n_units; j += 4) {
+      const uint32_t *ix = reinterpret_cast<const uint32_t *>(
+          local_all + (size_t)win * kSiteWindowSites + j * 64);
+      uint32_t idx[32];
+#pragma unroll
+      for (int k = 0; k < 32; ++k) idx[k] = __builtin_amdgcn_readfirstlane(ix[k]);
+      uint32_t r[4];
+#pragma unroll
+      for (int d = 0; d < 4; ++d) {
+        uint32_t v = 0;
+#pragma unroll
+        for (int t = 0; t < 8; ++t) {
+          const int sh = 8 * d + t, sl = 32 + 8 * d + t;
+          const uint32_t hi = (idx[sh >> 1] >> (16 * (sh & 1))) & 0xFFFFu;
+          const uint32_t lo = (idx[sl >> 1] >> (16 * (sl & 1))) & 0xFFFFu;
+          v |= ((my[hi >> 4] >> (2 * (hi & 15))) & 3u) << (4 * t + 2);
+          v |= ((my[lo >> 4] >> (2 * (lo & 15))) & 3u) << (4 * t);
+        }
+        r[d] = v;
+      }
+      int32_t cnt = 0;
+      uint32_t out[4];
+#pragma unroll
+      for (int d = 0; d < 4; ++d) {
+        const uint32_t H = r[d] & 0x55555555u, M = (r[d] >> 1) & 0x55555555u;
+        const uint32_t y = ~H & 0x55555555u, a = M & y;
+        out[d] = (a << 1) | y;
+        cnt += __popc(y) - __popc(H & M);
+      }
+      const uint32_t u = site_order_unit(j, win, windows, last);
+      const uint32_t ps = s0 + lane;
+      if (ps < s_end) t2[(size_t)u * geo.s_stride + ps] = make_uint4(out[0], out[1], out[2], out[3]);
+      const uint32_t st = u >> 2;
+      const uint32_t x = (kNumPhases * (st + 1) - 1) / all_steps;
+      const uint32_t xp = x < kNumPhases ? x : kNumPhases - 1;
+      atomicAdd(&acc[xp >> 1][lane], (uint32_t)cnt << (16 * (xp & 1)));
+    }
+  }
+  __syncthreads();
+  if (wave == 0) {
+    const uint32_t ps = s0 + lane;
+    if (ps < s_end) {
+      int32_t run = 0;
+      for (uint32_t x = 0; x < kNumCum; ++x) {
+        const uint32_t w = acc[x >> 1][lane];
+        const int32_t lo = (int16_t)(w & 0xFFFFu);
+        run += (x & 1) ? (int32_t)(w - (uint32_t)lo) >> 16 : lo;
+        prefix[(size_t)x * geo.s_stride + ps] = (float)run;
+      }
+    }
+  }
+}
+
+}
+
+hipError_t launch_site_order(const uint64_t *d_bit_sets, uint32_t words_per_sample,
+                             const PlaneGeometry &geo, uint4 *d_planes, hipStream_t stream) {
+  const uint32_t sites = geo.k_words * 32, units = geo.k_words / 2;
+  const uint32_t plane_sites = words_per_sample / 2 * 64;
+  const uint32_t n = stored_samples(geo);
+  if (units == 0 || n == 0 || sites > kSiteOrderMaxSites) return hipErrorInvalidValue;
+  const uint32_t stride = subset_stride(n), n_sub = (n + stride - 1) / stride;
+  unsigned long long *counts = plane_site_counts(d_planes, geo);
+  hipError_t e = hipMemsetAsync(counts, 0, (size_t)sites * 8, stream);
+  if (e != hipSuccess) return e;
+  site_counts_kernel<<<dim3((plane_sites / 64 + 3) / 4, kCountChunks), dim3(256), 0, stream>>>(
+      d_bit_sets, words_per_sample, n_sub, stride, counts);
+  e = hipGetLastError();
+  if (e != hipSuccess) return e;
+  const uint32_t windows = (units + kSiteWindowUnits - 1) / kSiteWindowUnits;
+  window_order_kernel<<<dim3(windows), dim3(256), 0, stream>>>(
+      counts, n_sub, plane_sites, units, plane_site_local(d_planes, geo),
+      plane_unit_mass(d_planes, geo));
+  e = hipGetLastError();
+  if (e != hipSuccess) return e;
+  site_mass_kernel<<<dim3(1), dim3(kNumPhases), 0, stream>>>(
+      plane_unit_mass(d_planes, geo), geo.k_words / 8, plane_site_mass(d_planes, geo));
+  return hipGetLastError();
+}
+
+hipError_t launch_gather_t2(const uint64_t *d_bit_sets, uint32_t words_per_sample,
+                            const PlaneGeometry &geo, uint4 *d_planes, uint32_t s_begin,
+                            uint32_t s_end, hipStream_t stream) {
+  if (s_end > geo.s_stride) s_end = geo.s_stride;
+  if (s_begin >= s_end || geo.k_words < 8) return hipSuccess;
+  gather_t2_kernel<<<dim3((s_end - s_begin + kGatherSamples - 1) / kGatherSamples), dim3(256), 0,
+                     stream>>>(d_bit_sets, words_per_sample, geo, plane_perm(d_planes, geo),
+                               plane_site_local(d_planes, geo),
+                               const_cast<uint4 *>(plane_t2(d_planes, geo)),
+                               const_cast<float *>(plane_prefix_u(d_planes, geo)), s_begin, s_end);
+  return hipGetLastError();
+}
+
+}
diff --git a/cuking_amd/csrc/king_sort.hip b/cuking_amd/csrc/king_sort.hip
--- a/cuking_amd/csrc/king_sort.hip
+++ b/cuking_amd/csrc/king_sort.hip
@@ -36,13 +36,15 @@
   if (p - begin >= n) {
     perm[p] = kNoSample;
     stats[p] = make_float2(0.f, 0.f);
+    if (prefix != nullptr)
 #pragma unroll
-    for (uint32_t c = 0; c < kNumCum; ++c) prefix[(size_t)c * geo.s_stride + p] = 0.f;
+      for (uint32_t c = 0; c < kNumCum; ++c) prefix[(size_t)c * geo.s_stride + p] = 0.f;
     return;
   }
   const uint32_t src = order[p - begin];
   perm[p] = (geo.diag || src < geo.rows_padded) ? src : geo.num_rows + (src - geo.col_base);
   stats[p] = tmp_stats[src];
+  if (prefix == nullptr) return;
 #pragma unroll 7
   for (uint32_t c = 0; c < kNumCum; ++c)
     prefix[(size_t)c * geo.s_stride + p] = tmp_prefix[(size_t)c * geo.s_stride + src];
@@ -60,14 +62,15 @@
 
 hipError_t launch_sample_order(const PlaneGeometry &geo, uint32_t words_per_sample,
                                uint4 *d_planes, uint32_t s_begin, uint32_t s_end, bool sort,
-                               void *sort_temp, size_t sort_temp_bytes, hipStream_t stream) {
+                               bool with_prefix, void *sort_temp, size_t sort_temp_bytes,
+                               hipStream_t stream) {
   if (s_end > geo.s_stride) s_end = geo.s_stride;
   if (s_begin >= s_end) return hipSuccess;
   const float2 *tmp_stats = plane_tmp_stats(d_planes, geo);
   const float *tmp_prefix = plane_tmp_prefix(d_planes, geo);
   uint32_t *perm = plane_perm(d_planes, geo);
   float2 *stats = const_cast<float2 *>(plane_stats(d_planes, geo));
-  float *prefix = const_cast<float *>(plane_prefix_u(d_planes, geo));
+  float *prefix = with_prefix ? const_cast<float *>(plane_prefix_u(d_planes, geo)) : nullptr;
   uint32_t *words = plane_sort_words(d_planes, geo);
   const float stored_sites = 32.f * (float)words_per_sample;
   struct Side { uint32_t begin, end, real_end; };
```
